# HKUST-Aerial-Robotics/FUEL

Measured on AMD Instinct MI355X. Metric: plan_cycles_per_sec, higher is better.
Workload: dtype u64 bit-planes / u16 (u32 beyond 255 voxels) exact squared distances / f32 ESDF / f64 log-odds and B-spline

## Files before the change

### fuel_amd/_lib.py

```python
import ctypes as C
import os

_HERE = os.path.dirname(os.path.abspath(__file__))
LIB_PATH = os.environ.get("FUELMI_LIB_PATH") or os.path.join(_HERE, "libfuelmi.so")
_LIB = None

K_INFLATE, K_ESDF_ZY, K_ESDF_X, K_FRONTIER, K_BSPLINE, K_INSERT, K_COUNT = range(7)


class FuelmiError(RuntimeError):
    pass


class MapCfg(C.Structure):
    _fields_ = [
        ("resolution", C.c_double),
        ("map_size", C.c_double * 3),
        ("ground_height", C.c_double),
        ("obstacles_inflation", C.c_double),
        ("local_bound_inflate", C.c_double),
        ("default_dist", C.c_double),
        ("optimistic", C.c_int),
        ("signed_dist", C.c_int),
        ("p_hit", C.c_double),
# ... 204 lines not shown
RENDER_HOST_NODE, RENDER_CUDA_NODE = 0, 1


class BsplineCfg(C.Structure):
    _fields_ = [(n, C.c_double) for n in
                ("ld_smooth", "ld_dist", "ld_feasi", "ld_start", "ld_end", "ld_guide", "ld_waypt",
                 "ld_view", "ld_time", "dist0", "max_vel", "max_acc", "wnl", "dlmin")] + \
               [("bspline_degree", C.c_int)]


_dp = C.POINTER(C.c_double)
_ip = C.POINTER(C.c_int)


class BsplineBatch(C.Structure):
    _fields_ = [
        ("cost_function", C.c_int), ("dim", C.c_int), ("point_num", C.c_int), ("n_traj", C.c_int),
        ("x", _dp), ("pt_dist", _dp), ("knot_span", _dp), ("time_lb", _dp),
        ("start_state", _dp), ("end_state", _dp), ("end_n", C.c_int),
        ("guide_pts", _dp), ("waypoints", _dp), ("waypt_idx", _ip), ("n_waypt", C.c_int),
        ("view_pt", _dp), ("view_dir", _dp), ("view_idx", _ip),
    ]


_P = C.c_void_p
_PP = C.POINTER(C.c_void_p)
SYMBOLS = {
    "fuelmi_last_error": (C.c_char_p, []),
    "fuelmi_version": (C.c_char_p, []),
    "fuelmi_init": (C.c_int, [C.c_int]),
    "fuelmi_hw_queues": (C.c_int, []),
    "fuelmi_hw_queues_state": (C.c_int, []),
    "fuelmi_device_count": (C.c_int, []),
    "fuelmi_map_create": (C.c_int, [C.POINTER(MapCfg), _PP]),
    "fuelmi_map_destroy": (None, [_P]),
    "fuelmi_map_get_info": (C.c_int, [_P, C.POINTER(MapInfo)]),
    "fuelmi_map_input_points": (C.c_int, [_P, C.c_void_p, C.c_int, C.c_int, _dp]),
    "fuelmi_map_insert_plan": (C.c_int, [_ip]),
    "fuelmi_map_input_depth": (C.c_int, [_P, C.c_void_p, C.c_int, C.c_int, C.POINTER(DepthCfg), _dp, _dp,
                                         C.POINTER(C.c_int)]),
    "fuelmi_host_register": (C.c_int, [C.c_void_p, C.c_size_t]),
    "fuelmi_host_unregister": (C.c_int, [C.c_void_p]),
    "fuelmi_device_alloc": (C.c_int, [C.c_int, C.c_size_t, C.POINTER(C.c_void_p)]),
    "fuelmi_device_upload": (C.c_int, [C.c_void_p, C.c_void_p, C.c_size_t]),
    "fuelmi_device_free": (C.c_int, [C.c_void_p]),
    "fuelmi_hbm_triad": (C.c_int, [C.c_int, C.c_size_t, C.c_int, _dp]),
    "fuelmi_hbm_expand": (C.c_int, [C.c_int, C.c_size_t, C.c_int, _dp]),
    "fuelmi_map_project_depth": (C.c_int, [_P, C.c_void_p, C.c_int, C.c_int, C.POINTER(DepthCfg), _dp, _dp,
                                           C.c_void_p, C.c_int, C.POINTER(C.c_int)]),
    "fuelmi_map_inflate_local": (C.c_int, [_P]),
    "fuelmi_map_update_esdf": (C.c_int, [_P]),
    "fuelmi_map_set_esdf_family": (C.c_int, [_P, C.c_int]),
    "fuelmi_map_last_esdf_family": (C.c_int, [_P]),
    "fuelmi_map_esdf_plan": (C.c_int, [_ip, _ip, _ip, C.c_int, C.c_int, _ip]),
    "fuelmi_map_last_inflate_kernel": (C.c_int, [_P]),
    "fuelmi_map_reset_buffer_all": (C.c_int, [_P]),
    "fuelmi_map_reset_buffer": (C.c_int, [_P, _dp, _dp]),
    "fuelmi_map_set_occupied": (C.c_int, [_P, _dp, C.c_int, C.c_int]),
    "fuelmi_map_get_local_bound": (C.c_int, [_P, _ip, _ip]),
    "fuelmi_map_set_local_bound": (C.c_int, [_P, _ip, _ip]),
    "fuelmi_map_get_updated_box": (C.c_int, [_P, _dp, _dp, C.c_int]),
    "fuelmi_map_set_updated_box": (C.c_int, [_P, _dp, _dp]),
    "fuelmi_map_upload_occupancy": (C.c_int, [_P, _dp]),
    "fuelmi_map_sync_host": (C.c_int, [_P, _ip, _ip, _dp, C.c_void_p, _dp]),
    "fuelmi_map_register_mirrors": (C.c_int, [_P, _dp, C.c_void_p, _dp]),
    "fuelmi_map_unregister_mirrors": (C.c_int, [_P]),
    "fuelmi_map_dist_grad": (C.c_int, [_P, _dp, C.c_int, _dp, _dp]),
    "fuelmi_map_coarse_dist": (C.c_int, [_P, _dp, C.c_int, _dp]),
    "fuelmi_map_query_state": (C.c_int, [_P, _ip, C.c_int, _ip, _ip]),
    "fuelmi_map_synchronize": (C.c_int, [_P]),
    "fuelmi_frontier_set_viewpoint_cfg": (C.c_int, [_P, C.POINTER(ViewpointCfg)]),
    "fuelmi_frontier_compute_to_visit": (C.c_int, [_P, C.POINTER(C.c_int), C.POINTER(C.c_int)]),
    "fuelmi_frontier_viewpoint_count": (C.c_int, [_P, C.c_int, C.c_int]),
    "fuelmi_frontier_viewpoints": (C.c_int, [_P, C.c_int, C.c_int, _dp, C.POINTER(C.c_int)]),
    "fuelmi_frontier_is_covered": (C.c_int, [_P, C.POINTER(C.c_int)]),
    "fuelmi_frontier_cluster_filtered_size": (C.c_int, [_P, C.c_int, C.c_int]),
    "fuelmi_frontier_cluster_filtered": (C.c_int, [_P, C.c_int, C.c_int, C.c_void_p]),
    "fuelmi_frontier_create": (C.c_int, [_P, C.POINTER(FrontierCfg), _PP]),
    "fuelmi_frontier_destroy": (None, [_P]),
    "fuelmi_frontier_reset": (C.c_int, [_P]),
    "fuelmi_frontier_stats": (C.c_int, [_P, C.POINTER(C.c_int)]),
    "fuelmi_frontier_resolved_in_launch": (C.c_int, [_P]),
    "fuelmi_frontier_path_stats": (C.c_int, [_P, C.POINTER(C.c_int)]),
    "fuelmi_frontier_changed_stats": (C.c_int, [_P, C.POINTER(C.c_int)]),
    "fuelmi_frontier_order_stats": (C.c_int, [_P, C.POINTER(C.c_int)]),
    "fuelmi_frontier_synchronize": (C.c_int, [_P]),
    "fuelmi_bench_cycles": (C.c_int, [_P, _P, _P, _dp, _dp, C.c_int, C.c_int, C.POINTER(C.c_int), _dp]),
    "fuelmi_bench_host_profile": (C.c_int, [_P, _dp]),
    "fuelmi_bench_cycles_delivered": (C.c_int, [_P, _P, _P, _dp, _dp, C.c_int, _ip, C.c_size_t, _dp, _dp,
                                                C.POINTER(C.c_int), _dp]),
    "fuelmi_bench_stream": (C.c_int, [_P, _P, _P, C.c_int, C.POINTER(C.c_void_p), C.c_int, C.c_int, C.POINTER(DepthCfg),
                                      _dp, _dp, C.c_int, C.POINTER(C.c_int), _dp, _dp]),
    "fuelmi_frontier_search": (C.c_int, [_P, _ip]),
    "fuelmi_frontier_search_begin": (C.c_int, [_P]),
    "fuelmi_frontier_search_end": (C.c_int, [_P, _ip]),
    "fuelmi_frontier_keep_previous": (C.c_int, [_P, C.c_int]),
    "fuelmi_frontier_commit": (C.c_int, [_P, C.c_int]),
    "fuelmi_frontier_count": (C.c_int, [_P, C.c_int]),
    "fuelmi_frontier_cluster_size": (C.c_int, [_P, C.c_int, C.c_int]),
    "fuelmi_frontier_cluster_cells": (C.c_int, [_P, C.c_int, C.c_int, _ip]),
    "fuelmi_frontier_cluster_centres": (C.c_int, [_P, C.c_int, C.c_int, _dp]),
    "fuelmi_frontier_cluster_info": (C.c_int, [_P, C.c_int, C.c_int, _dp]),
    "fuelmi_frontier_removed_count": (C.c_int, [_P]),
    "fuelmi_frontier_removed_ids": (C.c_int, [_P, _ip]),
    "fuelmi_frontier_get_flags": (C.c_int, [_P, C.c_void_p]),
    "fuelmi_map_path_costs": (C.c_int, [_P, C.POINTER(PathCfg), C.c_int, _dp, _dp, _dp, _ip, _ip, _dp]),
    "fuelmi_map_path_stats": (C.c_int, [_P, _ip]),
    "fuelmi_map_refine_tours": (C.c_int, [_P, C.POINTER(RefineCfg), C.c_int, _dp, _ip, _ip, _dp, _ip, _dp, _ip, _dp]),
    "fuelmi_map_goal_paths": (C.c_int, [_P, C.POINTER(GoalCfg), C.c_int, _dp, _dp, _ip, _dp, _ip, _dp, _dp, _ip, _dp]),
    "fuelmi_map_goal_path_times": (C.c_int, [_P, _dp]),
    "fuelmi_map_waypoint_trajs": (C.c_int, [_P, C.POINTER(WptrajCfg), C.c_int, _ip, _dp, _dp, _dp, _ip, _dp, _dp, _ip, _dp,
                                            _ip, _dp, _dp, _dp, _dp]),
    "fuelmi_wptraj_plan": (C.c_int, [C.POINTER(WptrajCfg), _ip]),
    "fuelmi_map_kino_paths": (C.c_int, [_P, C.POINTER(KinoCfg), C.c_int, _dp, _dp, _dp, _dp, _dp, _ip, _ip, _ip, _ip, _ip,
                                        _dp, _dp, _dp, _ip, _dp, _dp, _dp, _dp, _ip, _ip, _dp, _dp]),
    "fuelmi_bspline_dev_load_kino": (C.c_int, [_P, C.POINTER(KinoCfg), _dp, _dp, _dp, _dp, _dp, _ip, _dp]),
    "fuelmi_kino_plan": (C.c_int, [C.POINTER(KinoCfg), C.POINTER(C.c_longlong)]),
    "fuelmi_map_topo_paths": (C.c_int, [_P, C.POINTER(TopoCfg), C.c_int, _dp, _dp, C.c_int, _ip, _dp, C.c_int, _ip, _dp, _dp,
                                        _ip, _ip, _ip, _ip, _ip, _ip, _dp, _ip, _ip, _dp, _ip, _dp, _ip, _dp, _ip, _dp]),
    "fuelmi_topo_plan": (C.c_int, [C.POINTER(TopoCfg), C.POINTER(C.c_longlong)]),
    "fuelmi_map_topo_pool_bytes": (C.c_longlong, [_P]),
    "fuelmi_map_collision_ranges": (C.c_int, [_P, C.POINTER(ColRangeCfg), C.c_int, _ip, _dp, _dp, _ip, _ip, _ip, _ip, _dp,
                                              _dp, _dp, _dp, _ip, _dp, _ip, _dp, _dp, _dp]),
    "fuelmi_colrange_plan": (C.c_int, [C.POINTER(ColRangeCfg), _ip]),
    "fuelmi_map_guide_points": (C.c_int, [_P, C.c_int, C.c_int, _dp, _ip, _dp, C.c_double, C.c_int, C.c_int, _ip, _ip, _dp,
                                          _ip, _ip, _ip, _dp]),
    "fuelmi_map_local_segments": (C.c_int, [_P, C.POINTER(LocalSegCfg), C.c_int, _ip, _dp, _dp, _dp, _ip, _dp, _dp, _dp, _dp,
                                            _dp, _dp, C.c_int, _ip, _ip, _dp, _dp, _dp, _ip, _ip, _dp, _ip, _dp, _dp, _ip,
                                            _dp, _dp, _ip, _dp]),
    "fuelmi_localseg_plan": (C.c_int, [C.POINTER(LocalSegCfg), _ip]),
    "fuelmi_bspline_dev_load_local_segments": (C.c_int, [_P, C.c_int, C.c_int, C.c_int, _ip, _dp, _dp, _dp, _ip, _dp, _dp,
                                                         _dp, _dp, _dp, _dp, _ip, _ip, _dp, _dp, _dp, _ip, _dp]),
    "fuelmi_map_info_gains": (C.c_int, [_P, C.POINTER(GainCfg), C.c_int, _dp, _ip, _dp, C.c_int, _ip, _dp, _ip, _ip, _dp, _ip,
                                        _ip, _ip]),
    "fuelmi_map_yaw_paths": (C.c_int, [_P, C.POINTER(YawPathCfg), C.c_int, _ip, _dp, _dp, _dp, _ip, _dp, _dp, _ip, _dp, _ip,
                                       _dp, _dp, _ip]),
    "fuelmi_yawpath_plan": (C.c_int, [C.POINTER(YawPathCfg), _ip]),
    "fuelmi_map_plan_yaws": (C.c_int, [_P, C.POINTER(BsplineCfg), C.POINTER(YawCfg), C.c_int, _ip, _dp, _dp, _dp, _dp, _ip,
                                       _dp, _ip, _dp, _dp, _ip, _dp, _dp, _dp, _dp, _dp]),
    "fuelmi_bspline_dev_plan_yaws": (C.c_int, [_P, C.POINTER(YawCfg), _dp, _dp, _ip, _dp, _ip, _dp, _dp, _ip, _dp, _dp,
                                               _dp, _dp, _dp]),
    "fuelmi_yaw_plan": (C.c_int, [C.POINTER(YawCfg), _ip]),
    "fuelmi_map_check_trajs": (C.c_int, [_P, C.POINTER(TrajChkCfg), C.c_int, _ip, _dp, _dp, _dp, _ip, _ip, _dp, _ip, _ip, _dp,
                                         _dp, _ip, _dp]),
    "fuelmi_bspline_dev_check_trajs": (C.c_int, [_P, C.POINTER(TrajChkCfg), _dp, _ip, _ip, _dp, _ip, _ip, _dp, _dp, _ip, _dp]),
    "fuelmi_traj_check_plan": (C.c_int, [C.POINTER(TrajChkCfg), _ip]),
    "fuelmi_map_sample_trajs": (C.c_int, [_P, C.POINTER(TrajSmpCfg), C.c_int, _ip, _dp, _dp, _ip, _dp, _dp, _dp, _ip, _dp,
                                          _ip, _dp, _dp, _dp, _dp, _dp, _dp, _dp, _dp, _dp]),
    "fuelmi_bspline_dev_sample_trajs": (C.c_int, [_P, C.POINTER(TrajSmpCfg), _ip, _dp, _dp, _dp, _ip, _dp, _ip, _dp, _dp,
                                                  _dp, _dp, _dp, _dp, _dp, _dp, _dp]),
    "fuelmi_traj_sample_plan": (C.c_int, [C.POINTER(TrajSmpCfg), _ip]),
    "fuelmi_map_adjust_trajs": (C.c_int, [_P, C.POINTER(TrajAdjCfg), C.c_int, _ip, _dp, _dp, _dp, _dp, _ip, _ip, _dp, _dp, _dp,
                                          _ip]),
    "fuelmi_bspline_dev_adjust_trajs": (C.c_int, [_P, C.POINTER(TrajAdjCfg), _dp, _dp, _ip, _ip, _dp, _dp, _dp, _ip]),
    "fuelmi_traj_adjust_plan": (C.c_int, [C.POINTER(TrajAdjCfg), _ip]),
    "fuelmi_map_extract_cloud": (C.c_int, [_P, C.POINTER(CloudCfg), C.c_void_p, C.c_int, _ip]),
    "fuelmi_cloud_plan": (C.c_int, [_ip, _ip, _ip, _ip]),
    "fuelmi_map_cloud_times": (C.c_int, [_P, _dp]),
    "fuelmi_tsp_create": (C.c_int, [C.c_int, C.POINTER(TspCfg), _PP]),
    "fuelmi_tsp_destroy": (None, [_P]),
    "fuelmi_tsp_solve": (C.c_int, [_P, C.c_int, _ip, C.POINTER(C.c_int32), _ip, C.POINTER(C.c_int64), _ip]),
    "fuelmi_render_create": (C.c_int, [C.POINTER(RenderCfg), _PP]),
    "fuelmi_render_destroy": (C.c_int, [_P]),
    "fuelmi_render_set_cloud": (C.c_int, [_P, C.c_void_p, C.c_int]),
    "fuelmi_render_depth": (C.c_int, [_P, C.c_int, _dp, _dp, C.c_double, C.c_void_p, C.c_void_p, _ip]),
    "fuelmi_render_frame_raw": (C.c_void_p, [_P, C.c_int]),
# ... 50 lines not shown
```

### fuel_amd/csrc/frontier.hip

```cpp
#include <algorithm>
#include <chrono>
#include <cmath>
#include <cstdlib>
#include <cstring>
#include <list>
#include <memory>
#include <vector>

#include "fuelmi_internal.h"
#include "frontier_internal.h"

__global__ void k_zero_words(u64* p, int n) {
  for (int i = blockIdx.x * blockDim.x + threadIdx.x; i < n; i += gridDim.x * blockDim.x) p[i] = 0ull;
}

template <typename T>
static int dmalloc(fuelmi_frontier* f, T** p, size_t n) {
  void* d = nullptr;
  HIPCHK(hipMalloc(&d, std::max<size_t>(n, 1) * sizeof(T)));
  f->allocs.push_back(d);
  *p = (T*)d;
  const char* fp = reinterpret_cast<const char*>(p), *f0 = reinterpret_cast<const char*>(&f->F);
  if (fp >= f0 && fp < f0 + sizeof(FArgs))
    f->f_scratch.push_back({(size_t)(fp - f0), std::max<size_t>(n, 1) * sizeof(T)});
// ... 304 lines not shown
    std::swap(f->F, f->F2);
    if (f->pool_dirty) HIPCHK(hipStreamWaitEvent(f->stream, f->ev_tail, 0));
    f->pool_dirty = false;
  }
  std::swap(f->flag, f->flag2);
  f->flag_cur ^= 1;
  f->F.flag = f->flag.p;
  f->zero_deferred = true;
  return defer_zeroing ? FUELMI_OK : frontier_finish_reset(f);
}

extern "C" int fuelmi_frontier_search_begin(fuelmi_frontier* f) {
  ARGCHK(f);
  FRONTIER_HAS_MAP(f);
  FRONTIER_NOT_SEARCHING(f, "fuelmi_frontier_search_begin");
  fuelmi_map* m = f->map;
  HIPCHK(hipSetDevice(m->device));
  const Geo& g = m->g;
  FArgs& F = f->F;
  f->tmp.clear();
  g_ht.start();
  {
    const int rcm = frontier_materialize_lists(f);
    if (rcm) return rcm;
  }
  {
    const int rcr = frontier_apply_reset(f, true);
    if (rcr) return rcr;
  }
  struct FinishReset {
    fuelmi_frontier* f;
    ~FinishReset() {
      (void)frontier_finish_reset(f);
      g_ht.lap(9);
    }
  } finish_reset{f};
  g_ht.lap(0);
  double umin[3], umax[3];
  fuelmi_map_get_updated_box(m, umin, umax, 1);

  if (f->planes_waited[f->flag_cur] != m->planes_ver + 1) {
    HIPCHK(hipStreamWaitEvent(f->stream, m->ev_planes, 0));
    f->planes_waited[f->flag_cur] = m->planes_ver + 1;
  }
  f->scope.reset(new StageScope(m, FUELMI_K_FRONTIER, f->stream));
  f->removed_ids.clear();
  for (int q = 0; q < 3; ++q) f->rm_lo[q] = 1, f->rm_hi[q] = 0;
  g_ht.lap(1);
  struct PlanesRead {
    fuelmi_frontier* f;
    bool done = false;
    ~PlanesRead() {
      if (done || !f->map) return;
      if (!f->mark_planes_read)
        map_add_late_reader(f->map, f->stream, f->ev_planes_read, &f->mark_planes_read);
      else if (hipEventRecord(f->ev_planes_read, f->stream) == hipSuccess)
        map_add_plane_reader(f->map, f->ev_planes_read);
    }
  } planes_read{f};
  int rc = remove_changed_begin(f, umin, umax);
  if (rc) return rc;
  g_ht.lap(2);

  const int nv[3] = {g.nx, g.ny, g.nz};
  FVar hv;
  memset(&hv, 0, sizeof(hv));
  bool empty = false;
  for (int k = 0; k < 3; ++k) {
    double infl = (k == 2) ? 0.5 : 1.0;
    double smin = std::max(umin[k] - infl, m->cfg.box_min[k]);
    double smax = std::min(umax[k] + infl, m->cfg.box_max[k]);
    int lo = (int)std::floor((smin - g.org[k]) * g.res_inv);
    int hi = (int)std::floor((smax - g.org[k]) * g.res_inv);
    lo = std::max(lo, 0);
    hi = std::min(hi, nv[k] - 1);
    hv.sbox.lo[k] = lo;
    hv.sbox.hi[k] = hi;
    if (lo > hi) empty = true;
  }
  f->pending = true;
  f->fusion_at_begin = m->fusion_count;
  f->search_empty = empty;
  f->fast_launched = false;
  if (empty) return FUELMI_OK;

  int rlo[3], rhi[3];
  const bool all = f->dirty_all || f->seen_epoch != m->occ_epoch;
  for (int k = 0; k < 3; ++k) {
    rlo[k] = hv.sbox.lo[k], rhi[k] = hv.sbox.hi[k];
    if (f->rm_lo[0] <= f->rm_hi[0]) rlo[k] = std::min(rlo[k], f->rm_lo[k]), rhi[k] = std::max(rhi[k], f->rm_hi[k]);
    if (all) rlo[k] = 0, rhi[k] = nv[k] - 1;
    hv.qreg.lo[k] = std::max(F.qbox.lo[k], rlo[k]);
    hv.qreg.hi[k] = std::min(F.qbox.hi[k], rhi[k]);
  }
  f->dirty_all = true;
  bool have_q = true;
  for (int k = 0; k < 3; ++k)
    if (hv.qreg.lo[k] > hv.qreg.hi[k]) have_q = false;
  if (!have_q)
    for (int k = 0; k < 3; ++k) hv.qreg.lo[k] = 1, hv.qreg.hi[k] = 0;
  hv.nty = hv.ntiles = 0;
  hv.nty_f = hv.ntiles_f = 0;
  hv.ftx = 4, hv.fty = 8;
  if (have_q) {
    const int qx = hv.qreg.hi[0] - hv.qreg.lo[0] + 1, qy = hv.qreg.hi[1] - hv.qreg.lo[1] + 1;
    hv.nty = (qy + f->TY - 1) / f->TY;
    hv.ntiles = ((qx + f->TX - 1) / f->TX) * hv.nty;
  }
  {
    int p0[2], p1[2];
    for (int k = 0; k < 2; ++k) {
      p0[k] = hv.sbox.lo[k], p1[k] = hv.sbox.hi[k];
      if (have_q) p0[k] = std::min(p0[k], hv.qreg.lo[k]), p1[k] = std::max(p1[k], hv.qreg.hi[k]);
      p0[k] = std::max(p0[k], F.qbox.lo[k]);
      p1[k] = std::min(p1[k], F.qbox.hi[k] + 1);
    }
    const int qx = p1[0] - p0[0] + 1, qy = p1[1] - p0[1] + 1;
    int pick = 3;
    for (int k = 0; k < 4; ++k)
      if (menu_tiles(qx, qy, k) >= 512) {
        pick = k;
        break;
      }
    if (f->menu_min_ttl > 0) --f->menu_min_ttl, pick = std::max(pick, f->menu_min);
    f->fast_menu = pick;
    hv.px0 = p0[0], hv.py0 = p0[1], hv.px1 = p1[0], hv.py1 = p1[1];
    set_fast_tiles(hv, pick);
  }
  auto adr = [&](const int* id) { return (long)id[0] * g.nyz + (long)id[1] * g.nz + id[2]; };
  long a_lo = adr(hv.sbox.lo), a_hi = adr(hv.sbox.hi);
  if (have_q) {
    a_lo = std::min(a_lo, adr(hv.qreg.lo));
    a_hi = std::max(a_hi, adr(hv.qreg.hi));
  }
  a_lo = std::max(0L, a_lo - 2L * g.nyz);
  a_hi = std::min((long)g.N - 1, a_hi + 2L * g.nyz);
  hv.w0 = (int)((a_lo >> 6) & ~255L);
  const int w_hi = (int)(a_hi >> 6);
  hv.nblocks = (w_hi - hv.w0) / 256 + 1;
  hv.nwords = hv.nblocks * 256;
  const bool fast = f->fast_ok;
  hv.fresh = 0;
  if (F.dbg)
    HIPCHK(hipMemsetAsync(F.dbg, 0, (size_t)(3 * (hv.ntiles_f + 1)) * FR_DBG_SLOTS * sizeof(unsigned long long), f->stream));
  hv.epoch = ++f->epoch;
  if (hv.epoch == 0u) hv.epoch = f->epoch = 1u;
  *f->h_var = hv;

  f->npass = f->last_nkept > 192 ? 2 : 1;

  g_ht.lap(3);
  if (fast) {
    f->fast_launched = true;
    planes_read.done = true;
    return frontier_enqueue_fast(f);
  }
  return frontier_launch_legacy(f, f->npass);
}

static void frontier_timing_report(fuelmi_frontier* f) {
  const FArgs& F = f->F;
  (void)hipStreamSynchronize(f->stream);
  const int nt = f->h_var->ntiles_f;
  std::vector<unsigned long long> d((size_t)(3 * (nt + 1)) * FR_DBG_SLOTS);
  (void)hipMemcpy(d.data(), F.dbg, d.size() * sizeof(unsigned long long), hipMemcpyDeviceToHost);
  unsigned long long t0 = ~0ull, t1 = 0;
  double phase[8] = {0, 0, 0, 0, 0, 0, 0, 0};
  int busiest = 0, nonempty = 0;
  for (int b = 0; b < nt; ++b) {
    const unsigned long long* r = &d[(size_t)b * FR_DBG_SLOTS];
    if (!r[0]) continue;
    t0 = std::min(t0, r[0]);
    for (int k = 1; k < 8; ++k)
      if (r[k]) t1 = std::max(t1, r[k]);
    if (r[8] > d[(size_t)busiest * FR_DBG_SLOTS + 8]) busiest = b;
    if (r[8]) ++nonempty;
  }
  {
    double st_av = 0, st_mx = 0, du_av = 0, du_mx = 0;
    int cnt = 0;
    for (int b = 0; b < nt; ++b) {
      const unsigned long long* r = &d[(size_t)b * FR_DBG_SLOTS];
      if (!r[0] || !r[6] || r[6] < r[0]) continue;
      const double st = (double)(r[0] - t0) / 100.0, du = (double)(r[6] - r[0]) / 100.0;
      st_av += st, st_mx = std::max(st_mx, st), du_av += du, du_mx = std::max(du_mx, du), ++cnt;
    }
    std::fprintf(stderr, "[fr-timing] ccl: %d tiles with cells: start avg %.1f max %.1f, duration avg %.1f max %.1f us\n", cnt,
                 st_av / std::max(cnt, 1), st_mx, du_av / std::max(cnt, 1), du_mx);
  }
  const unsigned long long* rb = &d[(size_t)busiest * FR_DBG_SLOTS];
  for (int k = 1; k < 8; ++k) phase[k] = rb[k] && rb[k - 1] ? (double)(rb[k] - rb[k - 1]) / 100.0 : 0.0;
  std::fprintf(stderr, "[fr-timing] tiles %d (non-empty %d) span %.1f us; busiest tile %d (%llu cells, start +%.1f us): "
               "bits %.1f labels %.1f unions %.1f roots %.1f records %.1f write %.1f us; %llu unions, %llu find steps, %llu links, %llu roots\n", nt, nonempty,
               (double)(t1 - t0) / 100.0, busiest, rb[8], (double)(rb[0] - t0) / 100.0, phase[1], phase[2], phase[3],
               phase[4], phase[5], phase[6], rb[9], rb[10], rb[11], rb[12]);
  for (int kern = 1; kern <= 2; ++kern) {
    const int np = kern == 1 ? 4 : 6;
    double mx[8] = {0}, av[8] = {0};
    unsigned long long c0 = ~0ull, c1 = 0;
    int cnt = 0;
    for (int b = 0; b < nt; ++b) {
      const unsigned long long* r = &d[(size_t)(kern * (nt + 1) + b) * FR_DBG_SLOTS];
      if (!r[0] || !r[np]) continue;
      c0 = std::min(c0, r[0]), c1 = std::max(c1, r[np]);
      for (int k = 1; k <= np; ++k) {
        const double ph = r[k] && r[k - 1] ? (double)(r[k] - r[k - 1]) / 100.0 : 0.0;
        mx[k] = std::max(mx[k], ph), av[k] += ph;
      }
      ++cnt;
    }
    double st_av = 0, st_mx = 0, du_av = 0, du_mx = 0;
    for (int b = 0; b < nt; ++b) {
      const unsigned long long* r = &d[(size_t)(kern * (nt + 1) + b) * FR_DBG_SLOTS];
      if (!r[0] || !r[np]) continue;
      const double st = (double)(r[0] - c0) / 100.0, du = (double)(r[np] - r[0]) / 100.0;
      st_av += st, st_mx = std::max(st_mx, st), du_av += du, du_mx = std::max(du_mx, du);
    }
    {
      unsigned long long e0 = ~0ull;
      double ea = 0, em = 0, la = 0, lm = 0;
      int n2 = 0;
      for (int b = 0; b < nt; ++b) {
        const unsigned long long v = d[(size_t)b * FR_DBG_SLOTS + 12 + kern];
        if (v) e0 = std::min(e0, v);
      }
      for (int b = 0; b < nt; ++b) {
        const unsigned long long v = d[(size_t)b * FR_DBG_SLOTS + 12 + kern];
        const unsigned long long* r = &d[(size_t)(kern * (nt + 1) + b) * FR_DBG_SLOTS];
        if (!v || !r[0] || r[0] < v) continue;
        const double e = (double)(v - e0) / 100.0, l = (double)(r[0] - v) / 100.0;
        ea += e, em = std::max(em, e), la += l, lm = std::max(lm, l), ++n2;
      }
      std::fprintf(stderr, "[fr-timing]   entry avg %.1f max %.1f us after the first workgroup; entry -> first stamp avg %.1f max %.1f us\n",
                   ea / std::max(n2, 1), em, la / std::max(n2, 1), lm);
    }
    std::fprintf(stderr, "[fr-timing] %s: span %.1f us over %d tiles; start avg %.1f max %.1f, duration avg %.1f max %.1f; phases avg/max:",
                 kern == 1 ? "cross (bits, build, list, append)" : "out (bits, cells, column, first, rows, flags)",
                 cnt ? (double)(c1 - c0) / 100.0 : 0.0, cnt, st_av / std::max(cnt, 1), st_mx, du_av / std::max(cnt, 1), du_mx);
    for (int k = 1; k <= np; ++k) std::fprintf(stderr, " %.1f/%.1f", av[k] / std::max(cnt, 1), mx[k]);
    std::fprintf(stderr, "\n");
  }
  const unsigned long long* rr = &d[(size_t)nt * FR_DBG_SLOTS];
  std::fprintf(stderr, "[fr-timing] resolve: init %.1f unions %.1f find %.1f reduce %.1f clusters %.1f seeds %.1f rank %.1f "
               "codes %.1f publish %.1f us; pairs %llu roots %llu cells %llu\n", (rr[1] - rr[0]) / 100.0,
               (rr[2] - rr[1]) / 100.0, (rr[3] - rr[2]) / 100.0, (rr[4] - rr[3]) / 100.0, (rr[5] - rr[4]) / 100.0, 0.0,
               (rr[6] - rr[5]) / 100.0, (rr[7] - rr[6]) / 100.0, (rr[8] - rr[7]) / 100.0, rr[9], rr[10], rr[11]);
}

static int frontier_collect_fast(fuelmi_frontier* f) {
  fuelmi_map* m = f->map;
  FArgs& F = f->F;
  u32* counts = F.h_counts;
  volatile u32* stamp = counts + 15;
  const u32 want = f->h_var->epoch;
  const auto w0 = std::chrono::steady_clock::now();
  const int rcw = stamp_wait<u32>(stamp, want, f->stream, "frontier search: the chain finished without publishing its result");
  f->wait_us_acc += std::chrono::duration<double, std::micro>(std::chrono::steady_clock::now() - w0).count();
  if (rcw) return rcw;
  g_ht.lap(11);
  f->tail_pending = true;
  F.fast = 1;
  if (F.dbg) frontier_timing_report(f);
  if (counts[2] == 3u) {
    *stamp = 0u;
    const int rcl = frontier_enqueue_late_resolve(f);
    if (rcl) return rcl;
    const int rc = stamp_wait<u32>(stamp, want, f->stream, "frontier search: k_resolve finished without publishing its result");
    if (rc) return rc;
    ++f->n_late_resolve;
  }
  f->kr_skip_ok = counts[2] == 0u && counts[9] == 1u && 2u * counts[10] <= f->rcap_used;
  ++f->n_fast;
  if (counts[9] == 1u)
    ++f->n_in_launch;
  else if (f->fuse_tried && counts[2] == 0u)
    f->fuse_skip = 16;
  if (counts[2] == 2u && m->fusion_count != f->fusion_at_begin) {
    fuelmi_set_error("frontier search: the fast chain overflowed AFTER the map was fused again (a frame queued between "
                     "_search_begin and _search_end): the occupancy this search was about is gone -- call _search_end before the next fusion "
                     "on inputs this noisy");
    remove_changed_end(f);
    f->dirty_all = true;
    return FUELMI_ELIMIT;
  }
  while (counts[2] == 2u && f->fast_menu < 3 && (counts[6] == 11u || counts[6] == 12u || counts[6] == 15u || counts[6] == 18u)) {
    HIPCHK(frontier_tail_sync(f) == FUELMI_OK ? hipSuccess : hipErrorUnknown);
    ++f->fast_menu;
    FVar hv = *f->h_var;
    set_fast_tiles(hv, f->fast_menu);
    hv.epoch = ++f->epoch;
    if (hv.epoch == 0u) hv.epoch = f->epoch = 1u;
    *f->h_var = hv;
    f->kr_skip_ok = false;
    if (getenv("FUELMI_FR_TIMING")) std::fprintf(stderr, "[fr-timing] capacity code %u: again with %d x %d tiles\n", counts[6], hv.ftx, hv.fty);
    const int rcr = frontier_enqueue_fast(f);
    if (rcr) return rcr;
    const int rcw = stamp_wait<u32>(stamp, hv.epoch, f->stream,
                                    "frontier search: the re-tiled chain finished without publishing its result");
    if (rcw) return rcw;
    f->tail_pending = true;
    ++f->n_retiled;
    f->menu_min = f->fast_menu, f->menu_min_ttl = 64;
  }
  if (counts[2] == 2u) {
    --f->n_fast;
    ++f->n_fallback;
    if (getenv("FUELMI_FR_TIMING")) std::fprintf(stderr, "[fr-timing] fallback to the legacy chain: capacity code %u\n", counts[6]);
    HIPCHK(frontier_tail_sync(f) == FUELMI_OK ? hipSuccess : hipErrorUnknown);
    F.fast = 0;
    f->npass = 1;
    int rcl = frontier_enqueue_chain(f, f->npass);
    if (rcl) return rcl;
    HIPCHK(hipStreamSynchronize(f->stream));
  }
  return FUELMI_OK;
}


static int frontier_assemble(fuelmi_frontier* f, u32 nq, u32 nkept, u32 n_out) {
  const Geo& g = f->map->g;
  FArgs& F = f->F;
  KeptRec* h_rec = F.h_rec;
  const u32* h_part = F.h_part;
  const u32* h_cells = F.h_cells;
  u32 ncl = nkept, ncells = n_out;
  std::vector<std::vector<float>> filtered;
  const bool split_mode = f->cfg.split != 0;
  bool ref_order = f->cfg.reference_order == 1;
  if (f->cfg.reference_order == 2) {
    ref_order = true;
    for (u32 r = 0; r < nkept; ++r)
      if (h_rec[r].size > FR_REFORDER_AUTO) ref_order = false;
  }
  f->ref_now = ref_order;
  f->order_last = ref_order ? 1 : 0;
  if (ref_order)
    ++f->n_order_ref;
  else if (f->cfg.reference_order == 2) {
    ++f->n_order_fallback;
    u32 big = 0;
    for (u32 r = 0; r < nkept; ++r) big = std::max(big, h_rec[r].size);
    f->order_fallback_cells = big;
  }
  int fin = nkept <= 256 ? 1 : 0;
  std::vector<u32> off2;
  u32 n_in = n_out;
  if (split_mode && !ref_order) HIPCHK(frontier_tail_sync(f) == FUELMI_OK ? hipSuccess : hipErrorUnknown);
  if (ref_order) {
    int rc = frontier_reference_order(f, nq, nkept, n_out, fin, &n_in, &off2, !split_mode);
    if (rc) return rc;
    f->tail_pending = false;
    fin = 1 - fin;
    ncells = n_in;
  }
  if (split_mode) {
    int rc = frontier_split_run(f, nq, nkept, n_in, fin, &ncl, &ncells, &filtered);
    if (rc) return rc;
    fin = ncl <= 256 ? 1 : 0;
  }
  f->last_fin = fin;
  f->cells_fetch = F.fast && !ref_order && !split_mode && nq > F.hcells_direct_max;
  f->cells_fetch_n = ncells;
  const u32 nchunk = ((ref_order || F.fast) && !split_mode) ? 0u : (ncells + SZ_CH - 1) / SZ_CH;
  for (u32 c = 0; c < nchunk; ++c) {
    const u32* rec = h_part + (size_t)c * 10;
    const u32 r = rec[0];
    if (r >= ncl) continue;
    for (int q = 0; q < 3; ++q) {
      h_rec[r].sum[q] += rec[1 + q];
      h_rec[r].box[q] = std::min(h_rec[r].box[q], rec[4 + q]);
      h_rec[r].box[3 + q] = std::max(h_rec[r].box[3 + q], rec[7 + q]);
    }
  }

  for (u32 r = 0; r < ncl; ++r) {
    const KeptRec& kr = h_rec[r];
    f->tmp.emplace_back();
    HCluster& c = f->tmp.back();
    const bool seed = !split_mode && kr.slot >= nq;
    const u32 cnt = kr.size - (seed ? 1u : 0u);
    c.lazy = reinterpret_cast<const int*>(h_cells) + kr.off;
    c.lazy_n = cnt;
    if (ref_order && !split_mode) {
      c.lazy = reinterpret_cast<const int*>(h_cells) + off2[r];
      c.lazy_n = kr.size;
    }
// ... 69 lines not shown
    ~DropLate() {
      if (f->map) map_drop_late_reader(f->map, f->ev_planes_read);
    }
  } drop_late{f};
  if (f->search_empty) {
    if (!f->pend_rm.empty()) {
      HIPCHK(hipStreamSynchronize(f->stream));
      remove_changed_end(f);
    }
    return FUELMI_OK;
  }
  FArgs& F = f->F;
  const u32* counts = F.h_counts;
  F.fast = 0;
  g_ht.start();
  if (g_ht.on) --g_ht.n;
  g_ht.lap(10);
  if (f->fast_launched) {
    const int rc = frontier_collect_fast(f);
    if (rc) return rc;
  } else {
    ++f->n_legacy;
    HIPCHK(stream_poll(f->stream));
  }
  remove_changed_end(f);
  if (f->rm_failed) {
    f->rm_failed = false;
    f->dirty_all = true;
    fuelmi_set_error("frontier search: the changed-cluster test's in-kernel barrier timed out (device oversubscribed for 50 ms?)");
    return FUELMI_EHIP;
  }
  if (counts[2] || counts[3] > F.cap_kept) {
    fuelmi_set_error("frontier capacity exceeded (cells %u/%u seeds %u/%u clusters %u/%u)", counts[0], F.cap_q,
                     counts[1], F.cap_s, counts[3], F.cap_kept);
    return FUELMI_ELIMIT;
  }
  const u32 nq = counts[0], nkept = counts[3], n_out = counts[5];
  f->last_nkept = (int)nkept;
  if (nkept > 256 && f->npass < 2) {
    const int rc = frontier_second_pass(f);
    if (rc) return rc;
  }
  if (nkept == 0) {
    f->dirty_all = false;
    f->seen_epoch = m->occ_epoch;
    return FUELMI_OK;
  }
  const int rc = frontier_assemble(f, nq, nkept, n_out);
  if (rc) return rc;
  *n_new = (int)f->tmp.size();
  f->dirty_all = false;
  f->seen_epoch = m->occ_epoch;
  g_ht.lap(12);
  return FUELMI_OK;
}


extern "C" int fuelmi_frontier_search(fuelmi_frontier* f, int* n_new) {
  ARGCHK(f && n_new);
  int rc = fuelmi_frontier_search_begin(f);
  if (rc) return rc;
  return fuelmi_frontier_search_end(f, n_new);
}

extern "C" int fuelmi_frontier_synchronize(fuelmi_frontier* f) {
  ARGCHK(f);
  FRONTIER_HAS_MAP(f);
  HIPCHK(hipSetDevice(f->device));
  f->tail_pending = false;
  HIPCHK(frontier_drain(f));
  return FUELMI_OK;
}
extern "C" int fuelmi_frontier_resolved_in_launch(const fuelmi_frontier* f) { return f ? f->n_in_launch : FUELMI_EINVAL; }
extern "C" int fuelmi_frontier_stats(const fuelmi_frontier* f, int out3[3]) {
  ARGCHK(f && out3);
  out3[0] = f->n_fast, out3[1] = f->n_legacy, out3[2] = f->n_fallback;
  return FUELMI_OK;
}
extern "C" int fuelmi_frontier_path_stats(const fuelmi_frontier* f, int out2[2]) {
  ARGCHK(f && out2);
  out2[0] = f->n_late_resolve, out2[1] = f->n_retiled;
  return FUELMI_OK;
}
extern "C" int fuelmi_frontier_changed_stats(const fuelmi_frontier* f, int out[9]) {
  ARGCHK(f && out);
  for (int k = 0; k < 4; ++k) out[k] = f->rm_paths[k];
  out[4] = f->rm_last_nc, out[5] = (int)f->rm_last_total, out[6] = f->rm_last_mark;
  out[7] = f->n_pool_rebuilds, out[8] = (int)f->pool_cap;
  return FUELMI_OK;
}
extern "C" int fuelmi_frontier_order_stats(const fuelmi_frontier* f, int out4[4]) {
  ARGCHK(f && out4);
  out4[0] = f->order_last, out4[1] = f->n_order_ref, out4[2] = f->n_order_fallback, out4[3] = (int)f->order_fallback_cells;
  return FUELMI_OK;
}

extern "C" int fuelmi_frontier_reset(fuelmi_frontier* f) {
  ARGCHK(f);
  FRONTIER_HAS_MAP(f);
  FRONTIER_NOT_SEARCHING(f, "fuelmi_frontier_reset");
  fuelmi_map* m = f->map;
  HIPCHK(hipSetDevice(m->device));
  f->frontiers.clear();
  f->dormant.clear();
  f->prev.clear();
  if (f->keep_prev && f->stream2 && !f->fresh_pending && !f->tmp.empty()) {
    f->prev.swap(f->tmp);
    if (f->cells_fetch) {
      f->cells_fetch = false;
      HIPCHK(hipMemcpyAsync(f->F.h_cells, f->F.ms_val[f->last_fin], (size_t)f->cells_fetch_n * sizeof(u32), hipMemcpyDeviceToHost,
                            f->stream));
    }
    HIPCHK(hipEventRecord(f->ev_prev, f->stream));
    f->prev_pending = true;
    f->tail_pending = false;
  }
  f->tmp.clear();
  f->removed_ids.clear();
  f->dirty_all = true;
  f->pool_used = 0;
  f->fresh_pending = true;
  return FUELMI_OK;
}

extern "C" int fuelmi_frontier_keep_previous(fuelmi_frontier* f, int on) {
  ARGCHK(f);
  f->keep_prev = on != 0;
  if (!on) f->prev.clear();
  return FUELMI_OK;
}

extern "C" int fuelmi_frontier_commit(fuelmi_frontier* f, int dormant) {
  ARGCHK(f);
  FRONTIER_HAS_MAP(f);
  FRONTIER_NOT_SEARCHING(f, "fuelmi_frontier_commit");
  auto& dst = dormant ? f->dormant : f->frontiers;
  HIPCHK(hipSetDevice(f->map->device));
  const int rc = frontier_keep_clusters(f, f->tmp);
  if (rc) return rc;
  dst.splice(dst.end(), f->tmp);
  return FUELMI_OK;
}
```

### fuel_amd/csrc/frontier_internal.h

```cpp
#ifndef FUELMI_FRONTIER_INTERNAL_H_
#define FUELMI_FRONTIER_INTERNAL_H_

#include <algorithm>
#include <chrono>
#include <cstring>
#include <list>
#include <memory>
#include <vector>

#include "fuelmi_internal.h"

#define NOCLAIM 0xFFFFFFFFu
#define SZ_CH 1024

struct KeptRec {
  u32 addr, slot, size, off;
  unsigned long long sum[3];
  u32 box[6];
  u32 pad[2];
};

struct FVar {
  Box3 sbox;
  int w0;
  int nwords;
  int nblocks;
  int fresh;
  Box3 qreg;
  int nty, ntiles;
  u32 epoch;
  int pad2;
  int nty_f, ntiles_f;
  int ftx, fty;
  int px0, py0, px1, py1;
  int ntx_f;
  int pad3[3];
};

#define FR_RCAP 8192
#define FR_RC8 (FR_RCAP / 8)
#define FR_TCELL 2048
#define FR_TPAIR 1536
#define FR_TROOT 128
#define FR_TXS 16
#define FR_KCAP 256
#define FR_PCAP (1u << 18)
#define FCTR(k) ((k) * 32)
#define FR_DONE_CTR FCTR(32)
#define FR_NCTR (41 * 32)
#define FR_PMCAP 16384
#define FR_REFORDER_AUTO 26624u
#define FR_UNCLAIMED 0xFFFFFFFFu
#define FR_NOTKEPT 0xFFFFFFFEu
struct TRec {
  u32 size;
  u32 sx, sy, sz;
  u32 lo[3], hi[3];
  u32 tx;
  u32 own;
};

struct FArgs {
  Box3 qbox;
  const FVar* var;
  u32 cap_q, cap_s;
  int cluster_min;
  const u64* occ;
  const u64* unk;
  u64* flag;
  u64* qb;
  u64* sb;
  u64* pref;
  u64* blocksum;
  u64* blockscan;
  u32* counts;
  u32* cell_adr;
  u32* parent;
  u32* claim;
  int* cell_slot;
  u32* seed_adr;
  u32* csize;
  u32* kept;
  u32 cap_kept;
  int* slot2rank;
  struct KeptRec* krec;
  u32* ms_key[2];
  u32* ms_val[2];
  u32* ms_hist;
  u32 ms_nb_max;
  u32* info_part;
  u32* h_counts;
  struct KeptRec* h_rec;
  u32* h_part;
  u32* h_cells;
  u32 hcells_direct_max;
  int keys_from_slots;
  FVar* var_w;
  u32* tq;
  u32* ts;
  unsigned char* vlab;
  unsigned char* tlab;
  u32* t_base;
  u32* t_nroots;
  struct TRec* trec;
  u32* tclaim;
  u32* rcode;
  unsigned short* rrow;
  u32* pm;
  int pm_stride;
  u32* pairs;
  u32* fctr;
  int fast;
  unsigned long long* dbg;
};
#define FR_HCELLS_DIRECT 32768u
#define FR_DBG_SLOTS 16
#define FR_DBG_MARK(F, blk, k)                                                                   \
  do {                                                                                           \
    if ((F).dbg && threadIdx.x == 0) (F).dbg[(size_t)(blk) * FR_DBG_SLOTS + (k)] = wall_clock64(); \
  } while (0)

#ifdef __HIPCC__
__device__ __forceinline__ void st_agent(u32* p, u32 v) { __hip_atomic_store(p, v, __ATOMIC_RELAXED, __HIP_MEMORY_SCOPE_AGENT); }
__device__ __forceinline__ u32 ld_agent(const u32* p) { return __hip_atomic_load(p, __ATOMIC_RELAXED, __HIP_MEMORY_SCOPE_AGENT); }
__device__ __forceinline__ void wait_vm_stores() { asm volatile("s_waitcnt vmcnt(0)" ::: "memory"); }
__device__ __forceinline__ void ld_agent_trec2(const TRec* p0, const TRec* p1, TRec& A, TRec& B) {
  static_assert(sizeof(TRec) == 48, "TRec is fetched as three 16-byte pieces");
  uint4 a0, a1, a2, b0, b1, b2;
  asm volatile(
      "global_load_dwordx4 %0, %6, off sc1\n\t"
      "global_load_dwordx4 %1, %6, off offset:16 sc1\n\t"
      "global_load_dwordx4 %2, %6, off offset:32 sc1\n\t"
      "global_load_dwordx4 %3, %7, off sc1\n\t"
      "global_load_dwordx4 %4, %7, off offset:16 sc1\n\t"
      "global_load_dwordx4 %5, %7, off offset:32 sc1\n\t"
      "s_waitcnt vmcnt(0)"
      : "=&v"(a0), "=&v"(a1), "=&v"(a2), "=&v"(b0), "=&v"(b1), "=&v"(b2)
      : "v"(p0), "v"(p1)
      : "memory");
  A.size = a0.x, A.sx = a0.y, A.sy = a0.z, A.sz = a0.w, A.lo[0] = a1.x, A.lo[1] = a1.y, A.lo[2] = a1.z, A.hi[0] = a1.w;
  A.hi[1] = a2.x, A.hi[2] = a2.y, A.tx = a2.z, A.own = a2.w;
  B.size = b0.x, B.sx = b0.y, B.sy = b0.z, B.sz = b0.w, B.lo[0] = b1.x, B.lo[1] = b1.y, B.lo[2] = b1.z, B.hi[0] = b1.w;
  B.hi[1] = b2.x, B.hi[2] = b2.y, B.tx = b2.z, B.own = b2.w;
}
__device__ __forceinline__ u32 rank_q(const FArgs& F, long a) {
  int w = (int)(a >> 6);
  int rel = w - F.var->w0;
  u64 pk = F.blockscan[rel >> 8] + F.pref[rel];
  return (u32)pk + (u32)__popcll(F.qb[w] & ((1ull << (a & 63)) - 1ull));
}
template <int CTRL, int ROW_MASK>
__device__ __forceinline__ u32 dpp_mov(u32 old, u32 v) {
  return (u32)__builtin_amdgcn_update_dpp((int)old, (int)v, CTRL, ROW_MASK, 0xF, false);
}
#define FUELMI_WAVE_RED(NAME, OP, ID)                                                        \
  __device__ __forceinline__ u32 NAME(u32 v) {                                               \
    v = OP(v, dpp_mov<0xB1, 0xF>(ID, v));                           \
    v = OP(v, dpp_mov<0x4E, 0xF>(ID, v));                           \
    v = OP(v, dpp_mov<0x141, 0xF>(ID, v));                              \
    v = OP(v, dpp_mov<0x140, 0xF>(ID, v));  \
    v = OP(v, dpp_mov<0x142, 0xA>(ID, v));                \
    v = OP(v, dpp_mov<0x143, 0xC>(ID, v));                \
    return (u32)__builtin_amdgcn_readlane((int)v, 63);                                       \
  }
__device__ __forceinline__ u32 red_add_(u32 a, u32 b) { return a + b; }
__device__ __forceinline__ u32 red_min_(u32 a, u32 b) { return min(a, b); }
__device__ __forceinline__ u32 red_max_(u32 a, u32 b) { return max(a, b); }
FUELMI_WAVE_RED(wave_add_u32, red_add_, 0u)
FUELMI_WAVE_RED(wave_min_u32, red_min_, 0xFFFFFFFFu)
FUELMI_WAVE_RED(wave_max_u32, red_max_, 0u)

__device__ __forceinline__ u64 q_window34(const Geo& g, const FVar& V, const FArgs& F, int xx, int yy, int c) {
  const bool inside = xx >= V.px0 && xx <= V.px1 && yy >= V.py0 && yy <= V.py1;
  const int xc = min(max(xx, V.px0), V.px1), yc = min(max(yy, V.py0), V.py1);
  const int nseg = (g.nz + 31) >> 5;
  const int tx = (xc - V.px0) / V.ftx, ty = (yc - V.py0) / V.fty;
  const int lx = xc - V.px0 - tx * V.ftx, ly = yc - V.py0 - ty * V.fty;
  const u32* p = F.tq + (size_t)(tx * V.nty_f + ty) * (size_t)(V.ftx * V.fty * nseg) + (size_t)(lx * V.fty + ly) * nseg + c;
  const bool has_lo = c > 0, has_hi = c + 1 < nseg;
  const u32 lo = p[has_lo ? -1 : 0], mid = p[0], hi = p[has_hi ? 1 : 0];
  const u64 w = (u64)(has_lo ? lo >> 31 : 0u) | ((u64)mid << 1) | ((u64)(has_hi ? hi & 1u : 0u) << 33);
  return inside ? w : 0ull;
}

__device__ __forceinline__ u32 q_bits3(const Geo& g, const FVar& V, const FArgs& F, int xx, int yy, int z) {
  const int c = z >> 5;
  return (u32)(q_window34(g, V, F, xx, yy, c) >> (z - 32 * c)) & 7u;
}
__device__ __forceinline__ u32 rank_s(const FArgs& F, long a) {
  int w = (int)(a >> 6);
  int rel = w - F.var->w0;
  u64 pk = F.blockscan[rel >> 8] + F.pref[rel];
  return (u32)(pk >> 32) + (u32)__popcll(F.sb[w] & ((1ull << (a & 63)) - 1ull));
}

__device__ __forceinline__ u64 f1_word(const Geo& g, const u64* __restrict__ occ, const u64* __restrict__ unk,
                                       int w, u64 z0, u64 zl, u64 y0, u64 yl) {
  long a0 = 64L * w;
  u64 valid = (a0 + 64 <= g.N) ? ~0ull : bit_range(0, (int)max(0L, g.N - a0));
  u64 free_ = ~occ[w] & ~unk[w] & valid;
  if (free_ == 0ull) return 0ull;
  u64 nb = (plane_window(unk, a0 + 1) & ~zl) | (plane_window(unk, a0 - 1) & ~z0) |
           (plane_window(unk, a0 + g.nz) & ~yl) | (plane_window(unk, a0 - g.nz) & ~y0) |
           plane_window(unk, a0 + g.nyz) | plane_window(unk, a0 - g.nyz);
  return free_ & nb;
}
__device__ __forceinline__ u32 lds_find_h(u32* lab, u32 i) {
// ... 51 lines not shown
    }
    if (lazy_seed < 0) {
      if (lazy_n) memcpy(out, lazy, (size_t)lazy_n * sizeof(int));
      return;
    }
    const size_t k = (size_t)(std::lower_bound(lazy, lazy + lazy_n, lazy_seed) - lazy);
    if (k) memcpy(out, lazy, k * sizeof(int));
    out[k] = lazy_seed;
    if (lazy_n > k) memcpy(out + k + 1, lazy + k, (lazy_n - k) * sizeof(int));
  }
  void materialize() {
    if (!lazy) return;
    std::vector<int> v(size());
    copy_to(v.data());
    cells.swap(v);
    lazy = nullptr;
  }
};

struct fuelmi_frontier {
  fuelmi_map* map = nullptr;
  int device = 0;
  fuelmi_frontier_cfg cfg;
  int iz_min = 0;
  Plane flag, qb, sb;
  Plane flag2;
  int flag_cur = 0;
  hipEvent_t ev_tail = nullptr;
  bool zero_deferred = false;
  FArgs F;
  FArgs F2;
  hipStream_t stream2 = nullptr;
  struct ScratchRec {
    size_t field_off, bytes;
  };
  std::vector<ScratchRec> f_scratch;
  void* h_pin2 = nullptr;
  bool pool_dirty = false;
  std::vector<void*> allocs;
  std::list<HCluster> frontiers, dormant, tmp;
  std::list<HCluster> prev;
  hipEvent_t ev_planes_read = nullptr;
  hipEvent_t* tl_ev = nullptr;
  hipEvent_t ev_prev = nullptr;
  bool prev_pending = false;
  unsigned long long fusion_at_begin = 0;
  bool keep_prev = false;
  std::vector<int> removed_ids;
  hipStream_t stream = nullptr;
  hipEvent_t ev_dep = nullptr;
  unsigned long long planes_waited[2] = {0, 0};
  bool mark_planes_read = false;
  void* d_stage = nullptr;
  size_t d_stage_bytes = 0;
  void* h_pin = nullptr;
  size_t pin_bytes = 0;
  int last_nkept = 0, npass = 1;
  FVar* h_var = nullptr;
  FVar* d_var = nullptr;
  int TX = 1, TY = 16, ccl_tiles = 0;
  int fast_tiles = 0;
  size_t ccl_lds = 0;
  hipGraphExec_t graph_exec[2][2] = {{nullptr, nullptr}, {nullptr, nullptr}};
  bool pending = false, search_empty = false;
  bool ref_now = false;
  mutable bool cells_fetch = false;
  mutable u32 cells_fetch_n = 0;
  bool lazy_kept = false;
  mutable bool tail_pending = false;
  bool fast_launched = false;
  u32 epoch = 0;
  int fast_menu = 0;
  bool fast_ok = false;
  bool fresh_pending = false;
  int n_fast = 0, n_legacy = 0, n_fallback = 0;
  int n_in_launch = 0;
  int fuse_skip = 0;
  bool fuse_tried = false;
  bool kr_skip_ok = false;
  bool kr_queued = true;
  u32 rcap_used = 0;
  int menu_min = 0, menu_min_ttl = 0;
  int n_retiled = 0;
  int n_late_resolve = 0;
  int order_last = 0, n_order_ref = 0, n_order_fallback = 0;
  u32 order_fallback_cells = 0;
  double wait_us_acc = 0.0;
  size_t tile_lds[4] = {0, 0, 0, 0}, cross_lds[4] = {0, 0, 0, 0}, out_lds[4] = {0, 0, 0, 0}, fast_items[4] = {0, 0, 0, 0};
  size_t resolve_lds = 0;
  std::unique_ptr<StageScope> scope;
  bool dirty_all = true;
  unsigned seen_epoch = 0;
  int rm_lo[3], rm_hi[3];
  fuelmi_viewpoint_cfg vcfg;
  bool have_vcfg = false;
  struct PendingRm {
    std::list<HCluster>* list;
    std::list<HCluster>::iterator it;
    int pos;
  };
  std::vector<PendingRm> pend_rm;
  int* h_changed = nullptr;
  size_t h_changed_cap = 0;
  void* h_cand = nullptr;
  int* d_mark = nullptr;
  int rm_mark = 0;
  u32* rm_bar = nullptr;
  u32 rm_bar_total = 0;
  bool rm_failed = false;
  int rm_paths[4] = {0, 0, 0, 0};
  int rm_last_nc = 0, rm_last_mark = 0;
  u32 rm_last_total = 0;
  int n_pool_rebuilds = 0;
  void* h_put = nullptr;
  size_t h_put_cap = 0;
  u32* pool = nullptr;
  size_t pool_cap = 0, pool_used = 0;
  int last_fin = 1;
  struct SplitScratch* split = nullptr;
  struct OrderScratch* order = nullptr;
};
void frontier_split_free(fuelmi_frontier* f);
void frontier_order_free(fuelmi_frontier* f);
int frontier_reference_order(fuelmi_frontier* f, u32 nq, u32 nkept, u32 n_out, int fin, u32* n_total,
                             std::vector<u32>* h_off2, bool fetch_cells);
struct PoolPut {
  u64 dst;
  u32 src, n;
  int seed, pad;
};
int frontier_keep_clusters(fuelmi_frontier* f, std::list<HCluster>& clusters);
int frontier_materialize_lists(fuelmi_frontier* f);
static inline int frontier_tail_sync(const fuelmi_frontier* f) {
  if (!f->tail_pending) return FUELMI_OK;
  f->tail_pending = false;
  HIPCHK(stream_poll(f->stream));
  return FUELMI_OK;
}
static inline int frontier_prev_ready(const fuelmi_frontier* f) {
  if (!f->prev_pending) return FUELMI_OK;
  HIPCHK(event_poll(f->ev_prev));
  const_cast<fuelmi_frontier*>(f)->prev_pending = false;
  return FUELMI_OK;
}
static inline int frontier_cells_ready(const fuelmi_frontier* f) {
  const int rc = frontier_tail_sync(f);
  if (rc) return rc;
  if (f->cells_fetch) {
    f->cells_fetch = false;
    HIPCHK(hipMemcpy(f->F.h_cells, f->F.ms_val[f->last_fin], (size_t)f->cells_fetch_n * sizeof(u32), hipMemcpyDeviceToHost));
  }
  return FUELMI_OK;
}
#define FRONTIER_NOT_SEARCHING(f, what)                                                        \
  do {                                                                                         \
    if ((f)->pending) {                                                                        \
      fuelmi_set_error(what ": a search is in flight (call fuelmi_frontier_search_end first)"); \
      return FUELMI_EINVAL;                                                                    \
    }                                                                                          \
  } while (0)
#define FRONTIER_HAS_MAP(f)                                                                        \
  do {                                                                                             \
    if (!(f)->map) {                                                                               \
      fuelmi_set_error("the map of this frontier finder has been destroyed: only fuelmi_frontier_destroy is legal"); \
      return FUELMI_EINVAL;                                                                        \
    }                                                                                              \
  } while (0)
#define FDBG(name)                                                                     \
  do {                                                                                 \
    static const bool on__ = getenv("FUELMI_DEBUG_SYNC") != nullptr;                   \
    if (on__) {                                                                        \
      hipError_t e__ = hipStreamSynchronize(f->stream);                                \
      std::fprintf(stderr, "[fuelmi] %s: %s\n", name, hipGetErrorString(e__));         \
    }                                                                                  \
  } while (0)
static inline int fblocks(long n, int t, int cap = 1 << 16) {
  long b = (n + t - 1) / t;
  return (int)std::max(1L, std::min((long)cap, b));
}

struct HostTiming {
  bool on = getenv("FUELMI_HOST_TIMING") != nullptr;
  double acc[16] = {0};
  long n = 0;
  std::chrono::steady_clock::time_point t;
  void start() {
    if (on) t = std::chrono::steady_clock::now(), ++n;
  }
  void lap(int k) {
    if (!on) return;
    const auto now = std::chrono::steady_clock::now();
    acc[k] += std::chrono::duration<double, std::micro>(now - t).count();
    t = now;
  }
  void report() {
    if (!on || !n) return;
    static const char* names[16] = {"b:lists+reset", "b:box+wait+scope", "b:rm_begin", "b:region", "b:launch ccl", "b:events", "b:launch cross",
                                    "b:launch resolve", "b:launch out", "b:finish_reset", "e:pre-poll", "e:poll", "e:post-poll", "", "", ""};
    std::fprintf(stderr, "[host-timing] per search:");
    for (int k = 0; k < 13; ++k) std::fprintf(stderr, " %s %.2f", names[k], acc[k] / (double)n);
    std::fprintf(stderr, "\n");
    for (double& a : acc) a = 0;
    n = 0;
  }
};

#pragma GCC visibility push(hidden)
extern HostTiming g_ht;
int frontier_ensure_stage(fuelmi_frontier* f, size_t bytes);
hipError_t frontier_drain(const fuelmi_frontier* f);
int frontier_fetch_cluster(const fuelmi_frontier* f, const HCluster* c);
int frontier_apply_reset(fuelmi_frontier* f, bool defer_zeroing = false);
int remove_changed_begin(fuelmi_frontier* f, const double* umin, const double* umax);
void remove_changed_end(fuelmi_frontier* f);
int frontier_enqueue_chain(fuelmi_frontier* f, int npass);
int frontier_launch_legacy(fuelmi_frontier* f, int npass);
int frontier_second_pass(fuelmi_frontier* f);
int frontier_legacy_attrs(fuelmi_frontier* f);
size_t frontier_tile_lds(fuelmi_frontier* f, int qx, int qy);
int frontier_tile_attrs(fuelmi_frontier* f);
bool frontier_tile_fits(const fuelmi_frontier* f);
int menu_tiles(int qx, int qy, int mk);
void set_fast_tiles(FVar& hv, int mk);
int frontier_enqueue_fast(fuelmi_frontier* f);
int frontier_enqueue_late_resolve(fuelmi_frontier* f);
#pragma GCC visibility pop


int frontier_regroup(fuelmi_frontier* f, const FArgs& F2, int npass);
int frontier_split_run(fuelmi_frontier* f, u32 nq, u32 nkept, u32 n_out, int fin, u32* n_final, u32* n_cells,
                       std::vector<std::vector<float>>* filtered);


#ifdef __HIPCC__
template <bool kBox>
__device__ bool ray_clear(const Geo& g, const u64* infl, const u64* unk, const int* bmin, const int* bmax,
                          const double start[3], const double end[3]) {
  int c[3], ec[3], st[3];
  double tmax[3], tdel[3];
  for (int k = 0; k < 3; ++k) {
    const double s = start[k] / g.res, e = end[k] / g.res;
    c[k] = (int)floor(s);
    ec[k] = (int)floor(e);
    const double d = ec[k] - c[k];
    const int di = (int)d;
    st[k] = di == 0 ? 0 : (di < 0 ? -1 : 1);
    double ss = s, ds = d;
    if (ds < 0) {
      ss = -ss;
      ds = -ds;
    }
    ss = fmod(fmod(ss, 1.0) + 1.0, 1.0);
    tmax[k] = (1 - ss) / ds;
    tdel[k] = ((double)st[k]) / d;
  }
  const double off[3] = {0.5 - g.org[0] / g.res, 0.5 - g.org[1] / g.res, 0.5 - g.org[2] / g.res};
  int guard = abs(ec[0] - c[0]) + abs(ec[1] - c[1]) + abs(ec[2] - c[2]) + 4;
  while (true) {
    const int id[3] = {(int)((double)c[0] + off[0]), (int)((double)c[1] + off[1]), (int)((double)c[2] + off[2])};
    if (c[0] == ec[0] && c[1] == ec[1] && c[2] == ec[2]) return true;
    if (kBox)
      for (int k = 0; k < 3; ++k)
        if (id[k] < bmin[k] || id[k] >= bmax[k]) return false;
    if (idx_in_map(g, id)) {
      const long a = (long)id[0] * g.nyz + (long)id[1] * g.nz + id[2];
      if (bit_at(infl, a) || bit_at(unk, a)) return false;
    }
    if (tmax[0] < tmax[1]) {
      if (tmax[0] < tmax[2]) {
        c[0] += st[0];
        tmax[0] += tdel[0];
      } else {
        c[2] += st[2];
        tmax[2] += tdel[2];
      }
    } else {
      if (tmax[1] < tmax[2]) {
        c[1] += st[1];
        tmax[1] += tdel[1];
      } else {
        c[2] += st[2];
        tmax[2] += tdel[2];
      }
    }
    if (--guard < 0) return true;
  }
}
#endif

#endif
```

### fuel_amd/csrc/frontier_tile.hip

```cpp
#include <algorithm>
#include <cstdlib>

#include "frontier_internal.h"

struct TileGeo {
  int tx, ty, x0, y0, nxl, nyl, TX, TY, nseg, items;
};
struct TilePro {
  FVar V;
  u32 ovf, nroots, gbase, pad;
};
__device__ __forceinline__ void stage_tile_pro(const FArgs& F, TilePro* sp) {
  constexpr int NV = (int)(sizeof(FVar) / 4);
  static_assert(sizeof(FVar) % 4 == 0 && NV + 3 <= 64, "FVar does not fit one wave's lanes");
  const int t = threadIdx.x;
  const u32* src = reinterpret_cast<const u32*>(F.var) + (t < NV ? t : 0);
  if (t == NV) src = F.counts + 2;
  if (t == NV + 1) src = F.t_nroots + blockIdx.x;
  if (t == NV + 2) src = F.t_base + blockIdx.x;
  if (t < NV + 3) reinterpret_cast<u32*>(sp)[t] = *src;
  __syncthreads();
}
__device__ __forceinline__ TileGeo tile_geo(const Geo& g, const FVar& V, int t) {
  TileGeo T;
  T.TX = V.ftx, T.TY = V.fty;
  T.tx = t / V.nty_f, T.ty = t - T.tx * V.nty_f;
  T.x0 = V.px0 + T.tx * T.TX, T.y0 = V.py0 + T.ty * T.TY;
  T.nxl = min(T.TX, V.px1 - T.x0 + 1), T.nyl = min(T.TY, V.py1 - T.y0 + 1);
  T.nseg = (g.nz + 31) >> 5;
  T.items = T.TX * T.TY * T.nseg;
  return T;
}
__device__ __forceinline__ long tile_line_adr(const Geo& g, const TileGeo& T, int line) {
  const int lx = line / T.TY, ly = line - lx * T.TY;
  return (long)(T.x0 + lx) * g.nyz + (long)(T.y0 + ly) * g.nz;
}

#define FT_PER 8
#define FT_TRIP 2
struct SegPred {
  u32 q, s;
};
struct __attribute__((packed, aligned(4))) W2 {
  u32 a, b;
};
struct __attribute__((packed, aligned(4))) W3 {
  u32 a, b, c;
};
__device__ __forceinline__ u32 plane_window32(const u64* __restrict__ p, long bit) {
  const u32* q = reinterpret_cast<const u32*>(p);
  const long wi = bit >> 5;
  const int sh = (int)(bit & 31);
  const W2 w = *reinterpret_cast<const W2*>(q + wi);
  return (u32)((((u64)w.b << 32) | (u64)w.a) >> sh);
}
__device__ __forceinline__ SegPred seg_predicate(const Geo& g, const FVar& V, const FArgs& F, int x, int y, int c) {
  const long a = (long)x * g.nyz + (long)y * g.nz + 32 * c;
  const int zn = min(32, g.nz - 32 * c);
  u64 W;
  {
    const u32* q = reinterpret_cast<const u32*>(F.unk);
    const long wi = (a - 1) >> 5;
    const int sh = (int)((a - 1) & 31);
    const W3 w = *reinterpret_cast<const W3*>(q + wi);
    const u64 w01 = (u64)w.a | ((u64)w.b << 32);
    W = (w01 >> sh) | (((u64)w.c << 1) << (63 - sh));
  }
  const u32 occw = plane_window32(F.occ, a);
  const u32 ym_raw = plane_window32(F.unk, a - g.nz), yp_raw = plane_window32(F.unk, a + g.nz);
  const u32 xm = plane_window32(F.unk, a - g.nyz), xp = plane_window32(F.unk, a + g.nyz);
  const u32 fl_raw = plane_window32(F.flag, a);
  const u32 ym = y > 0 ? ym_raw : 0u, yp = y < g.ny - 1 ? yp_raw : 0u;
  const u32 fl = V.fresh ? 0u : fl_raw;
  u32 down = (u32)W, up = (u32)(W >> 2);
  const u32 self_unk = (u32)(W >> 1);
  if (c == 0) down &= ~1u;
  if (g.nz - 32 * c <= 32) up &= ~(1u << (zn - 1));
  const u32 valid = zn < 32 ? (1u << zn) - 1u : 0xFFFFFFFFu;
  const u32 f1 = ~occw & ~self_unk & (down | up | ym | yp | xm | xp) & valid & ~fl;
  auto zmask = [&](const Box3& b) -> u32 {
    if (x < b.lo[0] || x > b.hi[0] || y < b.lo[1] || y > b.hi[1]) return 0u;
    const int lo = max(32 * c, b.lo[2]) - 32 * c, hi = min(32 * c + 31, b.hi[2]) - 32 * c;
    if (lo > hi) return 0u;
    return ((hi - lo + 1 >= 32) ? 0xFFFFFFFFu : ((1u << (hi - lo + 1)) - 1u)) << lo;
  };
  const u32 mq = zmask(V.qreg), ms = zmask(V.sbox);
  SegPred r;
  r.q = f1 & mq;
  r.s = f1 & ms & ~mq;
  return r;
}

template <int NT>
__device__ __forceinline__ u32 tile_load_pred(const Geo& g, const TileGeo& T, const FVar& V, const FArgs& F, u32* segb,
                                              u32* segpre, u32* s_wsum, u32* lab, u32* segs, unsigned short* cseg) {
  const int lane = threadIdx.x & 63, wave = threadIdx.x >> 6;
  const int per = (T.items + NT - 1) / NT;
  const int it0 = threadIdx.x * per;
  u32 cnt = 0u;
  int c, lx, ly;
  {
    const int line = it0 / T.nseg;
    c = it0 - line * T.nseg;
    lx = line / T.TY;
    ly = line - lx * T.TY;
  }
#pragma nounroll
  for (int k0 = 0; k0 < per; k0 += FT_TRIP) {
    SegPred r[FT_TRIP];
#pragma unroll
    for (int h = 0; h < FT_TRIP; ++h) {
      r[h].q = r[h].s = 0u;
      const int it = it0 + k0 + h;
      if (k0 + h < per && it < T.items && lx < T.nxl && ly < T.nyl) r[h] = seg_predicate(g, V, F, T.x0 + lx, T.y0 + ly, c);
      if (++c == T.nseg) {
        c = 0;
        if (++ly == T.TY) ly = 0, ++lx;
      }
    }
#pragma unroll
    for (int h = 0; h < FT_TRIP; ++h) {
      const int it = it0 + k0 + h;
      if (k0 + h < per && it < T.items) {
        segb[it] = r[h].q, segs[it] = r[h].s;
        cnt += (u32)__popc(r[h].q);
      }
    }
  }
  u32 v = cnt;
  for (int off = 1; off < 64; off <<= 1) {
    const u32 t = (u32)__shfl_up((int)v, off, 64);
    if (lane >= off) v += t;
  }
  if (lane == 63) s_wsum[wave] = v;
  __syncthreads();
  u32 woff = 0u, tot = 0u;
#pragma unroll
  for (int k = 0; k < NT / 64; ++k) {
    if (k < wave) woff += s_wsum[k];
    tot += s_wsum[k];
  }
  u32 run = woff + v - cnt;
#pragma nounroll
  for (int k = 0; k < per; ++k) {
    if (it0 + k >= T.items) break;
    u32 rem = segb[it0 + k];
    segpre[it0 + k] = run;
    if (tot <= FR_TCELL) {
      u32 l = run;
      while (rem) {
        const int s0 = __builtin_ctz(rem);
        const u32 inv = ~(rem >> s0);
        const int len = min(inv ? __builtin_ctz(inv) : 32, 32 - s0);
        rem &= ~((len >= 32 ? 0xFFFFFFFFu : ((1u << len) - 1u)) << s0);
        for (int q = 0; q < len; ++q) lab[l + (u32)q] = l, cseg[l + (u32)q] = (unsigned short)(it0 + k);
        l += (u32)len;
      }
    }
    run += (u32)__popc(segb[it0 + k]);
  }
  if (threadIdx.x == 0) segpre[T.items] = tot;
  __syncthreads();
  return tot;
}
template <int NT, bool SCAN>
__device__ __forceinline__ u32 tile_load_arrays(const TileGeo& T, const FArgs& F, u32* segb, u32* segpre, u32* s_wsum,
                                                u32* segs) {
  const int lane = threadIdx.x & 63, wave = threadIdx.x >> 6;
  const u32* tq = F.tq + (size_t)blockIdx.x * T.items;
  const u32* ts = F.ts + (size_t)blockIdx.x * T.items;
  const int per = (T.items + NT - 1) / NT;
  const int it0 = threadIdx.x * per;
  u32 b[FT_PER], b2[FT_PER];
#pragma unroll
  for (int k = 0; k < FT_PER; ++k) {
    b[k] = b2[k] = 0u;
    if (k < per && it0 + k < T.items) b[k] = tq[it0 + k], b2[k] = ts[it0 + k];
  }
  u32 cnt = 0u;
#pragma unroll
  for (int k = 0; k < FT_PER; ++k)
    if (k < per && it0 + k < T.items) {
      segb[it0 + k] = b[k], segs[it0 + k] = b2[k];
      cnt += (u32)__popc(b[k]);
    }
  if (!SCAN) {
    __syncthreads();
    return 0u;
  }
  u32 v = cnt;
  for (int off = 1; off < 64; off <<= 1) {
    const u32 t = (u32)__shfl_up((int)v, off, 64);
    if (lane >= off) v += t;
  }
  if (lane == 63) s_wsum[wave] = v;
  __syncthreads();
  u32 woff = 0u, tot = 0u;
#pragma unroll
  for (int k = 0; k < NT / 64; ++k) {
    if (k < wave) woff += s_wsum[k];
    tot += s_wsum[k];
  }
  u32 run = woff + v - cnt;
#pragma unroll
  for (int k = 0; k < FT_PER; ++k)
    if (k < per && it0 + k < T.items) {
      segpre[it0 + k] = run;
      run += (u32)__popc(b[k]);
    }
  if (threadIdx.x == 0) segpre[T.items] = tot;
  __syncthreads();
  return tot;
}
__device__ __forceinline__ void pop_run32(u32& m, int& s, int& len) {
  s = __builtin_ctz(m);
  const u32 inv = ~(m >> s);
  len = inv ? __builtin_ctz(inv) : 32;
  len = min(len, 32 - s);
  m &= ~((len >= 32 ? 0xFFFFFFFFu : ((1u << len) - 1u)) << s);
}
__device__ __forceinline__ void pop_run64(u64& m, int& s, int& len) {
  s = __builtin_ctzll(m);
  const u64 inv = ~(m >> s);
  len = inv ? __builtin_ctzll(inv) : 64;
  len = min(len, 64 - s);
  m &= ~((len >= 64 ? ~0ull : ((1ull << len) - 1ull)) << s);
}

template <int NT>
__global__ void __launch_bounds__(NT) k_tile_ccl(Geo g, FArgs F, const FVar V) {
  if (blockIdx.x == 0 && threadIdx.x == 0) *F.var_w = V;
  if ((int)blockIdx.x >= V.ntiles_f) return;
  const TileGeo T = tile_geo(g, V, blockIdx.x);
  const Box3 sbox = V.sbox;
  extern __shared__ __attribute__((aligned(16))) unsigned char smem_raw[];
  const int nz = g.nz, nseg = T.nseg, items = T.items, TY = T.TY;
  u32* lab = reinterpret_cast<u32*>(smem_raw);
  u32* segb = lab + FR_TCELL;
  u32* segpre = segb + items;
  u32* acc = segpre + items + 1;
  u32* rrow = acc + FR_TROOT * 8;
  unsigned short* rootno = reinterpret_cast<unsigned short*>(rrow + FR_TROOT * FR_TXS);
  unsigned char* rcell = reinterpret_cast<unsigned char*>(rootno + FR_TCELL);
  u32* segs = reinterpret_cast<u32*>(rcell + FR_TCELL);
  u32* plist = reinterpret_cast<u32*>(rootno);
  unsigned short* cseg = reinterpret_cast<unsigned short*>(acc);
  static_assert((size_t)FR_TCELL * sizeof(unsigned short) <= (size_t)FR_TROOT * 8 * 4 + (size_t)FR_TROOT * FR_TXS * 4, "cell -> segment table does not fit");
  static_assert((size_t)FR_TPAIR * sizeof(u32) <= FR_TCELL * sizeof(unsigned short) + FR_TCELL, "pair list does not fit");
  __shared__ u32 s_wsum[NT / 64];
  __shared__ u32 s_nroots, s_base, s_flag;
  __shared__ u32 s_cnt[4];
  const int lane = threadIdx.x & 63;
  if (threadIdx.x == 0) s_nroots = 0u, s_flag = 0u, s_cnt[0] = s_cnt[1] = s_cnt[2] = s_cnt[3] = 0u;
  FR_DBG_MARK(F, blockIdx.x, 0);
  const u32 total = tile_load_pred<NT>(g, T, V, F, segb, segpre, s_wsum, lab, segs, cseg);
  {
    u32* tq = F.tq + (size_t)blockIdx.x * items;
    u32* ts = F.ts + (size_t)blockIdx.x * items;
    for (int it = threadIdx.x; it < items; it += NT) tq[it] = segb[it], ts[it] = segs[it];
  }
  FR_DBG_MARK(F, blockIdx.x, 1);
  if (total == 0u || total > FR_TCELL) {
    if (threadIdx.x == 0) {
      F.t_nroots[blockIdx.x] = 0u;
      F.t_base[blockIdx.x] = 0u;
      if (total > FR_TCELL) F.fctr[FCTR(9)] = 11u;
    }
    return;
  }
  FR_DBG_MARK(F, blockIdx.x, 2);
  __shared__ u32 s_np, s_chg, s_povf;
  if (threadIdx.x == 0) s_np = 0u, s_chg = 0u, s_povf = 0u;
  __syncthreads();
  auto walk_pairs = [&](auto&& fn) {
    for (u32 l = threadIdx.x; l < total; l += NT) {
      const int it = cseg[l];
      const u32 bits = segb[it];
      u32 k = l - segpre[it], rem = bits;
      while (k--) rem &= rem - 1u;
      const int zz = __builtin_ctz(rem);
      const int line = it / nseg, c = it - line * nseg, lx = line / TY, ly = line - lx * TY;
      const int z = 32 * c + zz;
      const bool seam = zz == 0 && c > 0 && (segb[it - 1] >> 31);
      const u32 own = seam ? l : lab[l];
      u32 pk[9];
      u32 nv = 0u;
      pk[0] = (l << 16) | (l - 1u);
      if (seam) nv |= 1u;
      const bool has_prev = seam || (zz > 0 && ((bits >> (zz - 1)) & 1u));
#pragma unroll
      for (int q = 0; q < 4; ++q) {
        pk[1 + 2 * q] = pk[2 + 2 * q] = 0u;
        const int nlx = lx + (q < 3 ? -1 : 0), nly = ly + (q < 3 ? q - 1 : -1);
        if (nlx < 0 || nly < 0 || nly >= TY) continue;
        const int nline = nlx * TY + nly;
        const int zlo = z - 1;
        const int s0 = max(zlo, 0) >> 5;
        const u64 w = (u64)segb[nline * nseg + s0] | ((s0 + 1 < nseg) ? ((u64)segb[nline * nseg + s0 + 1] << 32) : 0ull);
        u32 pat = (zlo >= 0) ? (u32)((w >> (zlo - 32 * s0)) & 7ull) : (u32)((w << 1) & 6ull);
        if (z + 1 >= nz) pat &= 3u;
        if (has_prev) pat = (pat & 6u) == 4u ? 4u : 0u;
        if (!pat) continue;
        const int zn = zlo + __builtin_ctz(pat);
        const int nit = nline * nseg + (zn >> 5);
        const u32 ln = segpre[nit] + (u32)__popc(segb[nit] & ((1u << (zn & 31)) - 1u));
        pk[1 + 2 * q] = (own << 16) | ln;
        nv |= 1u << (1 + 2 * q);
        if (pat == 5u) {
          pk[2 + 2 * q] = (own << 16) | (ln + 1u);
          nv |= 1u << (2 + 2 * q);
        }
      }
      fn(pk, nv);
    }
  };
  walk_pairs([&](const u32 (&pk)[9], u32 nv) {
    const u32 cnt = (u32)__popc(nv);
    u32 excl = 0u, tot = 0u;
#pragma unroll
    for (int b = 0; b < 4; ++b) {
      const unsigned long long bal = __ballot((cnt >> b) & 1u);
      excl += (u32)__builtin_amdgcn_mbcnt_hi((u32)(bal >> 32), __builtin_amdgcn_mbcnt_lo((u32)bal, 0u)) << b;
      tot += (u32)__popcll(bal) << b;
    }
    if (tot == 0u) return;
    const int leader = __builtin_ctzll(__ballot(1));
    u32 at = 0u;
    if (lane == leader) at = atomicAdd(&s_np, tot);
    at = (u32)__shfl((int)at, leader, 64) + excl;
#pragma unroll
    for (int k = 0; k < 9; ++k)
      if ((nv >> k) & 1u) {
        if (at < FR_TPAIR)
          plist[at] = pk[k];
        else
          s_povf = 1u;
        ++at;
      }
  });
  __syncthreads();
  {
    volatile u32* vl = lab;
    const u32 np = min(s_np, (u32)FR_TPAIR);
    for (;;) {
      bool any = false;
      for (u32 p = threadIdx.x; p < np; p += NT) {
        const u32 pr = plist[p];
        const u32 ru = vl[pr >> 16], rv = vl[pr & 0xFFFFu];
        if (ru != rv) {
          atomicMin(&lab[max(ru, rv)], min(ru, rv));
          any = true;
        }
      }
      if (any) s_chg = 1u;
      __syncthreads();
      const bool again = s_chg != 0u;
      __syncthreads();
      if (!again) break;
      if (threadIdx.x == 0) s_chg = 0u;
      for (u32 i = threadIdx.x; i < total; i += NT) {
        u32 r = vl[i];
        for (;;) {
          const u32 rr = vl[r];
          if (rr == r) break;
          r = rr;
        }
        vl[i] = r;
      }
      __syncthreads();
    }
  }
  if (s_povf) {
    walk_pairs([&](const u32 (&pk)[9], u32 nv) {
#pragma unroll
      for (int k = 0; k < 9; ++k)
        if ((nv >> k) & 1u) lds_union_h(lab, pk[k] >> 16, pk[k] & 0xFFFFu);
    });
  }
  __syncthreads();
  for (int t = threadIdx.x; t < FR_TROOT * 8; t += NT) {
    const int k = t & 7;
    acc[t] = (k >= 2 && k <= 4) ? 0xFFFFFFFFu : 0u;
  }
  for (int t = threadIdx.x; t < FR_TROOT * FR_TXS; t += NT) rrow[t] = 0u;
  FR_DBG_MARK(F, blockIdx.x, 3);
  for (u32 l = threadIdx.x; l < total; l += NT)
    if (lab[l] == l) {
      const u32 la = atomicAdd(&s_nroots, 1u);
      rootno[l] = (unsigned short)min(la, 0xFFFFu);
    }
  __syncthreads();
  const u32 nroots = s_nroots;
  if (nroots > FR_TROOT) {
    if (threadIdx.x == 0) {
      F.fctr[FCTR(9)] = 12u;
      F.t_nroots[blockIdx.x] = 0u;
      F.t_base[blockIdx.x] = 0u;
    }
    return;
  }
  if (threadIdx.x == 0) {
    const u32 xcd = blockIdx.x & 7u;
    const u32 b = atomicAdd(&F.fctr[FCTR(xcd)], nroots);
    if (b + nroots > FR_RC8) {
      F.fctr[FCTR(9)] = 13u;
      s_flag = 1u;
    }
    s_base = xcd * FR_RC8 + b;
  }
  for (u32 l = threadIdx.x; l < total; l += NT) rcell[l] = (unsigned char)rootno[lds_find_h(lab, l)];
  __syncthreads();
  FR_DBG_MARK(F, blockIdx.x, 4);
  for (int line0 = 0; line0 < T.TX * TY; line0 += NT) {
    const int line = line0 + threadIdx.x;
    const bool act = line < T.TX * TY;
    const int lx = line / TY, ly = line - lx * TY;
    const u32 x = (u32)(T.x0 + lx), y = (u32)(T.y0 + ly);
    const bool xy_in = (int)x >= sbox.lo[0] && (int)x <= sbox.hi[0] && (int)y >= sbox.lo[1] && (int)y <= sbox.hi[1];
    const long la = (long)x * g.nyz + (long)y * nz;
    u32 key = 0xFFFFFFFFu, n = 0u, sz = 0u, cl = 0xFFFFFFFFu, lz = 0xFFFFFFFFu, hz = 0u;
    auto flush = [&]() {
      u32* r = acc + key * 8u;
      atomicAdd(&r[0], n * y), atomicAdd(&r[1], sz), atomicMin(&r[2], cl), atomicMin(&r[3], y), atomicMin(&r[4], lz);
      atomicMax(&r[5], y), atomicMax(&r[6], hz);
      atomicAdd(&rrow[key * FR_TXS + (u32)lx], n);
    };
    for (int c = 0; act && c < nseg; ++c) {
      const int it = line * nseg + c;
      u32 rem = segb[it];
      u32 l = segpre[it];
      while (rem) {
        int s, len;
        pop_run32(rem, s, len);
        const u32 k2 = (u32)rcell[l];
        if (k2 != key) {
          if (key != 0xFFFFFFFFu) flush();
          key = k2, n = 0u, sz = 0u, cl = 0xFFFFFFFFu, lz = 0xFFFFFFFFu, hz = 0u;
        }
        const u32 z0 = (u32)(32 * c + s), z1 = z0 + (u32)len - 1u;
        n += (u32)len;
        sz += (u32)len * z0 + (u32)(len * (len - 1) / 2);
        lz = min(lz, z0), hz = max(hz, z1);
        if (xy_in) {
          const int zc = max((int)z0, sbox.lo[2]);
          if (zc <= min((int)z1, sbox.hi[2])) cl = min(cl, (u32)(la + zc));
        }
        l += (u32)len;
      }
    }
    const bool have = key != 0xFFFFFFFFu;
    const u64 hm = __ballot(have);
    if (hm) {
      const u32 first = (u32)__shfl((int)key, __builtin_ctzll(hm), 64);
      const bool uni = __ballot(have && key != first) == 0ull;
      if (uni) {
        u32 sy = have ? n * y : 0u, s2 = have ? sz : 0u, c2 = have ? cl : 0xFFFFFFFFu;
        u32 ly2 = have ? y : 0xFFFFFFFFu, lz2 = have ? lz : 0xFFFFFFFFu, hy2 = have ? y : 0u, hz2 = have ? hz : 0u;
        sy = wave_add_u32(sy), s2 = wave_add_u32(s2), c2 = wave_min_u32(c2), ly2 = wave_min_u32(ly2);
        lz2 = wave_min_u32(lz2), hy2 = wave_max_u32(hy2), hz2 = wave_max_u32(hz2);
        if (lane == __builtin_ctzll(hm)) {
          u32* r = acc + first * 8u;
          atomicAdd(&r[0], sy), atomicAdd(&r[1], s2), atomicMin(&r[2], c2), atomicMin(&r[3], ly2), atomicMin(&r[4], lz2);
          atomicMax(&r[5], hy2), atomicMax(&r[6], hz2);
        }
        if (have) atomicAdd(&rrow[key * FR_TXS + (u32)lx], n);
      } else if (have)
        flush();
    }
  }
  __syncthreads();
  FR_DBG_MARK(F, blockIdx.x, 5);
  const u32 gbase = s_base;
  if (threadIdx.x == 0) {
    F.t_base[blockIdx.x] = gbase;
    F.t_nroots[blockIdx.x] = s_flag ? 0u : nroots;
  }
  if (s_flag) return;
  if (threadIdx.x < nroots) {
    const u32* r = acc + threadIdx.x * 8;
    const u32* rw = rrow + threadIdx.x * FR_TXS;
    TRec R;
    u32 size = 0u, sx = 0u, lox = 0xFFFFFFFFu, hix = 0u;
    unsigned short* grow = F.rrow + (size_t)(gbase + threadIdx.x) * FR_TXS;
    for (int lx = 0; lx < FR_TXS; ++lx) {
      const u32 cnt = lx < T.TX ? rw[lx] : 0u;
      grow[lx] = (unsigned short)cnt;
      if (cnt) {
        size += cnt, sx += cnt * (u32)(T.x0 + lx);
        lox = min(lox, (u32)(T.x0 + lx)), hix = max(hix, (u32)(T.x0 + lx));
      }
    }
    R.size = size, R.sx = sx, R.sy = r[0], R.sz = r[1];
    R.lo[0] = lox, R.lo[1] = r[3], R.lo[2] = r[4], R.hi[0] = hix, R.hi[1] = r[5], R.hi[2] = r[6];
    R.tx = (u32)T.tx, R.own = r[2];
    F.trec[gbase + threadIdx.x] = R;
    F.tclaim[gbase + threadIdx.x] = r[2];
  }
  {
    unsigned char* tl = F.tlab + (size_t)blockIdx.x * FR_TCELL;
    for (u32 l = threadIdx.x; l < total; l += NT) tl[l] = rcell[l];
  }
  for (int it = threadIdx.x; it < items; it += NT) {
    u32 rem = segb[it];
    if (!rem) continue;
    const int line = it / nseg, c = it - line * nseg;
    unsigned char* vl = F.vlab + tile_line_adr(g, T, line) + 32 * c;
    u32 l = segpre[it];
    while (rem) {
      const int b = __builtin_ctz(rem);
      rem &= rem - 1u;
      vl[b] = rcell[l++];
    }
  }
  FR_DBG_MARK(F, blockIdx.x, 6);
  if (F.dbg && threadIdx.x == 0) {
    F.dbg[(size_t)blockIdx.x * FR_DBG_SLOTS + 8] = total;
    F.dbg[(size_t)blockIdx.x * FR_DBG_SLOTS + 9] = s_cnt[0];
    F.dbg[(size_t)blockIdx.x * FR_DBG_SLOTS + 10] = s_cnt[1];
    F.dbg[(size_t)blockIdx.x * FR_DBG_SLOTS + 11] = s_cnt[2];
    F.dbg[(size_t)blockIdx.x * FR_DBG_SLOTS + 12] = nroots;
  }
}

#define XC_SET 256
#define XC_WCAP 6144
template <int RS_T, bool IN_LAUNCH>
__device__ __forceinline__ bool resolve_body(const Geo& g, const FArgs& F, const FVar& V, unsigned char* smem_raw, const u32 rcap);

__device__ __forceinline__ void xc_insert(u32* s_set, u32* s_list, u32* s_n, u32* fctr, u32 key) {
  u32 h = (key * 2654435761u) >> 24;
  bool done = false;
  for (int probe = 0; probe < XC_SET && !done; ++probe) {
    const u32 old = atomicCAS(&s_set[h], 0xFFFFFFFFu, key);
    if (old == 0xFFFFFFFFu) {
      s_list[atomicAdd(s_n, 1u)] = key;
      done = true;
    } else if (old == key)
      done = true;
    h = (h + 1u) & (XC_SET - 1u);
  }
  if (!done) st_agent(&fctr[FCTR(9)], 15u);
}
template <int NT>
__global__ void __launch_bounds__(NT) k_tile_cross(Geo g, FArgs F, const u32 rcap) {
  FR_DBG_MARK(F, blockIdx.x, 13);
  __shared__ TilePro s_pro;
  stage_tile_pro(F, &s_pro);
  const FVar& V = s_pro.V;
  if ((int)blockIdx.x >= V.ntiles_f) return;
  const TileGeo T = tile_geo(g, V, blockIdx.x);
  const int nz = g.nz, nseg = T.nseg, TY = T.TY;
  const int lane = threadIdx.x & 63;
  extern __shared__ __attribute__((aligned(16))) unsigned char smem_raw[];
  u32* segq = reinterpret_cast<u32*>(smem_raw);
  u32* segs = segq + T.items;
  u32* wl = segs + T.items;
  __shared__ u32 s_set[XC_SET];
  __shared__ u32 s_list[XC_SET];
  __shared__ u32 s_n, s_base, s_nw;
  __shared__ u32 s_tb[9];
  const int dblk = V.ntiles_f + 1 + (int)blockIdx.x;
  FR_DBG_MARK(F, dblk, 0);
  u32 tb9;
  {
    const int t9 = (int)threadIdx.x % 9, dtx = t9 / 3 - 1, dty = t9 % 3 - 1;
    const int ntx = T.tx + dtx, nty = T.ty + dty;
    const bool ok = ntx >= 0 && ntx < V.ntx_f && nty >= 0 && nty < V.nty_f;
    tb9 = F.t_base[ok ? ntx * V.nty_f + nty : (int)blockIdx.x];
    if (!ok) tb9 = 0u;
  }
  if (threadIdx.x < XC_SET) s_set[threadIdx.x] = 0xFFFFFFFFu;
  if (threadIdx.x == 0) s_n = 0u, s_nw = 0u;
  tile_load_arrays<NT, false>(T, F, segq, nullptr, nullptr, segs);
  if (threadIdx.x < 9) s_tb[threadIdx.x] = tb9;
  FR_DBG_MARK(F, dblk, 1);
  auto tile_of = [&](int x, int y) -> u32 {
    const int dtx = x < T.x0 ? -1 : (x >= T.x0 + T.TX ? 1 : 0), dty = y < T.y0 ? -1 : (y >= T.y0 + TY ? 1 : 0);
    return (u32)((dtx + 1) * 3 + dty + 1);
  };
  u32 k0 = 0xFFFFFFFFu, k1 = 0xFFFFFFFFu;
  auto do_item = [&](u32 bits, u32 own, int nb, u32 info, u64 w3) {
    const int c = (int)(info & 0xFFu);
    const u32 tb = s_tb[(info >> 8) & 0xFFu];
    w3 &= (1ull << 34) - 1ull;
    if (c == 0) w3 &= ~1ull;
    const int jend = nz - 32 * c + 1;
    if (jend < 34) w3 &= (1ull << jend) - 1ull;
    if (info >> 16) {
      while (w3) {
        int j, rl;
        pop_run64(w3, j, rl);
        const int b0 = max(j - 2, 0), b1 = min(j + rl - 1, 31);
        if (b0 > b1) continue;
        const u32 m = bits & (((b1 - b0 + 1 >= 32) ? 0xFFFFFFFFu : ((1u << (b1 - b0 + 1)) - 1u)) << b0);
        if (!m) continue;
        const u32 r = tb + (u32)F.vlab[(long)nb + j];
        atomicMin(&F.tclaim[r], own + (u32)__builtin_ctz(m));
      }
      return;
    }
    u32 rem = bits;
    while (rem && w3) {
      int s, len;
      pop_run32(rem, s, len);
      u64 m = (w3 >> s) & ((1ull << (len + 2)) - 1ull);
      if (!m) continue;
      const u32 ga = s_tb[4] + (u32)F.vlab[(long)own + s];
      while (m) {
        int j, rl;
        pop_run64(m, j, rl);
        const u32 gb = tb + (u32)F.vlab[(long)nb + s + j];
        if (gb == ga) continue;
        const u32 key = (min(ga, gb) << 16) | max(ga, gb);
        if (key == k0 || key == k1) continue;
        if (k0 == 0xFFFFFFFFu)
          k0 = key;
        else if (k1 == 0xFFFFFFFFu)
          k1 = key;
        else
          xc_insert(s_set, s_list, &s_n, F.fctr, key);
      }
    }
  };
  auto flush_pairs = [&]() {
#pragma unroll
    for (int q = 0; q < 2; ++q) {
      const u32 kq = q ? k1 : k0;
      const bool on = kq != 0xFFFFFFFFu;
      u64 todo = __ballot(on);
      while (todo) {
        const int leader = __builtin_ctzll(todo);
        const u32 key = (u32)__shfl((int)kq, leader, 64);
        todo &= ~__ballot(on && kq == key);
        if (lane == leader) xc_insert(s_set, s_list, &s_n, F.fctr, key);
      }
    }
    k0 = k1 = 0xFFFFFFFFu;
  };
  auto decode = [&](u32 e, u32& bits, u32& own, int& nb, u32& info, int& xx, int& yy) {
    int it, c;
    if (e >> 31) {
      const int sj = (int)(e & 0x7FFFFFFFu), l = sj % 9;
      it = sj / 9;
      const int line = it / nseg, lx = line / TY, ly = line - lx * TY;
      c = it - line * nseg;
      xx = T.x0 + lx + l / 3 - 1, yy = T.y0 + ly + l % 3 - 1;
      bits = (xx >= V.px0 && xx <= V.px1 && yy >= V.py0 && yy <= V.py1) ? segs[it] : 0u;
      own = (u32)((long)(T.x0 + lx) * g.nyz + (long)(T.y0 + ly) * nz + 32 * c);
      info = (u32)c | (tile_of(xx, yy) << 8) | (1u << 16);
    } else {
      const int k = (int)(e & 3u), fs = (int)(e >> 2), fl = fs / nseg;
      c = fs - fl * nseg;
      int lx = 0, ly = fl;
      if (fl >= TY) lx = 1 + ((fl - TY) >> 1), ly = ((fl - TY) & 1) ? TY - 1 : 0;
      xx = T.x0 + lx + (k < 3 ? -1 : 0), yy = T.y0 + ly + (k < 3 ? k - 1 : -1);
      bits = segq[(lx * TY + ly) * nseg + c];
      own = (u32)((long)(T.x0 + lx) * g.nyz + (long)(T.y0 + ly) * nz + 32 * c);
      info = (u32)c | (tile_of(xx, yy) << 8);
    }
    nb = (int)((long)xx * g.nyz + (long)yy * nz + 32 * c - 1);
  };
  const int nfl = TY + 2 * (T.nxl - 1);
  const int fitems = nfl * nseg * 4;
  for (int fi = threadIdx.x; fi < fitems; fi += NT) {
    const int k = fi & 3, fs = fi >> 2, fl = fs / nseg, c = fs - fl * nseg;
    int lx = 0, ly = fl;
    if (fl >= TY) lx = 1 + ((fl - TY) >> 1), ly = ((fl - TY) & 1) ? TY - 1 : 0;
    if (!segq[(lx * TY + ly) * nseg + c]) continue;
    const int kdx = k < 3 ? -1 : 0, kdy = k < 3 ? k - 1 : -1;
    const int xx = T.x0 + lx + kdx, yy = T.y0 + ly + kdy;
    const bool cross = (kdx < 0 && lx == 0) || (kdy < 0 && ly == 0) || (kdy > 0 && ly == TY - 1);
    if (!(cross && ly < T.nyl && xx >= V.px0 && yy >= V.py0 && yy <= V.py1)) continue;
    const u32 slot = atomicAdd(&s_nw, 1u);
    if (slot < XC_WCAP)
      wl[slot] = (u32)fi;
    else
      st_agent(&F.fctr[FCTR(9)], 18u);
  }
  for (int it = threadIdx.x; it < T.items; it += NT) {
    if (!segs[it]) continue;
    const u32 slot0 = atomicAdd(&s_nw, 9u);
    for (int l = 0; l < 9; ++l) {
      const u32 e = 0x80000000u | (u32)(it * 9 + l);
      if (slot0 + (u32)l < XC_WCAP)
        wl[slot0 + (u32)l] = e;
      else
        st_agent(&F.fctr[FCTR(9)], 18u);
    }
  }
  __syncthreads();
  FR_DBG_MARK(F, dblk, 2);
  const u32 nw = min(s_nw, (u32)XC_WCAP);
  for (u32 w0 = 0; w0 < nw; w0 += 2 * NT) {
    u32 b0 = 0u, b1 = 0u, o0 = 0u, o1 = 0u, i0 = 0u, i1 = 0u;
    int n0 = 0, n1 = 0, xa = 0, ya = 0, xb = 0, yb = 0;
    u64 wa = 0ull, wb = 0ull;
    const u32 ja = w0 + threadIdx.x, jb = ja + NT;
    if (ja < nw) decode(wl[ja], b0, o0, n0, i0, xa, ya);
    if (jb < nw) decode(wl[jb], b1, o1, n1, i1, xb, yb);
    wa = q_window34(g, V, F, xa, ya, (int)(i0 & 0xFFu));
    wb = q_window34(g, V, F, xb, yb, (int)(i1 & 0xFFu));
    if (!b0) wa = 0ull;
    if (!b1) wb = 0ull;
#pragma nounroll
    for (int h = 0; h < 2; ++h) {
      const u32 bb = h ? b1 : b0;
      const u64 ww = h ? wb : wa;
      if (bb && ww) do_item(bb, h ? o1 : o0, h ? n1 : n0, h ? i1 : i0, ww);
      flush_pairs();
    }
  }
  __syncthreads();
  FR_DBG_MARK(F, dblk, 3);
  const u32 n = s_n;
  if (n != 0u) {
    const u32 xcd = blockIdx.x & 7u;
    if (threadIdx.x == 0) s_base = atomicAdd(&F.fctr[FCTR(16 + xcd)], n);
    __syncthreads();
    const u32 base = s_base;
    if (base + n > FR_PCAP / 8u) {
      if (threadIdx.x == 0) st_agent(&F.fctr[FCTR(9)], 14u);
    } else if (threadIdx.x < n)
      st_agent(&F.pairs[(size_t)xcd * (FR_PCAP / 8u) + base + threadIdx.x], s_list[threadIdx.x]);
  }
  FR_DBG_MARK(F, dblk, 4);
  if constexpr (NT == 512) {
    if (rcap == 0u) return;
    __shared__ u32 s_last;
    wait_vm_stores();
    __syncthreads();
    if (threadIdx.x == 0) {
      const u32 xcd = blockIdx.x & 7u, n_x = ((u32)V.ntiles_f + 7u - xcd) >> 3;
      u32 last = 0u;
      if (atomicAdd(&F.fctr[FR_DONE_CTR + FCTR(1 + xcd)], 1u) == n_x - 1u) {
        const u32 n_groups = min((u32)V.ntiles_f, 8u);
        last = atomicAdd(&F.fctr[FR_DONE_CTR], 1u) == n_groups - 1u ? 1u : 0u;
      }
      s_last = last;
    }
    __syncthreads();
    if (!s_last) return;
    const bool no_kr = (rcap >> 31) != 0u;
    if (resolve_body<NT, true>(g, F, V, smem_raw, rcap & 0x7FFFFFFFu) || !no_kr) return;
    if (threadIdx.x == 0) {
      F.counts[2] = 3u;
      F.h_counts[2] = 3u;
      F.h_counts[6] = 20u;
      __hip_atomic_store(&F.h_counts[15], V.epoch, __ATOMIC_RELEASE, __HIP_MEMORY_SCOPE_SYSTEM);
    }
  }
}

struct CAcc {
  u32 n, sx, sy, sz, cl, lx, ly, lz, hx, hy, hz;
};
__device__ __forceinline__ void cacc_reduce(CAcc& a) {
  a.n = wave_add_u32(a.n), a.sx = wave_add_u32(a.sx), a.sy = wave_add_u32(a.sy), a.sz = wave_add_u32(a.sz);
  a.cl = wave_min_u32(a.cl), a.lx = wave_min_u32(a.lx), a.ly = wave_min_u32(a.ly), a.lz = wave_min_u32(a.lz);
  a.hx = wave_max_u32(a.hx), a.hy = wave_max_u32(a.hy), a.hz = wave_max_u32(a.hz);
}

#define RS_TK 1024
#define RS_SH 512
static inline size_t resolve_lds_bytes(size_t rcap) {
  return (4 * rcap + 6 * (size_t)FR_KCAP + 6 * (size_t)FR_KCAP + 3 * (size_t)RS_SH) * sizeof(u32) + 3 * (size_t)FR_KCAP * sizeof(unsigned long long);
}
template <int RS_T, bool IN_LAUNCH>
__device__ __forceinline__ bool resolve_body(const Geo& g, const FArgs& F, const FVar& V, unsigned char* smem_raw, const u32 rcap) {
  auto ldw = [&](const u32* p) -> u32 { return IN_LAUNCH ? ld_agent(p) : *p; };
  u32* par = reinterpret_cast<u32*>(smem_raw);
  u32* siz = par + rcap;
  u32* clm = siz + rcap;
  u32* rko = clm + rcap;
  u32* k_adr = rko + rcap;
  u32* k_slot = k_adr + FR_KCAP;
  u32* k_size = k_slot + FR_KCAP;
  u32* k_nq = k_size + FR_KCAP;
  u32* k_rank = k_nq + FR_KCAP;
  u32* k_off = k_rank + FR_KCAP;
  u32* kbox = k_off + FR_KCAP;
  u32* h_adr = kbox + FR_KCAP * 6;
  u32* h_sum = h_adr + RS_SH;
  u32* h_kept = h_sum + RS_SH;
  unsigned long long* ksum = reinterpret_cast<unsigned long long*>(h_kept + RS_SH);
  u32* pmx = siz;
  __shared__ u32 s_nk, s_ovf, s_nout, s_nq;
  __shared__ u32 s_fc[32];
  __shared__ u32 s_pre[9];
  const int lane = threadIdx.x & 63, wave = threadIdx.x >> 6;
  const int ntx = V.ntx_f;
  if (threadIdx.x < 32) s_fc[threadIdx.x] = ldw(&F.fctr[FCTR(threadIdx.x)]);
  const int dblk = V.ntiles_f;
  FR_DBG_MARK(F, dblk, 0);
  __syncthreads();
  if (threadIdx.x == 0) {
    s_nk = 0u, s_ovf = s_fc[9], s_nout = 0u, s_nq = 0u;
    u32 run = 0u;
    for (int k = 0; k < 8; ++k) {
      s_pre[k] = run;
      run += min(s_fc[k], (u32)FR_RC8);
    }
    s_pre[8] = run;
  }
  __syncthreads();
  const bool dead = s_ovf != 0u;
  const u32 R = s_pre[8];
  if (!dead && R > rcap) return false;
  auto dense_of = [&](u32 gidx) { return s_pre[gidx / FR_RC8] + (gidx & (FR_RC8 - 1u)); };
  auto gid_of = [&](u32 d) {
    u32 xc = 0u;
#pragma unroll
    for (int k = 1; k < 8; ++k) xc += d >= s_pre[k] ? 1u : 0u;
    return xc * FR_RC8 + (d - s_pre[xc]);
  };
  const u32 Rr = (R + RS_T - 1u) / RS_T * RS_T;
  u32 pp[9];
  pp[0] = 0u;
#pragma unroll
  for (int xc = 0; xc < 8; ++xc) pp[xc + 1] = pp[xc] + min(s_fc[16 + xc], FR_PCAP / 8u);
  auto pair_at = [&](u32 p) {
    u32 xc = 0u;
#pragma unroll
    for (int k = 1; k < 8; ++k) xc += p >= pp[k] ? 1u : 0u;
    return ldw(&F.pairs[(size_t)xc * (FR_PCAP / 8u) + (p - pp[xc])]);
  };
  u32 pk0 = 0u, pk1 = 0u, pk2 = 0u, pk3 = 0u;
  TRec T0, T1;
  T0.size = T1.size = 0u;
  auto load_rec = [&](u32 gi) -> TRec {
    TRec T;
    if (IN_LAUNCH)
      ld_agent_trec2(&F.trec[gi], &F.trec[gi], T, T);
    else
      T = F.trec[gi];
    return T;
  };
  if (!dead) {
    if (threadIdx.x < pp[8]) pk0 = pair_at(threadIdx.x);
    if (threadIdx.x + RS_T < pp[8]) pk1 = pair_at(threadIdx.x + RS_T);
    if (threadIdx.x + 2 * RS_T < pp[8]) pk2 = pair_at(threadIdx.x + 2 * RS_T);
    if (threadIdx.x + 3 * RS_T < pp[8]) pk3 = pair_at(threadIdx.x + 3 * RS_T);
    u32 nq_part = 0u;
    {
      const u32 d0 = threadIdx.x, d1 = threadIdx.x + RS_T;
      const u32 g0 = gid_of(min(d0, R ? R - 1u : 0u)), g1 = gid_of(min(d1, R ? R - 1u : 0u));
      const u32 c0 = ldw(&F.tclaim[g0]), c1 = ldw(&F.tclaim[g1]);
      if (IN_LAUNCH)
        ld_agent_trec2(&F.trec[g0], &F.trec[g1], T0, T1);
      else
        T0 = F.trec[g0], T1 = F.trec[g1];
      if (d0 < R) par[d0] = d0, siz[d0] = T0.size, clm[d0] = c0, rko[d0] = T0.own, nq_part += T0.size;
      if (d1 < R) par[d1] = d1, siz[d1] = T1.size, clm[d1] = c1, rko[d1] = T1.own, nq_part += T1.size;
    }
    for (u32 d = threadIdx.x + 2 * RS_T; d < R; d += RS_T) {
      const u32 gi = gid_of(d);
      const TRec T = load_rec(gi);
      par[d] = d;
      siz[d] = T.size;
      clm[d] = ldw(&F.tclaim[gi]);
      rko[d] = T.own;
      nq_part += T.size;
    }
    nq_part = wave_add_u32(nq_part);
    if (lane == 0 && nq_part) atomicAdd(&s_nq, nq_part);
    for (u32 i = threadIdx.x; i < RS_SH; i += RS_T) h_adr[i] = NOCLAIM, h_sum[i] = 0u, h_kept[i] = FR_NOTKEPT;
    for (u32 i = threadIdx.x; i < FR_KCAP * 6; i += RS_T) kbox[i] = (i % 6u) < 3u ? 0xFFFFFFFFu : 0u;
    for (u32 i = threadIdx.x; i < FR_KCAP * 3; i += RS_T) ksum[i] = 0ull;
  }
  __syncthreads();
  FR_DBG_MARK(F, dblk, 1);
  if (!dead) {
    if (threadIdx.x < pp[8]) lds_union_h(par, dense_of(pk0 >> 16), dense_of(pk0 & 0xFFFFu));
    if (threadIdx.x + RS_T < pp[8]) lds_union_h(par, dense_of(pk1 >> 16), dense_of(pk1 & 0xFFFFu));
    if (threadIdx.x + 2 * RS_T < pp[8]) lds_union_h(par, dense_of(pk2 >> 16), dense_of(pk2 & 0xFFFFu));
    if (threadIdx.x + 3 * RS_T < pp[8]) lds_union_h(par, dense_of(pk3 >> 16), dense_of(pk3 & 0xFFFFu));
    for (u32 p = threadIdx.x + 4 * RS_T; p < pp[8]; p += RS_T) {
      const u32 key = pair_at(p);
      lds_union_h(par, dense_of(key >> 16), dense_of(key & 0xFFFFu));
    }
  }
  __syncthreads();
  FR_DBG_MARK(F, dblk, 2);
  if (!dead) {
    for (u32 d0 = 0; d0 < Rr; d0 += RS_T) {
      const u32 d = d0 + threadIdx.x;
      const u32 rt = d < R ? lds_find_h(par, d) : 0u;
      const bool mov = d < R && rt != d;
      const u32 sz = mov ? siz[d] : 0u, cl = mov ? clm[d] : NOCLAIM, ow = mov ? rko[d] : NOCLAIM;
      u64 todo = __ballot(mov);
      while (todo) {
        const int leader = __builtin_ctzll(todo);
        const u32 first = (u32)__shfl((int)rt, leader, 64);
        const bool mine = mov && rt == first;
        u32 s2 = mine ? sz : 0u, c2 = mine ? cl : NOCLAIM, o2 = mine ? ow : NOCLAIM;
        s2 = wave_add_u32(s2), c2 = wave_min_u32(c2), o2 = wave_min_u32(o2);
        if (lane == leader) {
          atomicAdd(&siz[first], s2);
          atomicMin(&clm[first], c2);
          atomicMin(&rko[first], o2);
        }
        todo &= ~__ballot(mine);
      }
    }
  }
  __syncthreads();
  FR_DBG_MARK(F, dblk, 3);
  if (!dead) {
    for (u32 d = threadIdx.x; d < R; d += RS_T) {
      if (lds_find_h(par, d) != d) continue;
      const u32 cl = clm[d], ow = rko[d];
      if (cl == NOCLAIM) {
        rko[d] = FR_UNCLAIMED;
        continue;
      }
      if (cl == ow) {
        if ((int)siz[d] > F.cluster_min) {
          const u32 e = atomicAdd(&s_nk, 1u);
          if (e < FR_KCAP) {
            k_adr[e] = cl, k_slot[e] = 0u, k_size[e] = siz[d], k_nq[e] = siz[d];
            rko[d] = e;
          } else {
            s_ovf = 1u;
            rko[d] = FR_NOTKEPT;
          }
        } else
          rko[d] = FR_NOTKEPT;
      } else {
        u32 h = (cl * 2654435761u) >> 23;
        bool done = false;
        for (int probe = 0; probe < RS_SH && !done; ++probe) {
          const u32 old = atomicCAS(&h_adr[h], NOCLAIM, cl);
          if (old == NOCLAIM || old == cl) {
            atomicAdd(&h_sum[h], siz[d]);
            rko[d] = 0x80000000u | h;
            done = true;
          }
          h = (h + 1u) & (RS_SH - 1u);
        }
        if (!done) {
          s_ovf = 1u;
          rko[d] = FR_NOTKEPT;
        }
      }
    }
  }
  __syncthreads();
  FR_DBG_MARK(F, dblk, 4);
  if (!dead && threadIdx.x < RS_SH && h_adr[threadIdx.x] != NOCLAIM) {
    const u32 cl = h_adr[threadIdx.x], sum = h_sum[threadIdx.x];
    if ((int)(sum + 1u) > F.cluster_min) {
      const u32 e = atomicAdd(&s_nk, 1u);
      if (e < FR_KCAP) {
        k_adr[e] = cl, k_slot[e] = 0xFFFFFFFFu, k_size[e] = sum + 1u, k_nq[e] = sum;
        h_kept[threadIdx.x] = e;
      } else
        s_ovf = 1u;
    }
  }
  __syncthreads();
  FR_DBG_MARK(F, dblk, 5);
  const u32 nk = min(s_nk, (u32)FR_KCAP);
  const u32 nq = s_nq;
  if (IN_LAUNCH && !dead && s_ovf == 0u && (size_t)nk * (size_t)ntx > 2 * (size_t)rcap) return false;
  const bool bad =dead || s_ovf != 0u || (size_t)nk * (size_t)ntx > 2 * (size_t)rcap || ntx > F.pm_stride;
  if (!bad) {
    if (threadIdx.x < nk) {
      const u32 ai = k_adr[threadIdx.x];
      u32 rank = 0u, off = 0u;
      for (u32 j = 0; j < nk; ++j)
        if (k_adr[j] < ai) {
          ++rank;
          off += k_nq[j];
        }
      k_rank[threadIdx.x] = rank;
      k_off[threadIdx.x] = off;
      atomicAdd(&s_nout, k_nq[threadIdx.x]);
    }
    for (u32 i = threadIdx.x; i < nk * (u32)ntx; i += RS_T) pmx[i] = 0u;
  }
  __syncthreads();
  FR_DBG_MARK(F, dblk, 6);
  if (!bad) {
    for (u32 d0 = 0; d0 < Rr; d0 += RS_T) {
      const u32 d = d0 + threadIdx.x;
      u32 e = FR_UNCLAIMED, gi = 0u;
      if (d < R) {
        gi = gid_of(d);
        e = rko[lds_find_h(par, d)];
        if (e != FR_UNCLAIMED && e != FR_NOTKEPT && (e & 0x80000000u)) e = h_kept[e & 0x7FFFFFFFu];
      }
      const bool kept = e < FR_KCAP;
      if (d < R) F.rcode[gi] = kept ? k_rank[e] : e;
      CAcc A;
      A.n = 0u, A.sx = A.sy = A.sz = 0u, A.cl = A.lx = A.ly = A.lz = 0xFFFFFFFFu, A.hx = A.hy = A.hz = 0u;
      if (kept) {
        const TRec T = d0 == 0u ? T0 : (d0 == (u32)RS_T ? T1 : load_rec(gi));
        A.sx = T.sx, A.sy = T.sy, A.sz = T.sz, A.lx = T.lo[0], A.ly = T.lo[1], A.lz = T.lo[2];
        A.hx = T.hi[0], A.hy = T.hi[1], A.hz = T.hi[2];
        atomicAdd(&pmx[k_rank[e] * (u32)ntx + T.tx], T.size);
      }
      const u64 km = __ballot(kept);
      if (km) {
        u32 first = (u32)__shfl((int)e, __builtin_ctzll(km), 64);
        {
          const u64 same = __ballot(kept && e == first);
          const u64 rest = km & ~same;
          if (rest) {
            const u32 second = (u32)__shfl((int)e, __builtin_ctzll(rest), 64);
            if (__popcll(__ballot(kept && e == second)) > __popcll(same)) first = second;
          }
        }
        const bool mine = kept && e == first;
        auto add = [&](u32 ke, const CAcc& B) {
          unsigned long long* qs = ksum + ke * 3u;
          u32* q = kbox + ke * 6u;
          atomicAdd(&qs[0], (unsigned long long)B.sx), atomicAdd(&qs[1], (unsigned long long)B.sy);
          atomicAdd(&qs[2], (unsigned long long)B.sz);
          atomicMin(&q[0], B.lx), atomicMin(&q[1], B.ly), atomicMin(&q[2], B.lz);
          atomicMax(&q[3], B.hx), atomicMax(&q[4], B.hy), atomicMax(&q[5], B.hz);
        };
        if (kept && !mine) add(e, A);
        CAcc B = A;
        if (!mine) B.sx = B.sy = B.sz = 0u, B.lx = B.ly = B.lz = 0xFFFFFFFFu, B.hx = B.hy = B.hz = 0u;
        cacc_reduce(B);
        if (lane == __builtin_ctzll(__ballot(mine))) add(first, B);
      }
    }
  }
  __syncthreads();
  FR_DBG_MARK(F, dblk, 7);
  if (!bad) {
    for (u32 r = (u32)wave; r < nk; r += RS_T / 64) {
      u32 run = 0u;
      for (int c0 = 0; c0 < ntx; c0 += 64) {
        const int c = c0 + lane;
        const u32 v = c < ntx ? pmx[r * (u32)ntx + (u32)c] : 0u;
        u32 s = v;
        for (int off = 1; off < 64; off <<= 1) {
          const u32 t = (u32)__shfl_up((int)s, off, 64);
          if (lane >= off) s += t;
        }
        if (c < ntx) F.pm[(size_t)r * F.pm_stride + c] = run + s - v;
        run += (u32)__shfl((int)s, 63, 64);
      }
    }
  }
  if (F.dbg && threadIdx.x == 0) {
    F.dbg[(size_t)dblk * FR_DBG_SLOTS + 9] = pp[8];
    F.dbg[(size_t)dblk * FR_DBG_SLOTS + 10] = R;
    F.dbg[(size_t)dblk * FR_DBG_SLOTS + 11] = nq;
  }
  if (!bad && threadIdx.x < nk) {
    const u32 e = threadIdx.x;
    KeptRec r;
    r.addr = k_adr[e], r.slot = k_slot[e], r.size = k_size[e], r.off = k_off[e];
    r.sum[0] = ksum[e * 3u], r.sum[1] = ksum[e * 3u + 1u], r.sum[2] = ksum[e * 3u + 2u];
    for (int k = 0; k < 6; ++k) r.box[k] = kbox[e * 6u + (u32)k];
    r.pad[0] = r.pad[1] = 0u;
    F.krec[k_rank[e]] = r;
    F.h_rec[k_rank[e]] = r;
  }
  if (threadIdx.x == 0) {
    const bool cap = !bad && nq > F.cap_q;
    F.counts[0] = min(nq, F.cap_q);
    F.counts[1] = 0u;
    F.counts[2] = bad ? 2u : (cap ? 1u : 0u);
    F.counts[6] = dead ? s_fc[9] : (s_ovf ? 16u : (bad ? 17u : 0u));
    F.counts[3] = bad ? 0u : nk;
    F.counts[5] = bad ? 0u : s_nout;
  }
  if (threadIdx.x < 32) F.fctr[FCTR(threadIdx.x)] = 0u;
  if (threadIdx.x >= 32 && threadIdx.x < 41) F.fctr[FR_DONE_CTR + FCTR(threadIdx.x - 32)] = 0u;
  if (threadIdx.x == 0) {
    F.counts[8] = V.epoch;
    F.counts[9] = IN_LAUNCH ? 1u : 0u;
    F.counts[10] = R;
  }
  __syncthreads();
  if (threadIdx.x < 15) F.h_counts[threadIdx.x] = F.counts[threadIdx.x];
  __syncthreads();
  FR_DBG_MARK(F, dblk, 8);
  if (threadIdx.x == 0) {
    __hip_atomic_store(&F.h_counts[15], V.epoch, __ATOMIC_RELEASE, __HIP_MEMORY_SCOPE_SYSTEM);
  }
  return true;
}
__global__ void __launch_bounds__(RS_TK) k_resolve(Geo g, FArgs F) {
  extern __shared__ __attribute__((aligned(16))) unsigned char smem_raw[];
  __shared__ FVar s_v;
  __shared__ u32 s_done;
  {
    constexpr int NV = (int)(sizeof(FVar) / 4);
    const int t = threadIdx.x;
    const u32* src = reinterpret_cast<const u32*>(F.var) + (t < NV ? t : 0);
    if (t == NV) src = F.counts + 8;
    const u32 w = *src;
    if (t < NV) reinterpret_cast<u32*>(&s_v)[t] = w;
    if (t == NV) s_done = w;
    __syncthreads();
    if (s_done == s_v.epoch) return;
  }
  (void)resolve_body<RS_TK, false>(g, F, s_v, smem_raw, FR_RCAP);
}

template <int NT>
__global__ void __launch_bounds__(NT) k_tile_out(Geo g, FArgs F) {
  FR_DBG_MARK(F, blockIdx.x, 14);
  __shared__ TilePro s_pro;
  stage_tile_pro(F, &s_pro);
  const FVar& V = s_pro.V;
  if ((int)blockIdx.x >= V.ntiles_f) return;
  if (s_pro.ovf) return;
  const TileGeo T = tile_geo(g, V, blockIdx.x);
  const int nseg = T.nseg, items = T.items, TY = T.TY;
  extern __shared__ __attribute__((aligned(16))) unsigned char smem_raw[];
  u32* segb = reinterpret_cast<u32*>(smem_raw);
  u32* segpre = segb + items;
  u32* segs = segpre + items + 1;
  u32* cadr = segs + items;
  u32* rowall = cadr + FR_TCELL;
  u32* rowpos = rowall + T.TX * FR_TROOT;
  u32* kmap = rowpos + T.TX * FR_TROOT;
  u32* code = kmap + FR_KCAP;
  unsigned short* ckey = reinterpret_cast<unsigned short*>(code + FR_TROOT);
  __shared__ u32 s_wsum[NT / 64];
  __shared__ u32 s_cn[64], s_cb[64], s_cp[65];
  const int lane = threadIdx.x & 63, wave = threadIdx.x >> 6;
  const int dblk = 2 * V.ntiles_f + 2 + (int)blockIdx.x;
  FR_DBG_MARK(F, dblk, 0);
  const u32 nroots = s_pro.nroots, gbase = s_pro.gbase;
  u32 my_code = F.rcode[gbase + (threadIdx.x < nroots ? threadIdx.x : 0u)];
  if (threadIdx.x >= nroots) my_code = FR_UNCLAIMED;
  const u64 my_tl = reinterpret_cast<const u64*>(F.tlab + (size_t)blockIdx.x * FR_TCELL)[threadIdx.x & (FR_TCELL / 8 - 1)];
  u32 pre_cn, pre_cb;
  {
    const bool ok = threadIdx.x < 64 && (int)threadIdx.x < V.nty_f;
    const int tt = ok ? T.tx * V.nty_f + (int)threadIdx.x : (int)blockIdx.x;
    pre_cn = F.t_nroots[tt], pre_cb = F.t_base[tt];
    if (!ok) pre_cn = 0u, pre_cb = 0u;
  }
  const u32 total = tile_load_arrays<NT, true>(T, F, segb, segpre, s_wsum, segs);
  FR_DBG_MARK(F, dblk, 1);
  auto or_flags = [&](long a0, u32 bits) {
    if (!bits) return;
    const long w = a0 >> 6;
    const int sh = (int)(a0 & 63);
    atomicOr(reinterpret_cast<unsigned long long*>(&F.flag[w]), (unsigned long long)bits << sh);
    if (sh > 32) atomicOr(reinterpret_cast<unsigned long long*>(&F.flag[w + 1]), (unsigned long long)bits >> (64 - sh));
  };
  if (total == 0u || nroots == 0u) {
    for (int it = threadIdx.x; it < items; it += NT) {
      const u32 sb = segs[it];
      if (!sb) continue;
      const int line = it / nseg, c = it - line * nseg;
      or_flags(tile_line_adr(g, T, line) + 32 * c, sb);
    }
    return;
  }
  for (int k = threadIdx.x; k < FR_KCAP; k += NT) kmap[k] = 0xFFFFFFFFu;
  for (int k = threadIdx.x; k < T.TX * FR_TROOT; k += NT) rowall[k] = 0u, rowpos[k] = 0u;
  if (threadIdx.x < nroots) code[threadIdx.x] = my_code;
  __syncthreads();
  if (threadIdx.x < nroots && code[threadIdx.x] < FR_KCAP) atomicMin(&kmap[code[threadIdx.x]], threadIdx.x);
  if (threadIdx.x < FR_TCELL / 8) {
#pragma unroll
    for (int q = 0; q < 8; ++q) ckey[8 * threadIdx.x + q] = (unsigned short)((my_tl >> (8 * q)) & 0xFFull);
  }
  for (int it = threadIdx.x; it < items; it += NT) {
    u32 rem = segb[it];
    if (!rem) continue;
    const int line = it / nseg, c = it - line * nseg;
    const u32 a0 = (u32)(tile_line_adr(g, T, line) + 32 * c);
    u32 l = segpre[it];
    while (rem) {
      const int b = __builtin_ctz(rem);
      rem &= rem - 1u;
      cadr[l++] = a0 + (u32)b;
    }
  }
  __syncthreads();
  for (u32 l = threadIdx.x; l < total; l += NT) {
    const u32 cd = code[ckey[l]];
    ckey[l] = (unsigned short)(cd < FR_KCAP ? kmap[cd] : (cd == FR_UNCLAIMED ? 0xFFFFu : 0xFFFEu));
  }
  FR_DBG_MARK(F, dblk, 2);
  const int nty = V.nty_f;
  for (int t0 = 0; t0 < nty; t0 += 64) {
    const int nt = min(64, nty - t0);
    __syncthreads();
    if (threadIdx.x < 64) {
      u32 cn = pre_cn, cb = pre_cb;
      if (t0 > 0) {
        cn = cb = 0u;
        if ((int)threadIdx.x < nt) {
          const int tt = T.tx * nty + t0 + threadIdx.x;
          cn = F.t_nroots[tt], cb = F.t_base[tt];
        }
      }
      u32 s = cn;
      for (int off = 1; off < 64; off <<= 1) {
        const u32 t = (u32)__shfl_up((int)s, off, 64);
        if (lane >= off) s += t;
      }
      s_cn[threadIdx.x] = cn, s_cb[threadIdx.x] = cb, s_cp[threadIdx.x] = s - cn;
      if (threadIdx.x == 63) s_cp[64] = s;
    }
    __syncthreads();
    const u32 ncomp = s_cp[64];
    for (u32 j = threadIdx.x; j < ncomp; j += NT) {
      int lo = 0, hi = nt - 1;
      while (lo < hi) {
        const int mid = (lo + hi + 1) >> 1;
        if (s_cp[mid] <= j)
          lo = mid;
        else
          hi = mid - 1;
      }
      const u32 gi = s_cb[lo] + (j - s_cp[lo]);
      const u32 cd = F.rcode[gi];
      if (cd >= FR_KCAP) continue;
      const u32 rep = kmap[cd];
      if (rep == 0xFFFFFFFFu) continue;
      const uint4* rw = reinterpret_cast<const uint4*>(F.rrow + (size_t)gi * FR_TXS);
      const uint4 r0 = rw[0], r1 = rw[1];
      const u32 pk[8] = {r0.x, r0.y, r0.z, r0.w, r1.x, r1.y, r1.z, r1.w};
      const bool front = t0 + lo < T.ty;
#pragma unroll
      for (int q = 0; q < 8; ++q) {
        const u32 c0 = pk[q] & 0xFFFFu, c1 = pk[q] >> 16;
        if (c0 && 2 * q < T.TX) {
          atomicAdd(&rowall[(2 * q) * FR_TROOT + rep], c0);
          if (front) atomicAdd(&rowpos[(2 * q) * FR_TROOT + rep], c0);
        }
        if (c1 && 2 * q + 1 < T.TX) {
          atomicAdd(&rowall[(2 * q + 1) * FR_TROOT + rep], c1);
          if (front) atomicAdd(&rowpos[(2 * q + 1) * FR_TROOT + rep], c1);
        }
      }
    }
  }
  __syncthreads();
  FR_DBG_MARK(F, dblk, 3);
  for (u32 j = threadIdx.x; j < nroots * (u32)T.TX; j += NT) {
    const u32 rep = j / (u32)T.TX, lx = j - rep * (u32)T.TX;
    const u32 cd = code[rep];
    if (cd >= FR_KCAP || kmap[cd] != rep) continue;
    u32 pos = F.krec[cd].off + F.pm[(size_t)cd * F.pm_stride + T.tx];
    for (u32 q = 0; q < lx; ++q) pos += rowall[q * FR_TROOT + rep];
    rowpos[lx * FR_TROOT + rep] += pos;
  }
  __syncthreads();
  FR_DBG_MARK(F, dblk, 4);
  u32* key_out = F.ms_key[1];
  u32* val_out = F.ms_val[1];
  const bool direct = F.counts[0] <= F.hcells_direct_max;
  for (int lx = wave; lx < T.nxl; lx += NT / 64) {
    const u32 l0 = segpre[lx * TY * nseg], l1 = segpre[(lx + 1) * TY * nseg];
    for (u32 lb = l0; lb < l1; lb += 64u) {
      const u32 l = lb + (u32)lane;
      const u32 kk = l < l1 ? (u32)ckey[l] : 0xFFFFu;
      const bool active = kk < FR_TROOT;
      u32 pos = 0u;
      u64 todo = __ballot(active);
      while (todo) {
        const int leader = __builtin_ctzll(todo);
        const u32 dl = (u32)__shfl((int)kk, leader, 64);
        const u64 same = __ballot(active && kk == dl);
        volatile u32* rp = &rowpos[(u32)lx * FR_TROOT + dl];
        const u32 base = *rp;
        if (active && kk == dl) pos = base + (u32)__popcll(same & ((1ull << lane) - 1ull));
        if (lane == leader) *rp = base + (u32)__popcll(same);
        todo &= ~same;
      }
      if (active) {
        const u32 a = cadr[l];
        key_out[pos] = code[kk];
        val_out[pos] = a;
        if (direct) F.h_cells[pos] = a;
      }
    }
  }
  FR_DBG_MARK(F, dblk, 5);
  for (int it = threadIdx.x; it < items; it += NT) {
    u32 rem = segb[it];
    u32 fl = segs[it];
    u32 l = segpre[it];
    while (rem) {
      const int b = __builtin_ctz(rem);
      rem &= rem - 1u;
      if (ckey[l++] != 0xFFFFu) fl |= 1u << b;
    }
    if (!fl) continue;
    const int line = it / nseg, c = it - line * nseg;
    or_flags(tile_line_adr(g, T, line) + 32 * c, fl);
  }  FR_DBG_MARK(F, dblk, 6);
}

static const int kFastMenu[4][2] = {{16, 32}, {8, 32}, {8, 16}, {4, 8}};
int menu_tiles(int qx, int qy, int mk) {
  return ((qx + kFastMenu[mk][0] - 1) / kFastMenu[mk][0]) * ((qy + kFastMenu[mk][1] - 1) / kFastMenu[mk][1]);
}
static int fast_launch_tiles(const FArgs& F, int mk) {
  return menu_tiles(F.qbox.hi[0] - F.qbox.lo[0] + 2, F.qbox.hi[1] - F.qbox.lo[1] + 2, mk);
}
void set_fast_tiles(FVar& hv, int mk) {
  const int qx = hv.px1 - hv.px0 + 1, qy = hv.py1 - hv.py0 + 1;
  hv.ftx = kFastMenu[mk][0], hv.fty = kFastMenu[mk][1];
  hv.ntx_f = std::max(0, (qx + hv.ftx - 1) / hv.ftx);
  hv.nty_f = std::max(0, (qy + hv.fty - 1) / hv.fty);
  hv.ntiles_f = hv.ntx_f * hv.nty_f;
}

int frontier_enqueue_fast(fuelmi_frontier* f) {
  const Geo& g = f->map->g;
  FArgs& F = f->F;
  const int mk = f->fast_menu;
  const int tiles = fast_launch_tiles(F, mk);
  if (f->tl_ev) HIPCHK(hipEventRecord(f->tl_ev[0], f->stream));
  k_tile_ccl<512><<<tiles, 512, f->tile_lds[mk], f->stream>>>(g, F, *f->h_var);
  FDBG("k_tile_ccl");
  g_ht.lap(4);
  if (f->mark_planes_read) {
    HIPCHK(hipEventRecord(f->ev_planes_read, f->stream));
    map_add_plane_reader(f->map, f->ev_planes_read);
  } else {
    map_add_late_reader(f->map, f->stream, f->ev_planes_read, &f->mark_planes_read);
  }
  if (f->tl_ev) HIPCHK(hipEventRecord(f->tl_ev[1], f->stream));
  g_ht.lap(5);
  {
    bool fuse_now = f->h_var->ntiles_f > 0;
    if (fuse_now && f->fuse_skip > 0) --f->fuse_skip, fuse_now = false;
    f->fuse_tried = fuse_now;
    const size_t lds_x = fuse_now ? std::max(f->cross_lds[mk], resolve_lds_bytes(1024)) : f->cross_lds[mk];
    const u32 rcap = fuse_now ? (u32)std::min<size_t>((lds_x - resolve_lds_bytes(0)) / 16, FR_RCAP) : 0u;
    f->kr_queued = !(fuse_now && f->kr_skip_ok);
    k_tile_cross<512><<<tiles, 512, lds_x, f->stream>>>(g, F, rcap | (f->kr_queued ? 0u : 0x80000000u));
    f->rcap_used = rcap;
  }
  FDBG("k_tile_cross");
  g_ht.lap(6);
  if (f->kr_queued) k_resolve<<<1, RS_TK, f->resolve_lds, f->stream>>>(g, F);
  FDBG("k_resolve");
  g_ht.lap(7);
  if (f->tl_ev) HIPCHK(hipEventRecord(f->tl_ev[2], f->stream));
  k_tile_out<512><<<tiles, 512, f->out_lds[mk], f->stream>>>(g, F);
  FDBG("k_tile_out");
  g_ht.lap(8);
  if (f->tl_ev) HIPCHK(hipEventRecord(f->tl_ev[3], f->stream));
  HIPCHK(hipGetLastError());
  return FUELMI_OK;
}

size_t frontier_tile_lds(fuelmi_frontier* f, int qx, int qy) {
  const Geo& g = f->map->g;
  size_t seg_words = 0;
  for (int k = 0; k < 4; ++k) {
    const int ftx = kFastMenu[k][0], fty = kFastMenu[k][1];
    const size_t items = (size_t)(ftx * fty) * ((g.nz + 31) / 32);
    seg_words = std::max(seg_words, (size_t)((qx + 1 + ftx - 1) / ftx) * ((qy + 1 + fty - 1) / fty) * items);
    f->fast_items[k] = items;
    f->tile_lds[k] = (FR_TCELL + 3 * items + 1 + (size_t)FR_TROOT * 8 + (size_t)FR_TROOT * FR_TXS) * sizeof(u32) +
                     FR_TCELL * sizeof(unsigned short) + FR_TCELL;
    f->cross_lds[k] = (2 * items + (size_t)XC_WCAP) * sizeof(u32);
    f->out_lds[k] = (3 * items + 1 + FR_TCELL + 2 * (size_t)kFastMenu[k][0] * FR_TROOT + FR_KCAP + FR_TROOT) * sizeof(u32) +
                    FR_TCELL * sizeof(unsigned short);
    f->tile_lds[k] = (f->tile_lds[k] + 15) & ~(size_t)15;
    f->cross_lds[k] = (f->cross_lds[k] + 15) & ~(size_t)15;
    f->out_lds[k] = (f->out_lds[k] + 15) & ~(size_t)15;
  }
  return seg_words;
}
int frontier_tile_attrs(fuelmi_frontier* f) {
  const size_t lds_max = std::max(f->tile_lds[0], f->out_lds[0]);
  if (lds_max > 64 * 1024 && lds_max <= 150 * 1024) {
    HIPCHK(hipFuncSetAttribute(reinterpret_cast<const void*>(&k_tile_ccl<512>), hipFuncAttributeMaxDynamicSharedMemorySize, 150 * 1024));
    HIPCHK(hipFuncSetAttribute(reinterpret_cast<const void*>(&k_tile_out<512>), hipFuncAttributeMaxDynamicSharedMemorySize, 150 * 1024));
  }
  f->resolve_lds = resolve_lds_bytes(FR_RCAP);
  HIPCHK(hipFuncSetAttribute(reinterpret_cast<const void*>(&k_resolve), hipFuncAttributeMaxDynamicSharedMemorySize,
                             (int)f->resolve_lds));
  return FUELMI_OK;
}
bool frontier_tile_fits(const fuelmi_frontier* f) {
  return std::max(f->tile_lds[0], f->out_lds[0]) <= 150 * 1024 && f->fast_items[0] <= (size_t)FT_PER * 512;
}

int frontier_enqueue_late_resolve(fuelmi_frontier* f) {
  const Geo& g = f->map->g;
  FArgs& F = f->F;
  const int mk = f->fast_menu;
  k_resolve<<<1, RS_TK, f->resolve_lds, f->stream>>>(g, F);
  k_tile_out<512><<<fast_launch_tiles(F, mk), 512, f->out_lds[mk], f->stream>>>(g, F);
  HIPCHK(hipGetLastError());
  return FUELMI_OK;
}
```

### fuel_amd/host.py

```python
import ctypes as C

import numpy as np

from . import _lib
from ._lib import (BsplineBatch, BsplineCfg, CloudCfg, ColRangeCfg, FrontierCfg, GainCfg, GoalCfg, KinoCfg, LocalSegCfg, MapCfg, MapInfo, PathCfg, RefineCfg, RenderCfg, TopoCfg, TrajAdjCfg, TrajChkCfg, TrajSmpCfg, TspCfg,
                   WptrajCfg, YawCfg, YawPathCfg, check, lib)

DEFAULT_MAP = dict(resolution=0.1, ground_height=-1.0, obstacles_inflation=0.199,
                   local_bound_inflate=0.5, default_dist=0.0, optimistic=0, signed_dist=0,
                   p_hit=0.65, p_miss=0.35, p_min=0.12, p_max=0.90, p_occ=0.80,
                   max_ray_length=4.5, virtual_ceil_height=-10.0)
DEFAULT_BSPLINE = dict(ld_smooth=20.0, ld_dist=10.0, ld_feasi=2.0, ld_start=100.0, ld_end=0.5,
                       ld_guide=1.5, ld_waypt=0.3, ld_view=0.0, ld_time=1.0, dist0=0.7,
                       max_vel=2.0, max_acc=2.0, wnl=1.0, dlmin=0.0, bspline_degree=3)

SMOOTHNESS, DISTANCE, FEASIBILITY, START, END, GUIDE, WAYPOINTS, VIEWCONS, MINTIME = \
    (1 << k for k in range(9))
GUIDE_PHASE = SMOOTHNESS | GUIDE | START | END
NORMAL_PHASE = SMOOTHNESS | DISTANCE | FEASIBILITY | START | END


def _dp(a):
    return None if a is None else a.ctypes.data_as(C.POINTER(C.c_double))

# ... 1123 lines not shown
            self.L.fuelmi_host_unregister(C.c_void_p(self.ptr))
            self.ptr = None
        self.array = None

    def __del__(self):
        try:
            self.close()
        except Exception:
            pass


class EDTEnvironment:

    def __init__(self):
        self.sdf_map_ = None

    def setMap(self, sdf_map):
        self.sdf_map_ = sdf_map

    def evaluateEDTWithGrad(self, pos, time=-1.0):
        return self.sdf_map_.getDistWithGrad(pos)

    def evaluateCoarseEDT(self, pos, time=-1.0):
        return self.sdf_map_.getDistance(pos)


class FrontierFinder:

    def __init__(self, edt_or_map, cluster_min=100, min_z=0.4, cluster_size_xy=2.0, down_sample=3, split=False,
                 reference_order=False):
        self.L = lib()
        self.map = edt_or_map.sdf_map_ if isinstance(edt_or_map, EDTEnvironment) else edt_or_map
        cfg = FrontierCfg(cluster_min, min_z, cluster_size_xy, down_sample, int(split), int(reference_order))
        h = C.c_void_p()
        check(self.L.fuelmi_frontier_create(self.map.h, C.byref(cfg), C.byref(h)))
        self.h = h

    def close(self):
        if getattr(self, "h", None):
            self.L.fuelmi_frontier_destroy(self.h)
            self.h = None

    def __del__(self):
        try:
            self.close()
        except Exception:
            pass

    def searchFrontiers(self):
        n = C.c_int()
        check(self.L.fuelmi_frontier_search(self.h, C.byref(n)))
        return n.value

    def searchFrontiersBegin(self):
        check(self.L.fuelmi_frontier_search_begin(self.h))

    def searchFrontiersEnd(self):
        n = C.c_int()
        check(self.L.fuelmi_frontier_search_end(self.h, C.byref(n)))
        return n.value

    def commit(self, dormant=False):
        check(self.L.fuelmi_frontier_commit(self.h, int(dormant)))

    def reset(self):
        check(self.L.fuelmi_frontier_reset(self.h))

    def sync(self):
        from ._lib import check as _c
        _c(self.L.fuelmi_frontier_synchronize(self.h))

    def stats(self):
        o = (C.c_int * 3)()
        check(self.L.fuelmi_frontier_stats(self.h, o))
        return tuple(o)

    def resolvedInLaunch(self):
        return self.L.fuelmi_frontier_resolved_in_launch(self.h)

    def pathStats(self):
        o = (C.c_int * 2)()
        check(self.L.fuelmi_frontier_path_stats(self.h, o))
        return tuple(o)

    def changedStats(self):
        o = (C.c_int * 9)()
        check(self.L.fuelmi_frontier_changed_stats(self.h, o))
        return {"paths": tuple(o[:4]), "nc": o[4], "total": o[5], "mark": o[6], "rebuilds": o[7], "pool_cap": o[8]}

    def orderStats(self):
        o = (C.c_int * 4)()
        check(self.L.fuelmi_frontier_order_stats(self.h, o))
        return tuple(o)

    def clusters(self, which=0):
        out = []
        cnt = self.L.fuelmi_frontier_count(self.h, which)
        if cnt < 0:
            check(cnt)
        for k in range(cnt):
            n = self.L.fuelmi_frontier_cluster_size(self.h, which, k)
            a = np.empty(n, dtype=np.int32)
            check(self.L.fuelmi_frontier_cluster_cells(self.h, which, k, _ip(a)))
            out.append(a)
        return out

    def clusterCentres(self, which=0):
        out = []
        cnt = self.L.fuelmi_frontier_count(self.h, which)
        if cnt < 0:
            check(cnt)
        for k in range(cnt):
            n = self.L.fuelmi_frontier_cluster_size(self.h, which, k)
            a = np.empty((n, 3))
            check(self.L.fuelmi_frontier_cluster_centres(self.h, which, k, _dp(a)))
            out.append(a)
        return out

    def keepPrevious(self, on=True):
        check(self.L.fuelmi_frontier_keep_previous(self.h, int(bool(on))))

    @staticmethod
    def viewpointConfig(rmin=1.5, rmax=2.5, rnum=3, dphi=15 * 3.1415926 / 180.0, clearance=0.21, min_visib_num=15,
                        min_candidate_dist=0.75, min_view_finish_fraction=0.2, top_angle=0.56125,
                        left_angle=0.69222, right_angle=0.68901, max_dist=4.5):
        return _lib.ViewpointCfg(rmin, rmax, rnum, dphi, clearance, min_visib_num, min_candidate_dist,
                                 min_view_finish_fraction, top_angle, left_angle, right_angle, max_dist)

    def setViewpointConfig(self, cfg):
        self.vcfg = cfg
        check(self.L.fuelmi_frontier_set_viewpoint_cfg(self.h, C.byref(cfg)))

    def computeFrontiersToVisit(self):
        a, d = C.c_int(), C.c_int()
        check(self.L.fuelmi_frontier_compute_to_visit(self.h, C.byref(a), C.byref(d)))
        return a.value, d.value

    def viewpoints(self, which, k):
        n = self.L.fuelmi_frontier_viewpoint_count(self.h, which, k)
        if n < 0:
            check(n)
        py = np.empty((n, 4))
        vis = np.empty(n, dtype=np.int32)
        if n:
            check(self.L.fuelmi_frontier_viewpoints(self.h, which, k, _dp(py), _ip(vis)))
        return py, vis

    def isFrontierCovered(self):
        c = C.c_int()
        check(self.L.fuelmi_frontier_is_covered(self.h, C.byref(c)))
        return bool(c.value)

    def getTopViewpointsInfo(self, cur_pos):
        cur = np.asarray(cur_pos, dtype=float)
        pts, yaws, avgs = [], [], []
        for k in range(self.L.fuelmi_frontier_count(self.h, 1)):
            py, _ = self.viewpoints(1, k)
            pick = py[0]
            for v in py:
                if np.linalg.norm(v[:3] - cur) < self.vcfg.min_candidate_dist:
                    continue
                pick = v
                break
            pts.append(pick[:3].copy())
            yaws.append(float(pick[3]))
            avgs.append(self.clusterInfo(1, k)[0])
# ... 293 lines not shown
```

### include/fuelmi.h

```cpp
#ifndef FUELMI_H_
#define FUELMI_H_

#include <stddef.h>
#include <stdint.h>

#ifdef __cplusplus
extern "C" {
#endif

#define FUELMI_OK 0
#define FUELMI_EINVAL (-1)
#define FUELMI_ENODEV (-2)
#define FUELMI_EHIP (-3)
#define FUELMI_ENOMEM (-4)
#define FUELMI_ELIMIT (-5)

#define FUELMI_HWQ_UNINIT 0
#define FUELMI_HWQ_SET 1
#define FUELMI_HWQ_ENV 2
#define FUELMI_HWQ_LATE 3
int fuelmi_init(int hw_queues);
int fuelmi_hw_queues(void);
int fuelmi_hw_queues_state(void);
const char* fuelmi_last_error(void);
// ... 31 lines not shown

int fuelmi_map_create(const fuelmi_map_cfg* cfg, fuelmi_map** out);
void fuelmi_map_destroy(fuelmi_map* m);
int fuelmi_map_get_info(const fuelmi_map* m, fuelmi_map_info* info);

int fuelmi_map_input_points(fuelmi_map* m, const float* xyz, int stride_bytes, int n,
                            const double camera_pos[3]);
int fuelmi_map_insert_plan(int out[8]);
typedef struct {
  double fx, fy, cx, cy;
  double depth_filter_maxdist, depth_filter_mindist;
  int depth_filter_margin;
  double k_depth_scaling_factor;
  int skip_pixel;
} fuelmi_depth_cfg;
int fuelmi_host_register(void* ptr, size_t bytes);
int fuelmi_host_unregister(void* ptr);
int fuelmi_device_alloc(int device, size_t bytes, void** out);
int fuelmi_device_upload(void* dst, const void* src, size_t bytes);
int fuelmi_device_free(void* ptr);
int fuelmi_hbm_triad(int device, size_t bytes, int reps, double* gb_per_s);
int fuelmi_hbm_expand(int device, size_t bytes_in, int reps, double* gb_per_s);
int fuelmi_map_input_depth(fuelmi_map* m, const unsigned short* depth, int rows, int cols,
                           const fuelmi_depth_cfg* cfg, const double cam_pos[3], const double cam_q_wxyz[4],
                           int* n_points);
int fuelmi_map_project_depth(fuelmi_map* m, const unsigned short* depth, int rows, int cols,
                             const fuelmi_depth_cfg* cfg, const double cam_pos[3], const double cam_q_wxyz[4],
                             float* xyz, int cap, int* n_points);
int fuelmi_map_inflate_local(fuelmi_map* m);
int fuelmi_map_update_esdf(fuelmi_map* m);
enum { FUELMI_ESDF_AUTO = -1, FUELMI_ESDF_PLAIN = 0, FUELMI_ESDF_FAR = 1, FUELMI_ESDF_PLAIN32 = 2 };
int fuelmi_map_set_esdf_family(fuelmi_map* m, int family);
int fuelmi_map_last_esdf_family(const fuelmi_map* m);
enum {
  FUELMI_ESDF_K_ZY = 0,
  FUELMI_ESDF_K_ZY4 = 1,
  FUELMI_ESDF_K_ZY_PK2 = 2,
  FUELMI_ESDF_K_X = 3,
  FUELMI_ESDF_K_X4 = 4,
  FUELMI_ESDF_K_X_PK2 = 5
};
enum { FUELMI_ESDF_PLAN_OPTIMISTIC = 1, FUELMI_ESDF_PLAN_SIGNED = 2, FUELMI_ESDF_PLAN_INTS = 42 };
int fuelmi_map_esdf_plan(const int dims[3], const int lo[3], const int hi[3], int family, int flags,
                         int out[FUELMI_ESDF_PLAN_INTS]);
int fuelmi_map_last_inflate_kernel(const fuelmi_map* m);
int fuelmi_map_reset_buffer_all(fuelmi_map* m);
int fuelmi_map_reset_buffer(fuelmi_map* m, const double min_pos[3], const double max_pos[3]);
int fuelmi_map_set_occupied(fuelmi_map* m, const double* pos_xyz, int n, int occ);
int fuelmi_map_get_local_bound(const fuelmi_map* m, int bmin[3], int bmax[3]);
int fuelmi_map_set_local_bound(fuelmi_map* m, const int bmin[3], const int bmax[3]);
int fuelmi_map_get_updated_box(fuelmi_map* m, double bmin[3], double bmax[3], int reset);
int fuelmi_map_set_updated_box(fuelmi_map* m, const double bmin[3], const double bmax[3]);

int fuelmi_map_upload_occupancy(fuelmi_map* m, const double* occ);

int fuelmi_map_sync_host(fuelmi_map* m, const int bmin[3], const int bmax[3], double* occupancy,
                         char* inflate, double* distance);
int fuelmi_map_register_mirrors(fuelmi_map* m, double* occupancy, char* inflate, double* distance);
int fuelmi_map_unregister_mirrors(fuelmi_map* m);

int fuelmi_map_dist_grad(fuelmi_map* m, const double* pos_xyz, int n, double* dist, double* grad_xyz);
int fuelmi_map_coarse_dist(fuelmi_map* m, const double* pos_xyz, int n, double* dist);
int fuelmi_map_query_state(fuelmi_map* m, const int* idx_xyz, int n, int* occupancy, int* inflate);

int fuelmi_map_synchronize(fuelmi_map* m);

typedef struct {
  int cluster_min;
  double min_z;
  double cluster_size_xy;
  int down_sample;
  int split;
  int reference_order;
} fuelmi_frontier_cfg;

typedef struct fuelmi_frontier fuelmi_frontier;

int fuelmi_frontier_create(fuelmi_map* m, const fuelmi_frontier_cfg* cfg, fuelmi_frontier** out);
void fuelmi_frontier_destroy(fuelmi_frontier* f);
int fuelmi_frontier_reset(fuelmi_frontier* f);
int fuelmi_frontier_stats(const fuelmi_frontier* f, int out3[3]);
int fuelmi_frontier_resolved_in_launch(const fuelmi_frontier* f);
int fuelmi_frontier_path_stats(const fuelmi_frontier* f, int out2[2]);
int fuelmi_frontier_changed_stats(const fuelmi_frontier* f, int out[9]);
int fuelmi_frontier_order_stats(const fuelmi_frontier* f, int out4[4]);
int fuelmi_frontier_synchronize(fuelmi_frontier* f);
typedef struct {
  double candidate_rmin, candidate_rmax;
  int candidate_rnum;
  double candidate_dphi;
  double min_candidate_clearance;
  int min_visib_num;
  double min_candidate_dist;
  double min_view_finish_fraction;
  double top_angle, left_angle, right_angle, max_dist;
} fuelmi_viewpoint_cfg;
int fuelmi_frontier_set_viewpoint_cfg(fuelmi_frontier* f, const fuelmi_viewpoint_cfg* cfg);
int fuelmi_frontier_compute_to_visit(fuelmi_frontier* f, int* n_active_new, int* n_dormant_new);
int fuelmi_frontier_viewpoint_count(const fuelmi_frontier* f, int which, int k);
int fuelmi_frontier_viewpoints(const fuelmi_frontier* f, int which, int k, double* pos_yaw4, int* visib);
int fuelmi_frontier_is_covered(fuelmi_frontier* f, int* covered);
int fuelmi_frontier_cluster_filtered_size(const fuelmi_frontier* f, int which, int k);
int fuelmi_frontier_cluster_filtered(const fuelmi_frontier* f, int which, int k, float* xyz);
int fuelmi_frontier_search(fuelmi_frontier* f, int* n_new);
int fuelmi_frontier_search_begin(fuelmi_frontier* f);
int fuelmi_frontier_search_end(fuelmi_frontier* f, int* n_new);
int fuelmi_frontier_keep_previous(fuelmi_frontier* f, int on);
int fuelmi_frontier_commit(fuelmi_frontier* f, int dormant);
int fuelmi_frontier_count(const fuelmi_frontier* f, int which);
int fuelmi_frontier_cluster_size(const fuelmi_frontier* f, int which, int k);
int fuelmi_frontier_cluster_cells(const fuelmi_frontier* f, int which, int k, int* adr);
int fuelmi_frontier_cluster_centres(const fuelmi_frontier* f, int which, int k, double* xyz);
int fuelmi_frontier_cluster_info(const fuelmi_frontier* f, int which, int k, double out9[9]);
int fuelmi_frontier_removed_count(const fuelmi_frontier* f);
int fuelmi_frontier_removed_ids(const fuelmi_frontier* f, int* ids);
int fuelmi_frontier_get_flags(fuelmi_frontier* f, char* flags);

typedef struct {
  double lattice_res;
  double edge_step;
  double no_path_cost;
  int max_path_points;
} fuelmi_path_cfg;
int fuelmi_map_path_costs(fuelmi_map* m, const fuelmi_path_cfg* cfg, int n, const double* p1_xyz,
                          const double* p2_xyz, double* length, int* kind, int* path_len, double* path_xyz);
int fuelmi_map_path_stats(const fuelmi_map* m, int stats[4]);

#define FUELMI_REFINE_LAST_ARGMIN 1
#define FUELMI_REFINE_MAX_LAYERS 64
#define FUELMI_REFINE_MAX_NODES 256
typedef struct {
  fuelmi_path_cfg path;
  double vm, yd, w_dir;
  double tour_lattice_res;
  int max_tour_points;
  int flags;
} fuelmi_refine_cfg;
int fuelmi_map_refine_tours(fuelmi_map* m, const fuelmi_refine_cfg* cfg, int n_prob, const double* start,
                            const int* layer_ptr, const int* node_ptr, const double* nodes, int* choice, double* cost,
                            int* tour_len, double* tour_xyz);

#define FUELMI_GOAL_CLOSE 0
#define FUELMI_GOAL_MID 1
#define FUELMI_GOAL_FAR 2
#define FUELMI_GOAL_NO_PATH 3
typedef struct {
  fuelmi_path_cfg path;
  double shorten_dist;
  double end_eps;
  double radius_close;
  double radius_far;
  int max_way_points;
} fuelmi_goal_cfg;
int fuelmi_map_goal_paths(fuelmi_map* m, const fuelmi_goal_cfg* cfg, int n_prob, const double* start_xyz,
                          const double* goal_xyz, int* status, double* length, int* n_way, double* way_xyz,
                          double* next_goal, int* raw_len, double* raw_xyz);
int fuelmi_map_goal_path_times(const fuelmi_map* m, double ms2[2]);

#define FUELMI_TSP_MAX_DIM 1024
#define FUELMI_TSP_EXACT_CAP 16
#define FUELMI_TSP_DEFAULT_RESTARTS 64
#define FUELMI_TSP_DEFAULT_KICKS 8
#define FUELMI_TSP_DEFAULT_EXACT_MAX 12
typedef struct {
  int restarts, kicks, exact_max;
  uint64_t seed;
// ... 443 lines not shown
```

Before: 11220.

## Size frontier tile kernels' LDS adaptively from recent per-tile usage history

Replaces the fixed worst-case LDS allocations of the frontier tile kernels (ccl, cross, out, fused resolve) with a per-search plan. The plan picks a capacity class from the maximum cells, roots, pairs, worklist and kept counts seen over the last several searches, and the kernels now report those maxima through atomic-max counters. Smaller LDS footprints should let more workgroups run per CU. In exchange, an overflow now triggers a rerun at the full class and a hold period, which adds host logic and the risk of extra launches.

```diff
diff --git a/fuel_amd/_lib.py b/fuel_amd/_lib.py
--- a/fuel_amd/_lib.py
+++ b/fuel_amd/_lib.py
@@ -310,6 +310,8 @@
     "fuelmi_frontier_stats": (C.c_int, [_P, C.POINTER(C.c_int)]),
     "fuelmi_frontier_resolved_in_launch": (C.c_int, [_P]),
     "fuelmi_frontier_path_stats": (C.c_int, [_P, C.POINTER(C.c_int)]),
+    "fuelmi_frontier_lds_plan": (C.c_int, [C.c_int, C.c_int, C.c_int, C.POINTER(C.c_uint), C.POINTER(C.c_uint)]),
+    "fuelmi_frontier_lds_stats": (C.c_int, [_P, C.POINTER(C.c_int)]),
     "fuelmi_frontier_changed_stats": (C.c_int, [_P, C.POINTER(C.c_int)]),
     "fuelmi_frontier_order_stats": (C.c_int, [_P, C.POINTER(C.c_int)]),
     "fuelmi_frontier_synchronize": (C.c_int, [_P]),
diff --git a/fuel_amd/csrc/frontier.hip b/fuel_amd/csrc/frontier.hip
--- a/fuel_amd/csrc/frontier.hip
+++ b/fuel_amd/csrc/frontier.hip
@@ -410,7 +410,13 @@
   f->fusion_at_begin = m->fusion_count;
   f->search_empty = empty;
   f->fast_launched = false;
-  if (empty) return FUELMI_OK;
+  f->lds_force_full = f->lds_full_ttl > 0;
+  if (f->lds_full_ttl > 0) --f->lds_full_ttl;
+  if (empty) {
+    const u32 zeros[16] = {0};
+    frontier_lds_note(f, zeros);
+    return FUELMI_OK;
+  }
 
   int rlo[3], rhi[3];
   const bool all = f->dirty_all || f->seen_epoch != m->occ_epoch;
@@ -452,6 +458,7 @@
       }
     if (f->menu_min_ttl > 0) --f->menu_min_ttl, pick = std::max(pick, f->menu_min);
     f->fast_menu = pick;
+
     hv.px0 = p0[0], hv.py0 = p0[1], hv.px1 = p1[0], hv.py1 = p1[1];
     set_fast_tiles(hv, pick);
   }
@@ -568,6 +575,12 @@
     for (int k = 1; k <= np; ++k) std::fprintf(stderr, " %.1f/%.1f", av[k] / std::max(cnt, 1), mx[k]);
     std::fprintf(stderr, "\n");
   }
+  std::fprintf(stderr, "[fr-timing] lds classes tile %d kept %d roots %d (%u cells %u components %u pairs %u list %u kept %u roots; ccl %u cross %u out %u B); "
+               "this search: %u cells %u components %u pairs %u list %u kept %u roots; reruns %d outgrown %d late %d hold %d\n",
+               f->plan.tile_class, f->plan.kept_class, f->plan.rcap_class, f->plan.caps.tcell, f->plan.caps.troot, f->plan.caps.tpair,
+               f->plan.caps.wcap, f->plan.caps.kcap, f->plan.rcap, f->plan.lds_ccl, f->plan.lds_cross, f->plan.lds_out, F.h_counts[11],
+               F.h_counts[12], F.h_counts[13], F.h_counts[14], F.h_counts[3], F.h_counts[10], f->n_class_rerun, f->n_class_outgrown,
+               f->n_late_resolve, f->lds_full_ttl);
   const unsigned long long* rr = &d[(size_t)nt * FR_DBG_SLOTS];
   std::fprintf(stderr, "[fr-timing] resolve: init %.1f unions %.1f find %.1f reduce %.1f clusters %.1f seeds %.1f rank %.1f "
                "codes %.1f publish %.1f us; pairs %llu roots %llu cells %llu\n", (rr[1] - rr[0]) / 100.0,
@@ -589,6 +602,7 @@
   f->tail_pending = true;
   F.fast = 1;
   if (F.dbg) frontier_timing_report(f);
+  bool late = false;
   if (counts[2] == 3u) {
     *stamp = 0u;
     const int rcl = frontier_enqueue_late_resolve(f);
@@ -596,13 +610,24 @@
     const int rc = stamp_wait<u32>(stamp, want, f->stream, "frontier search: k_resolve finished without publishing its result");
     if (rc) return rc;
     ++f->n_late_resolve;
+    if (f->plan.rcap_class < 2 || f->plan.kept_class < 1) ++f->n_class_outgrown, f->lds_full_ttl = FR_FULL_HOLD;
+    late = true;
   }
   f->kr_skip_ok = counts[2] == 0u && counts[9] == 1u && 2u * counts[10] <= f->rcap_used;
   ++f->n_fast;
   if (counts[9] == 1u)
     ++f->n_in_launch;
-  else if (f->fuse_tried && counts[2] == 0u)
-    f->fuse_skip = 16;
+  else if (f->fuse_tried && counts[2] == 0u && !late) {
+    LdsPlan full;
+    const bool reduced = f->plan.rcap_class < 2 || f->plan.kept_class < 1;
+    const size_t nkx = (size_t)counts[3] * (size_t)f->h_var->ntx_f;
+    if (reduced && frontier_lds_plan(f->fast_menu, m->g.nz, true, nullptr, &full) == FUELMI_OK && counts[10] <= full.rcap &&
+        nkx <= 2 * (size_t)full.rcap) {
+      ++f->n_class_outgrown;
+      f->lds_full_ttl = FR_FULL_HOLD;
+    } else
+      f->fuse_skip = 16;
+  }
   if (counts[2] == 2u && m->fusion_count != f->fusion_at_begin) {
     fuelmi_set_error("frontier search: the fast chain overflowed AFTER the map was fused again (a frame queued between "
                      "_search_begin and _search_end): the occupancy this search was about is gone -- call _search_end before the next fusion "
@@ -611,25 +636,39 @@
     f->dirty_all = true;
     return FUELMI_ELIMIT;
   }
-  while (counts[2] == 2u && f->fast_menu < 3 && (counts[6] == 11u || counts[6] == 12u || counts[6] == 15u || counts[6] == 18u)) {
+  auto run_again = [&](const char* why) -> int {
     HIPCHK(frontier_tail_sync(f) == FUELMI_OK ? hipSuccess : hipErrorUnknown);
-    ++f->fast_menu;
     FVar hv = *f->h_var;
     set_fast_tiles(hv, f->fast_menu);
     hv.epoch = ++f->epoch;
     if (hv.epoch == 0u) hv.epoch = f->epoch = 1u;
     *f->h_var = hv;
     f->kr_skip_ok = false;
-    if (getenv("FUELMI_FR_TIMING")) std::fprintf(stderr, "[fr-timing] capacity code %u: again with %d x %d tiles\n", counts[6], hv.ftx, hv.fty);
+    if (getenv("FUELMI_FR_TIMING")) std::fprintf(stderr, "[fr-timing] capacity code %u: again %s (%d x %d tiles)\n", counts[6], why, hv.ftx, hv.fty);
     const int rcr = frontier_enqueue_fast(f);
     if (rcr) return rcr;
     const int rcw = stamp_wait<u32>(stamp, hv.epoch, f->stream,
-                                    "frontier search: the re-tiled chain finished without publishing its result");
+                                    "frontier search: the chain run again finished without publishing its result");
     if (rcw) return rcw;
     f->tail_pending = true;
+    return FUELMI_OK;
+  };
+  if (counts[2] == 2u && f->plan.tile_class < FR_NCLASS - 1 && (counts[6] == 11u || counts[6] == 12u || counts[6] == 18u)) {
+    f->lds_force_full = true;
+    f->lds_full_ttl = FR_FULL_HOLD;
+    const int rcr = run_again("at the full LDS class");
+    if (rcr) return rcr;
+    ++f->n_class_rerun;
+  }
+  while (counts[2] == 2u && f->fast_menu < 3 && (counts[6] == 11u || counts[6] == 12u || counts[6] == 15u || counts[6] == 18u)) {
+    ++f->fast_menu;
+    f->lds_force_full = true;
+    const int rcr = run_again("on the next smaller tile");
+    if (rcr) return rcr;
     ++f->n_retiled;
     f->menu_min = f->fast_menu, f->menu_min_ttl = 64;
   }
+  if (counts[2] != 2u) frontier_lds_note(f, counts);
   if (counts[2] == 2u) {
     --f->n_fast;
     ++f->n_fallback;
@@ -865,6 +904,15 @@
   out2[0] = f->n_late_resolve, out2[1] = f->n_retiled;
   return FUELMI_OK;
 }
+extern "C" int fuelmi_frontier_lds_stats(const fuelmi_frontier* f, int out[12]) {
+  ARGCHK(f && out);
+  const LdsPlan& P = f->plan;
+  out[0] = f->n_class_rerun, out[1] = f->n_class_outgrown, out[2] = f->lds_full_ttl;
+  out[3] = P.tile_class, out[4] = P.kept_class, out[5] = P.rcap_class;
+  out[6] = (int)P.caps.tcell, out[7] = (int)P.caps.troot, out[8] = (int)P.caps.tpair, out[9] = (int)P.caps.wcap;
+  out[10] = (int)P.caps.kcap, out[11] = (int)P.rcap;
+  return FUELMI_OK;
+}
 extern "C" int fuelmi_frontier_changed_stats(const fuelmi_frontier* f, int out[9]) {
   ARGCHK(f && out);
   for (int k = 0; k < 4; ++k) out[k] = f->rm_paths[k];
diff --git a/fuel_amd/csrc/frontier_internal.h b/fuel_amd/csrc/frontier_internal.h
--- a/fuel_amd/csrc/frontier_internal.h
+++ b/fuel_amd/csrc/frontier_internal.h
@@ -45,9 +45,30 @@
 #define FR_TXS 16
 #define FR_KCAP 256
 #define FR_PCAP (1u << 18)
+#define XC_WCAP 6144
+struct TileCaps {
+  u32 tcell, troot, tpair, wcap;
+  u32 kcap;
+};
+#define FR_NCLASS 4
+#define FR_KCAP_SMALL 32
+#define FR_MARGIN_NUM 3u
+#define FR_MARGIN_DEN 2u
+#define FR_HIST 8
+#define FR_FULL_HOLD 64
+#define FR_NMAX 6
+struct LdsPlan {
+  TileCaps caps;
+  u32 rcap;
+  u32 lds_ccl, lds_cross, lds_out;
+  int tile_class, kept_class, rcap_class;
+};
 #define FCTR(k) ((k) * 32)
+#define FR_MAX_LINES 32
+#define FR_MAX_CTR FCTR(41)
+#define FCTR_MAX0 10
 #define FR_DONE_CTR FCTR(32)
-#define FR_NCTR (41 * 32)
+#define FR_NCTR ((41 + FR_MAX_LINES) * 32)
 #define FR_PMCAP 16384
 #define FR_REFORDER_AUTO 26624u
 #define FR_UNCLAIMED 0xFFFFFFFFu
@@ -123,6 +144,9 @@
 #ifdef __HIPCC__
 __device__ __forceinline__ void st_agent(u32* p, u32 v) { __hip_atomic_store(p, v, __ATOMIC_RELAXED, __HIP_MEMORY_SCOPE_AGENT); }
 __device__ __forceinline__ u32 ld_agent(const u32* p) { return __hip_atomic_load(p, __ATOMIC_RELAXED, __HIP_MEMORY_SCOPE_AGENT); }
+__device__ __forceinline__ void report_max(u32* fctr, int q, u32 v) {
+  (void)__hip_atomic_fetch_max(&fctr[FR_MAX_CTR + FCTR(blockIdx.x % FR_MAX_LINES) + q], v, __ATOMIC_RELAXED, __HIP_MEMORY_SCOPE_AGENT);
+}
 __device__ __forceinline__ void wait_vm_stores() { asm volatile("s_waitcnt vmcnt(0)" ::: "memory"); }
 __device__ __forceinline__ void ld_agent_trec2(const TRec* p0, const TRec* p1, TRec& A, TRec& B) {
   static_assert(sizeof(TRec) == 48, "TRec is fetched as three 16-byte pieces");
@@ -340,6 +364,13 @@
   u32 rcap_used = 0;
   int menu_min = 0, menu_min_ttl = 0;
   int n_retiled = 0;
+  u32 lds_hist[FR_HIST][FR_NMAX] = {};
+  int lds_hist_n = 0, lds_hist_at = 0;
+  int lds_full_ttl = 0;
+  bool lds_force_full = false;
+  LdsPlan plan = {};
+  int n_class_rerun = 0;
+  int n_class_outgrown = 0;
   int n_late_resolve = 0;
   int order_last = 0, n_order_ref = 0, n_order_fallback = 0;
   u32 order_fallback_cells = 0;
@@ -476,6 +507,8 @@
 int frontier_second_pass(fuelmi_frontier* f);
 int frontier_legacy_attrs(fuelmi_frontier* f);
 size_t frontier_tile_lds(fuelmi_frontier* f, int qx, int qy);
+int frontier_lds_plan(int mk, int nz, bool fused, const u32* hist, LdsPlan* out);
+void frontier_lds_note(fuelmi_frontier* f, const u32* counts);
 int frontier_tile_attrs(fuelmi_frontier* f);
 bool frontier_tile_fits(const fuelmi_frontier* f);
 int menu_tiles(int qx, int qy, int mk);
diff --git a/fuel_amd/csrc/frontier_tile.hip b/fuel_amd/csrc/frontier_tile.hip
--- a/fuel_amd/csrc/frontier_tile.hip
+++ b/fuel_amd/csrc/frontier_tile.hip
@@ -93,7 +93,7 @@
 
 template <int NT>
 __device__ __forceinline__ u32 tile_load_pred(const Geo& g, const TileGeo& T, const FVar& V, const FArgs& F, u32* segb,
-                                              u32* segpre, u32* s_wsum, u32* lab, u32* segs, unsigned short* cseg) {
+                                              u32* segpre, u32* s_wsum, u32* lab, u32* segs, unsigned short* cseg, const u32 tcell) {
   const int lane = threadIdx.x & 63, wave = threadIdx.x >> 6;
   const int per = (T.items + NT - 1) / NT;
   const int it0 = threadIdx.x * per;
@@ -146,7 +146,7 @@
     if (it0 + k >= T.items) break;
     u32 rem = segb[it0 + k];
     segpre[it0 + k] = run;
-    if (tot <= FR_TCELL) {
+    if (tot <= tcell) {
       u32 l = run;
       while (rem) {
         const int s0 = __builtin_ctz(rem);
@@ -228,43 +228,45 @@
 }
 
 template <int NT>
-__global__ void __launch_bounds__(NT) k_tile_ccl(Geo g, FArgs F, const FVar V) {
+__global__ void __launch_bounds__(NT) k_tile_ccl(Geo g, FArgs F, const FVar V, const TileCaps C) {
   if (blockIdx.x == 0 && threadIdx.x == 0) *F.var_w = V;
   if ((int)blockIdx.x >= V.ntiles_f) return;
   const TileGeo T = tile_geo(g, V, blockIdx.x);
   const Box3 sbox = V.sbox;
   extern __shared__ __attribute__((aligned(16))) unsigned char smem_raw[];
   const int nz = g.nz, nseg = T.nseg, items = T.items, TY = T.TY;
+  const u32 tcell = C.tcell, troot = C.troot, tpair = C.tpair;
   u32* lab = reinterpret_cast<u32*>(smem_raw);
-  u32* segb = lab + FR_TCELL;
+  u32* segb = lab + tcell;
   u32* segpre = segb + items;
   u32* acc = segpre + items + 1;
-  u32* rrow = acc + FR_TROOT * 8;
-  unsigned short* rootno = reinterpret_cast<unsigned short*>(rrow + FR_TROOT * FR_TXS);
-  unsigned char* rcell = reinterpret_cast<unsigned char*>(rootno + FR_TCELL);
-  u32* segs = reinterpret_cast<u32*>(rcell + FR_TCELL);
+  u32* rrow = acc + troot * 8;
+  unsigned short* rootno = reinterpret_cast<unsigned short*>(rrow + troot * FR_TXS);
+  unsigned char* rcell = reinterpret_cast<unsigned char*>(rootno + tcell);
+  u32* segs = reinterpret_cast<u32*>(rcell + tcell);
   u32* plist = reinterpret_cast<u32*>(rootno);
   unsigned short* cseg = reinterpret_cast<unsigned short*>(acc);
-  static_assert((size_t)FR_TCELL * sizeof(unsigned short) <= (size_t)FR_TROOT * 8 * 4 + (size_t)FR_TROOT * FR_TXS * 4, "cell -> segment table does not fit");
-  static_assert((size_t)FR_TPAIR * sizeof(u32) <= FR_TCELL * sizeof(unsigned short) + FR_TCELL, "pair list does not fit");
   __shared__ u32 s_wsum[NT / 64];
   __shared__ u32 s_nroots, s_base, s_flag;
   __shared__ u32 s_cnt[4];
   const int lane = threadIdx.x & 63;
   if (threadIdx.x == 0) s_nroots = 0u, s_flag = 0u, s_cnt[0] = s_cnt[1] = s_cnt[2] = s_cnt[3] = 0u;
   FR_DBG_MARK(F, blockIdx.x, 0);
-  const u32 total = tile_load_pred<NT>(g, T, V, F, segb, segpre, s_wsum, lab, segs, cseg);
+  const u32 total = tile_load_pred<NT>(g, T, V, F, segb, segpre, s_wsum, lab, segs, cseg, tcell);
   {
     u32* tq = F.tq + (size_t)blockIdx.x * items;
     u32* ts = F.ts + (size_t)blockIdx.x * items;
     for (int it = threadIdx.x; it < items; it += NT) tq[it] = segb[it], ts[it] = segs[it];
   }
   FR_DBG_MARK(F, blockIdx.x, 1);
-  if (total == 0u || total > FR_TCELL) {
+  if (total == 0u || total > tcell) {
     if (threadIdx.x == 0) {
       F.t_nroots[blockIdx.x] = 0u;
       F.t_base[blockIdx.x] = 0u;
-      if (total > FR_TCELL) F.fctr[FCTR(9)] = 11u;
+      if (total > tcell) {
+        F.fctr[FCTR(9)] = 11u;
+        report_max(F.fctr, 0, total);
+      }
     }
     return;
   }
@@ -331,7 +333,7 @@
 #pragma unroll
     for (int k = 0; k < 9; ++k)
       if ((nv >> k) & 1u) {
-        if (at < FR_TPAIR)
+        if (at < tpair)
           plist[at] = pk[k];
         else
           s_povf = 1u;
@@ -341,7 +343,7 @@
   __syncthreads();
   {
     volatile u32* vl = lab;
-    const u32 np = min(s_np, (u32)FR_TPAIR);
+    const u32 np = min(s_np, tpair);
     for (;;) {
       bool any = false;
       for (u32 p = threadIdx.x; p < np; p += NT) {
@@ -378,11 +380,11 @@
     });
   }
   __syncthreads();
-  for (int t = threadIdx.x; t < FR_TROOT * 8; t += NT) {
+  for (int t = threadIdx.x; t < (int)troot * 8; t += NT) {
     const int k = t & 7;
     acc[t] = (k >= 2 && k <= 4) ? 0xFFFFFFFFu : 0u;
   }
-  for (int t = threadIdx.x; t < FR_TROOT * FR_TXS; t += NT) rrow[t] = 0u;
+  for (int t = threadIdx.x; t < (int)troot * FR_TXS; t += NT) rrow[t] = 0u;
   FR_DBG_MARK(F, blockIdx.x, 3);
   for (u32 l = threadIdx.x; l < total; l += NT)
     if (lab[l] == l) {
@@ -391,7 +393,8 @@
     }
   __syncthreads();
   const u32 nroots = s_nroots;
-  if (nroots > FR_TROOT) {
+  if (threadIdx.x == 64) report_max(F.fctr, 0, total), report_max(F.fctr, 1, nroots), report_max(F.fctr, 2, s_np);
+  if (nroots > troot) {
     if (threadIdx.x == 0) {
       F.fctr[FCTR(9)] = 12u;
       F.t_nroots[blockIdx.x] = 0u;
@@ -523,9 +526,9 @@
 }
 
 #define XC_SET 256
-#define XC_WCAP 6144
 template <int RS_T, bool IN_LAUNCH>
-__device__ __forceinline__ bool resolve_body(const Geo& g, const FArgs& F, const FVar& V, unsigned char* smem_raw, const u32 rcap);
+__device__ __forceinline__ bool resolve_body(const Geo& g, const FArgs& F, const FVar& V, unsigned char* smem_raw, const u32 rcap,
+                                             const u32 kcap);
 
 __device__ __forceinline__ void xc_insert(u32* s_set, u32* s_list, u32* s_n, u32* fctr, u32 key) {
   u32 h = (key * 2654435761u) >> 24;
@@ -542,7 +545,7 @@
   if (!done) st_agent(&fctr[FCTR(9)], 15u);
 }
 template <int NT>
-__global__ void __launch_bounds__(NT) k_tile_cross(Geo g, FArgs F, const u32 rcap) {
+__global__ void __launch_bounds__(NT) k_tile_cross(Geo g, FArgs F, const u32 rcap, const TileCaps C) {
   FR_DBG_MARK(F, blockIdx.x, 13);
   __shared__ TilePro s_pro;
   stage_tile_pro(F, &s_pro);
@@ -672,7 +675,7 @@
     const bool cross = (kdx < 0 && lx == 0) || (kdy < 0 && ly == 0) || (kdy > 0 && ly == TY - 1);
     if (!(cross && ly < T.nyl && xx >= V.px0 && yy >= V.py0 && yy <= V.py1)) continue;
     const u32 slot = atomicAdd(&s_nw, 1u);
-    if (slot < XC_WCAP)
+    if (slot < C.wcap)
       wl[slot] = (u32)fi;
     else
       st_agent(&F.fctr[FCTR(9)], 18u);
@@ -682,7 +685,7 @@
     const u32 slot0 = atomicAdd(&s_nw, 9u);
     for (int l = 0; l < 9; ++l) {
       const u32 e = 0x80000000u | (u32)(it * 9 + l);
-      if (slot0 + (u32)l < XC_WCAP)
+      if (slot0 + (u32)l < C.wcap)
         wl[slot0 + (u32)l] = e;
       else
         st_agent(&F.fctr[FCTR(9)], 18u);
@@ -690,7 +693,7 @@
   }
   __syncthreads();
   FR_DBG_MARK(F, dblk, 2);
-  const u32 nw = min(s_nw, (u32)XC_WCAP);
+  const u32 nw = min(s_nw, C.wcap);
   for (u32 w0 = 0; w0 < nw; w0 += 2 * NT) {
     u32 b0 = 0u, b1 = 0u, o0 = 0u, o1 = 0u, i0 = 0u, i1 = 0u;
     int n0 = 0, n1 = 0, xa = 0, ya = 0, xb = 0, yb = 0;
@@ -712,6 +715,7 @@
   }
   __syncthreads();
   FR_DBG_MARK(F, dblk, 3);
+  if (threadIdx.x == 0 && s_nw * FR_MARGIN_NUM > (XC_WCAP / FR_NCLASS) * FR_MARGIN_DEN) report_max(F.fctr, 3, s_nw);
   const u32 n = s_n;
   if (n != 0u) {
     const u32 xcd = blockIdx.x & 7u;
@@ -741,7 +745,7 @@
     __syncthreads();
     if (!s_last) return;
     const bool no_kr = (rcap >> 31) != 0u;
-    if (resolve_body<NT, true>(g, F, V, smem_raw, rcap & 0x7FFFFFFFu) || !no_kr) return;
+    if (resolve_body<NT, true>(g, F, V, smem_raw, rcap & 0x7FFFFFFFu, C.kcap) || !no_kr) return;
     if (threadIdx.x == 0) {
       F.counts[2] = 3u;
       F.h_counts[2] = 3u;
@@ -762,24 +766,25 @@
 
 #define RS_TK 1024
 #define RS_SH 512
-static inline size_t resolve_lds_bytes(size_t rcap) {
-  return (4 * rcap + 6 * (size_t)FR_KCAP + 6 * (size_t)FR_KCAP + 3 * (size_t)RS_SH) * sizeof(u32) + 3 * (size_t)FR_KCAP * sizeof(unsigned long long);
+static inline size_t resolve_lds_bytes(size_t rcap, size_t kcap = FR_KCAP) {
+  return (4 * rcap + 6 * kcap + 6 * kcap + 3 * (size_t)RS_SH) * sizeof(u32) + 3 * kcap * sizeof(unsigned long long);
 }
 template <int RS_T, bool IN_LAUNCH>
-__device__ __forceinline__ bool resolve_body(const Geo& g, const FArgs& F, const FVar& V, unsigned char* smem_raw, const u32 rcap) {
+__device__ __forceinline__ bool resolve_body(const Geo& g, const FArgs& F, const FVar& V, unsigned char* smem_raw, const u32 rcap,
+                                             const u32 kcap) {
   auto ldw = [&](const u32* p) -> u32 { return IN_LAUNCH ? ld_agent(p) : *p; };
   u32* par = reinterpret_cast<u32*>(smem_raw);
   u32* siz = par + rcap;
   u32* clm = siz + rcap;
   u32* rko = clm + rcap;
   u32* k_adr = rko + rcap;
-  u32* k_slot = k_adr + FR_KCAP;
-  u32* k_size = k_slot + FR_KCAP;
-  u32* k_nq = k_size + FR_KCAP;
-  u32* k_rank = k_nq + FR_KCAP;
-  u32* k_off = k_rank + FR_KCAP;
-  u32* kbox = k_off + FR_KCAP;
-  u32* h_adr = kbox + FR_KCAP * 6;
+  u32* k_slot = k_adr + kcap;
+  u32* k_size = k_slot + kcap;
+  u32* k_nq = k_size + kcap;
+  u32* k_rank = k_nq + kcap;
+  u32* k_off = k_rank + kcap;
+  u32* kbox = k_off + kcap;
+  u32* h_adr = kbox + kcap * 6;
   u32* h_sum = h_adr + RS_SH;
   u32* h_kept = h_sum + RS_SH;
   unsigned long long* ksum = reinterpret_cast<unsigned long long*>(h_kept + RS_SH);
@@ -789,7 +794,10 @@
   __shared__ u32 s_pre[9];
   const int lane = threadIdx.x & 63, wave = threadIdx.x >> 6;
   const int ntx = V.ntx_f;
+  __shared__ u32 s_mx[FR_MAX_LINES * 4];
   if (threadIdx.x < 32) s_fc[threadIdx.x] = ldw(&F.fctr[FCTR(threadIdx.x)]);
+  if (threadIdx.x >= 64 && threadIdx.x < 64 + FR_MAX_LINES * 4)
+    s_mx[threadIdx.x - 64] = ldw(&F.fctr[FR_MAX_CTR + FCTR((threadIdx.x - 64) >> 2) + ((threadIdx.x - 64) & 3)]);
   const int dblk = V.ntiles_f;
   FR_DBG_MARK(F, dblk, 0);
   __syncthreads();
@@ -801,6 +809,11 @@
       run += min(s_fc[k], (u32)FR_RC8);
     }
     s_pre[8] = run;
+  }
+  if (threadIdx.x >= 64 && threadIdx.x < 68) {
+    u32 mx = 0u;
+    for (int k = 0; k < FR_MAX_LINES; ++k) mx = max(mx, s_mx[4 * k + (int)threadIdx.x - 64]);
+    s_fc[FCTR_MAX0 + (int)threadIdx.x - 64] = mx;
   }
   __syncthreads();
   const bool dead = s_ovf != 0u;
@@ -864,8 +877,8 @@
     nq_part = wave_add_u32(nq_part);
     if (lane == 0 && nq_part) atomicAdd(&s_nq, nq_part);
     for (u32 i = threadIdx.x; i < RS_SH; i += RS_T) h_adr[i] = NOCLAIM, h_sum[i] = 0u, h_kept[i] = FR_NOTKEPT;
-    for (u32 i = threadIdx.x; i < FR_KCAP * 6; i += RS_T) kbox[i] = (i % 6u) < 3u ? 0xFFFFFFFFu : 0u;
-    for (u32 i = threadIdx.x; i < FR_KCAP * 3; i += RS_T) ksum[i] = 0ull;
+    for (u32 i = threadIdx.x; i < kcap * 6; i += RS_T) kbox[i] = (i % 6u) < 3u ? 0xFFFFFFFFu : 0u;
+    for (u32 i = threadIdx.x; i < kcap * 3; i += RS_T) ksum[i] = 0ull;
   }
   __syncthreads();
   FR_DBG_MARK(F, dblk, 1);
@@ -916,7 +929,7 @@
       if (cl == ow) {
         if ((int)siz[d] > F.cluster_min) {
           const u32 e = atomicAdd(&s_nk, 1u);
-          if (e < FR_KCAP) {
+          if (e < kcap) {
             k_adr[e] = cl, k_slot[e] = 0u, k_size[e] = siz[d], k_nq[e] = siz[d];
             rko[d] = e;
           } else {
@@ -950,7 +963,7 @@
     const u32 cl = h_adr[threadIdx.x], sum = h_sum[threadIdx.x];
     if ((int)(sum + 1u) > F.cluster_min) {
       const u32 e = atomicAdd(&s_nk, 1u);
-      if (e < FR_KCAP) {
+      if (e < kcap) {
         k_adr[e] = cl, k_slot[e] = 0xFFFFFFFFu, k_size[e] = sum + 1u, k_nq[e] = sum;
         h_kept[threadIdx.x] = e;
       } else
@@ -959,7 +972,8 @@
   }
   __syncthreads();
   FR_DBG_MARK(F, dblk, 5);
-  const u32 nk = min(s_nk, (u32)FR_KCAP);
+  if (IN_LAUNCH && !dead && kcap < (u32)FR_KCAP && s_nk > kcap) return false;
+  const u32 nk = min(s_nk, kcap);
   const u32 nq = s_nq;
   if (IN_LAUNCH && !dead && s_ovf == 0u && (size_t)nk * (size_t)ntx > 2 * (size_t)rcap) return false;
   const bool bad =dead || s_ovf != 0u || (size_t)nk * (size_t)ntx > 2 * (size_t)rcap || ntx > F.pm_stride;
@@ -1071,10 +1085,13 @@
   }
   if (threadIdx.x < 32) F.fctr[FCTR(threadIdx.x)] = 0u;
   if (threadIdx.x >= 32 && threadIdx.x < 41) F.fctr[FR_DONE_CTR + FCTR(threadIdx.x - 32)] = 0u;
+  if (threadIdx.x >= 64 && threadIdx.x < 64 + FR_MAX_LINES * 4) F.fctr[FR_MAX_CTR + FCTR((threadIdx.x - 64) >> 2) + ((threadIdx.x - 64) & 3)] = 0u;
   if (threadIdx.x == 0) {
     F.counts[8] = V.epoch;
     F.counts[9] = IN_LAUNCH ? 1u : 0u;
     F.counts[10] = R;
+    F.counts[11] = s_fc[FCTR_MAX0], F.counts[12] = s_fc[FCTR_MAX0 + 1], F.counts[13] = s_fc[FCTR_MAX0 + 2];
+    F.counts[14] = s_fc[FCTR_MAX0 + 3];
   }
   __syncthreads();
   if (threadIdx.x < 15) F.h_counts[threadIdx.x] = F.counts[threadIdx.x];
@@ -1100,11 +1117,11 @@
     __syncthreads();
     if (s_done == s_v.epoch) return;
   }
-  (void)resolve_body<RS_TK, false>(g, F, s_v, smem_raw, FR_RCAP);
+  (void)resolve_body<RS_TK, false>(g, F, s_v, smem_raw, FR_RCAP, FR_KCAP);
 }
 
 template <int NT>
-__global__ void __launch_bounds__(NT) k_tile_out(Geo g, FArgs F) {
+__global__ void __launch_bounds__(NT) k_tile_out(Geo g, FArgs F, const TileCaps C) {
   FR_DBG_MARK(F, blockIdx.x, 14);
   __shared__ TilePro s_pro;
   stage_tile_pro(F, &s_pro);
@@ -1117,12 +1134,13 @@
   u32* segb = reinterpret_cast<u32*>(smem_raw);
   u32* segpre = segb + items;
   u32* segs = segpre + items + 1;
+  const u32 tcell = C.tcell, troot = C.troot;
   u32* cadr = segs + items;
-  u32* rowall = cadr + FR_TCELL;
-  u32* rowpos = rowall + T.TX * FR_TROOT;
-  u32* kmap = rowpos + T.TX * FR_TROOT;
+  u32* rowall = cadr + tcell;
+  u32* rowpos = rowall + T.TX * troot;
+  u32* kmap = rowpos + T.TX * troot;
   u32* code = kmap + FR_KCAP;
-  unsigned short* ckey = reinterpret_cast<unsigned short*>(code + FR_TROOT);
+  unsigned short* ckey = reinterpret_cast<unsigned short*>(code + troot);
   __shared__ u32 s_wsum[NT / 64];
   __shared__ u32 s_cn[64], s_cb[64], s_cp[65];
   const int lane = threadIdx.x & 63, wave = threadIdx.x >> 6;
@@ -1158,11 +1176,11 @@
     return;
   }
   for (int k = threadIdx.x; k < FR_KCAP; k += NT) kmap[k] = 0xFFFFFFFFu;
-  for (int k = threadIdx.x; k < T.TX * FR_TROOT; k += NT) rowall[k] = 0u, rowpos[k] = 0u;
+  for (int k = threadIdx.x; k < T.TX * (int)troot; k += NT) rowall[k] = 0u, rowpos[k] = 0u;
   if (threadIdx.x < nroots) code[threadIdx.x] = my_code;
   __syncthreads();
   if (threadIdx.x < nroots && code[threadIdx.x] < FR_KCAP) atomicMin(&kmap[code[threadIdx.x]], threadIdx.x);
-  if (threadIdx.x < FR_TCELL / 8) {
+  if (threadIdx.x < tcell / 8) {
 #pragma unroll
     for (int q = 0; q < 8; ++q) ckey[8 * threadIdx.x + q] = (unsigned short)((my_tl >> (8 * q)) & 0xFFull);
   }
@@ -1229,12 +1247,12 @@
       for (int q = 0; q < 8; ++q) {
         const u32 c0 = pk[q] & 0xFFFFu, c1 = pk[q] >> 16;
         if (c0 && 2 * q < T.TX) {
-          atomicAdd(&rowall[(2 * q) * FR_TROOT + rep], c0);
-          if (front) atomicAdd(&rowpos[(2 * q) * FR_TROOT + rep], c0);
+          atomicAdd(&rowall[(2 * q) * troot + rep], c0);
+          if (front) atomicAdd(&rowpos[(2 * q) * troot + rep], c0);
         }
         if (c1 && 2 * q + 1 < T.TX) {
-          atomicAdd(&rowall[(2 * q + 1) * FR_TROOT + rep], c1);
-          if (front) atomicAdd(&rowpos[(2 * q + 1) * FR_TROOT + rep], c1);
+          atomicAdd(&rowall[(2 * q + 1) * troot + rep], c1);
+          if (front) atomicAdd(&rowpos[(2 * q + 1) * troot + rep], c1);
         }
       }
     }
@@ -1246,8 +1264,8 @@
     const u32 cd = code[rep];
     if (cd >= FR_KCAP || kmap[cd] != rep) continue;
     u32 pos = F.krec[cd].off + F.pm[(size_t)cd * F.pm_stride + T.tx];
-    for (u32 q = 0; q < lx; ++q) pos += rowall[q * FR_TROOT + rep];
-    rowpos[lx * FR_TROOT + rep] += pos;
+    for (u32 q = 0; q < lx; ++q) pos += rowall[q * troot + rep];
+    rowpos[lx * troot + rep] += pos;
   }
   __syncthreads();
   FR_DBG_MARK(F, dblk, 4);
@@ -1259,14 +1277,14 @@
     for (u32 lb = l0; lb < l1; lb += 64u) {
       const u32 l = lb + (u32)lane;
       const u32 kk = l < l1 ? (u32)ckey[l] : 0xFFFFu;
-      const bool active = kk < FR_TROOT;
+      const bool active = kk < troot;
       u32 pos = 0u;
       u64 todo = __ballot(active);
       while (todo) {
         const int leader = __builtin_ctzll(todo);
         const u32 dl = (u32)__shfl((int)kk, leader, 64);
         const u64 same = __ballot(active && kk == dl);
-        volatile u32* rp = &rowpos[(u32)lx * FR_TROOT + dl];
+        volatile u32* rp = &rowpos[(u32)lx * troot + dl];
         const u32 base = *rp;
         if (active && kk == dl) pos = base + (u32)__popcll(same & ((1ull << lane) - 1ull));
         if (lane == leader) *rp = base + (u32)__popcll(same);
@@ -1311,13 +1329,85 @@
   hv.ntiles_f = hv.ntx_f * hv.nty_f;
 }
 
+static inline bool class_holds(u32 v, u32 cap) { return (unsigned long long)v * FR_MARGIN_NUM <= (unsigned long long)cap * FR_MARGIN_DEN; }
+int frontier_lds_plan(int mk, int nz, bool fused, const u32* hist, LdsPlan* out) {
+  if (mk < 0 || mk > 3 || nz < 1 || !out) return FUELMI_EINVAL;
+  const size_t items = (size_t)(kFastMenu[mk][0] * kFastMenu[mk][1]) * (size_t)((nz + 31) / 32);
+  static const u32 unit[4] = {FR_TCELL / FR_NCLASS, FR_TROOT / FR_NCLASS, FR_TPAIR / FR_NCLASS, XC_WCAP / FR_NCLASS};
+  int tc = FR_NCLASS - 1, kc = 1, rc = 2;
+  if (hist) {
+    tc = 0;
+    for (int q = 0; q < 4; ++q)
+      while (tc < FR_NCLASS - 1 && !class_holds(hist[q], unit[q] * (u32)(tc + 1) + (q == 2 ? (u32)items : 0u))) ++tc;
+    rc = class_holds(hist[4], 256u) ? 0 : (class_holds(hist[4], 512u) ? 1 : 2);
+    kc = class_holds(hist[5], FR_KCAP_SMALL) ? 0 : 1;
+  }
+  TileCaps& C = out->caps;
+  C.tcell = unit[0] * (u32)(tc + 1), C.troot = unit[1] * (u32)(tc + 1), C.tpair = unit[2] * (u32)(tc + 1) + (u32)items;
+  C.wcap = unit[3] * (u32)(tc + 1);
+  C.kcap = kc ? FR_KCAP : FR_KCAP_SMALL;
+  out->tile_class = tc, out->kept_class = kc, out->rcap_class = rc;
+  if ((size_t)C.tcell * sizeof(unsigned short) > (size_t)C.troot * 8 * 4 + (size_t)C.troot * FR_TXS * 4 ||
+      (size_t)C.tpair * sizeof(u32) > (size_t)C.tcell * sizeof(unsigned short) + C.tcell + items * sizeof(u32) || (C.tcell & 3u) ||
+      C.troot > 255u) {
+    fuelmi_set_error("frontier LDS plan: tile class %d does not hold its aliased tables", tc);
+    return FUELMI_EINVAL;
+  }
+  auto up16 = [](size_t b) { return (b + 15) & ~(size_t)15; };
+  out->lds_ccl = (u32)up16((C.tcell + 3 * items + 1 + (size_t)C.troot * 8 + (size_t)C.troot * FR_TXS) * sizeof(u32) +
+                           C.tcell * sizeof(unsigned short) + C.tcell);
+  const size_t cross = up16((2 * items + (size_t)C.wcap) * sizeof(u32));
+  out->rcap = 0u;
+  out->lds_cross = (u32)cross;
+  if (fused) {
+    const size_t want = rc == 0 ? 256 : (rc == 1 ? 512 : 1024);
+    const size_t lds_x = std::max(cross, resolve_lds_bytes(want, C.kcap));
+    out->rcap = (u32)std::min<size_t>((lds_x - resolve_lds_bytes(0, C.kcap)) / 16, FR_RCAP);
+    out->lds_cross = (u32)lds_x;
+  }
+  out->lds_out = (u32)up16((3 * items + 1 + C.tcell + 2 * (size_t)kFastMenu[mk][0] * C.troot + FR_KCAP + C.troot) * sizeof(u32) +
+                           C.tcell * sizeof(unsigned short));
+  return FUELMI_OK;
+}
+extern "C" int fuelmi_frontier_lds_plan(int menu, int nz, int fused, const unsigned* recent_max, unsigned out[12]) {
+  ARGCHK(out);
+  LdsPlan P;
+  const int rc = frontier_lds_plan(menu, nz, fused != 0, recent_max, &P);
+  if (rc) {
+    if (menu < 0 || menu > 3 || nz < 1) fuelmi_set_error("fuelmi_frontier_lds_plan: menu entry 0..3 and nz >= 1 expected");
+    return rc;
+  }
+  out[0] = P.caps.tcell, out[1] = P.caps.troot, out[2] = P.caps.tpair, out[3] = P.caps.wcap, out[4] = P.rcap, out[5] = P.caps.kcap;
+  out[6] = P.lds_ccl, out[7] = P.lds_cross, out[8] = P.lds_out;
+  out[9] = (unsigned)P.tile_class, out[10] = (unsigned)P.kept_class, out[11] = (unsigned)P.rcap_class;
+  return FUELMI_OK;
+}
+void frontier_lds_note(fuelmi_frontier* f, const u32* counts) {
+  u32* h = f->lds_hist[f->lds_hist_at];
+  h[0] = counts[11], h[1] = counts[12], h[2] = counts[13], h[3] = counts[14], h[4] = counts[10], h[5] = counts[3];
+  f->lds_hist_at = (f->lds_hist_at + 1) % FR_HIST;
+  f->lds_hist_n = std::min(f->lds_hist_n + 1, FR_HIST);
+}
+
 int frontier_enqueue_fast(fuelmi_frontier* f) {
   const Geo& g = f->map->g;
   FArgs& F = f->F;
   const int mk = f->fast_menu;
   const int tiles = fast_launch_tiles(F, mk);
+  bool fuse_now = f->h_var->ntiles_f > 0;
+  if (fuse_now && f->fuse_skip > 0) --f->fuse_skip, fuse_now = false;
+  f->fuse_tried = fuse_now;
+  {
+    u32 hmax[FR_NMAX] = {0, 0, 0, 0, 0, 0};
+    for (int k = 0; k < f->lds_hist_n; ++k)
+      for (int q = 0; q < FR_NMAX; ++q) hmax[q] = std::max(hmax[q], f->lds_hist[k][q]);
+    const bool full = f->lds_force_full || f->lds_hist_n == 0;
+    const int rcp = frontier_lds_plan(mk, g.nz, fuse_now, full ? nullptr : hmax, &f->plan);
+    if (rcp) return rcp;
+  }
+  const LdsPlan& P = f->plan;
   if (f->tl_ev) HIPCHK(hipEventRecord(f->tl_ev[0], f->stream));
-  k_tile_ccl<512><<<tiles, 512, f->tile_lds[mk], f->stream>>>(g, F, *f->h_var);
+  k_tile_ccl<512><<<tiles, 512, P.lds_ccl, f->stream>>>(g, F, *f->h_var, P.caps);
   FDBG("k_tile_ccl");
   g_ht.lap(4);
   if (f->mark_planes_read) {
@@ -1329,13 +1419,9 @@
   if (f->tl_ev) HIPCHK(hipEventRecord(f->tl_ev[1], f->stream));
   g_ht.lap(5);
   {
-    bool fuse_now = f->h_var->ntiles_f > 0;
-    if (fuse_now && f->fuse_skip > 0) --f->fuse_skip, fuse_now = false;
-    f->fuse_tried = fuse_now;
-    const size_t lds_x = fuse_now ? std::max(f->cross_lds[mk], resolve_lds_bytes(1024)) : f->cross_lds[mk];
-    const u32 rcap = fuse_now ? (u32)std::min<size_t>((lds_x - resolve_lds_bytes(0)) / 16, FR_RCAP) : 0u;
+    const u32 rcap = P.rcap;
     f->kr_queued = !(fuse_now && f->kr_skip_ok);
-    k_tile_cross<512><<<tiles, 512, lds_x, f->stream>>>(g, F, rcap | (f->kr_queued ? 0u : 0x80000000u));
+    k_tile_cross<512><<<tiles, 512, P.lds_cross, f->stream>>>(g, F, rcap | (f->kr_queued ? 0u : 0x80000000u), P.caps);
     f->rcap_used = rcap;
   }
   FDBG("k_tile_cross");
@@ -1344,7 +1430,7 @@
   FDBG("k_resolve");
   g_ht.lap(7);
   if (f->tl_ev) HIPCHK(hipEventRecord(f->tl_ev[2], f->stream));
-  k_tile_out<512><<<tiles, 512, f->out_lds[mk], f->stream>>>(g, F);
+  k_tile_out<512><<<tiles, 512, P.lds_out, f->stream>>>(g, F, P.caps);
   FDBG("k_tile_out");
   g_ht.lap(8);
   if (f->tl_ev) HIPCHK(hipEventRecord(f->tl_ev[3], f->stream));
@@ -1360,14 +1446,9 @@
     const size_t items = (size_t)(ftx * fty) * ((g.nz + 31) / 32);
     seg_words = std::max(seg_words, (size_t)((qx + 1 + ftx - 1) / ftx) * ((qy + 1 + fty - 1) / fty) * items);
     f->fast_items[k] = items;
-    f->tile_lds[k] = (FR_TCELL + 3 * items + 1 + (size_t)FR_TROOT * 8 + (size_t)FR_TROOT * FR_TXS) * sizeof(u32) +
-                     FR_TCELL * sizeof(unsigned short) + FR_TCELL;
-    f->cross_lds[k] = (2 * items + (size_t)XC_WCAP) * sizeof(u32);
-    f->out_lds[k] = (3 * items + 1 + FR_TCELL + 2 * (size_t)kFastMenu[k][0] * FR_TROOT + FR_KCAP + FR_TROOT) * sizeof(u32) +
-                    FR_TCELL * sizeof(unsigned short);
-    f->tile_lds[k] = (f->tile_lds[k] + 15) & ~(size_t)15;
-    f->cross_lds[k] = (f->cross_lds[k] + 15) & ~(size_t)15;
-    f->out_lds[k] = (f->out_lds[k] + 15) & ~(size_t)15;
+    LdsPlan P;
+    (void)frontier_lds_plan(k, g.nz, true, nullptr, &P);
+    f->tile_lds[k] = P.lds_ccl, f->cross_lds[k] = P.lds_cross, f->out_lds[k] = P.lds_out;
   }
   return seg_words;
 }
@@ -1391,7 +1472,7 @@
   FArgs& F = f->F;
   const int mk = f->fast_menu;
   k_resolve<<<1, RS_TK, f->resolve_lds, f->stream>>>(g, F);
-  k_tile_out<512><<<fast_launch_tiles(F, mk), 512, f->out_lds[mk], f->stream>>>(g, F);
+  k_tile_out<512><<<fast_launch_tiles(F, mk), 512, f->plan.lds_out, f->stream>>>(g, F, f->plan.caps);
   HIPCHK(hipGetLastError());
   return FUELMI_OK;
 }
diff --git a/fuel_amd/host.py b/fuel_amd/host.py
--- a/fuel_amd/host.py
+++ b/fuel_amd/host.py
@@ -1229,6 +1229,11 @@
         o = (C.c_int * 2)()
         check(self.L.fuelmi_frontier_path_stats(self.h, o))
         return tuple(o)
+
+    def ldsStats(self):
+        o = (C.c_int * 12)()
+        check(self.L.fuelmi_frontier_lds_stats(self.h, o))
+        return {"reruns": o[0], "outgrown": o[1], "hold": o[2], "classes": tuple(o[3:6]), "caps": tuple(o[6:12])}
 
     def changedStats(self):
         o = (C.c_int * 9)()
diff --git a/include/fuelmi.h b/include/fuelmi.h
--- a/include/fuelmi.h
+++ b/include/fuelmi.h
@@ -137,6 +137,9 @@
 int fuelmi_frontier_stats(const fuelmi_frontier* f, int out3[3]);
 int fuelmi_frontier_resolved_in_launch(const fuelmi_frontier* f);
 int fuelmi_frontier_path_stats(const fuelmi_frontier* f, int out2[2]);
+enum { FUELMI_FRONTIER_LDS_PLAN_INTS = 12 };
+int fuelmi_frontier_lds_plan(int menu, int nz, int fused, const unsigned* recent_max, unsigned out[FUELMI_FRONTIER_LDS_PLAN_INTS]);
+int fuelmi_frontier_lds_stats(const fuelmi_frontier* f, int out[12]);
 int fuelmi_frontier_changed_stats(const fuelmi_frontier* f, int out[9]);
 int fuelmi_frontier_order_stats(const fuelmi_frontier* f, int out4[4]);
 int fuelmi_frontier_synchronize(fuelmi_frontier* f);
```

New measurement: 11410 (median of 4 runs). About the same (+1.7%).
